# ChainSafe/halo2-verifier

Hardware: AMD Instinct MI355X
Metric: proofs verified/sec (BN254, k=14) (higher is better)
Workload: dtype u32 limbs (254-bit prime-field integers)

## Files before the change

### halo2_verifier_amd/csrc/batch.hip

```cpp
#include "../../include/h2v.h"
#include "batch.h"
#include <string.h>
#include <algorithm>
#include <utility>
#include <stdio.h>

using namespace h2v;

namespace h2v {

struct BatchSizes {
    uint32_t stream_words;
    size_t proofs, inst, pts, ycanon, words, chal, mult, slots, msm_scal, shared, left_scal, insteval, guard_scal, acc, results;
    uint32_t ws_terms, ws_problems, ws_per_problem;
};
BatchSizes batch_sizes(const Plan& pl, size_t N, size_t G, size_t largest) {
    BatchSizes z;
    z.stream_words = stream_words_for(pl.stream.size(), pl.opts.transcript);
    z.proofs = N * pl.proof_len;
    z.inst = N * (size_t)pl.n_instance_values * 32;
    z.pts = N * pl.n_points + pl.n_shared;
    z.ycanon = N * pl.n_points * 32;
    z.words = (size_t)z.stream_words * N;
    z.chal = (size_t)pl.squeeze_at.size() * N;
    z.mult = N;
    z.slots = (size_t)std::max(std::max(pl.n_slots, pl.n_slots_k[0]), std::max(pl.n_slots_k[1], pl.n_slots_k[2])) * N;
    z.msm_scal = (N * pl.n_points + G * pl.n_shared) * 8;
    z.shared = (size_t)pl.n_shared * N;
    z.left_scal = N * pl.n_points * 8;
    z.insteval = N * pl.inst_queries.size();
    z.guard_scal = N * pl.guard_term_order.size() * 8;
    z.acc = 2 * G;
    z.results = ResultsLayout{G, N}.total();
    z.ws_terms = (uint32_t)(2 * (N * pl.n_points + G * pl.n_shared));
    z.ws_problems = (uint32_t)(2 * G);
    z.ws_per_problem = (uint32_t)(largest * pl.n_points + pl.n_shared);
    return z;
}

int ensure_buffers(h2v_batch* b, const Plan& pl) {
    const size_t N = b->max_proofs, G = b->groups;
    size_t largest = (N + G - 1) / G;
    if (ragged(b)) { largest = 0; for (size_t g = 0; g < G; ++g) largest = std::max<size_t>(largest, b->group_off[g + 1] - b->group_off[g]); }
    const BatchSizes z = batch_sizes(pl, N, G, largest);
    int rc;
    if ((rc = b->proofs.reserve(z.proofs)) || (rc = b->inst.reserve(z.inst)) || (rc = b->pts.reserve(z.pts)) || (rc = b->phi.reserve(z.pts)) ||
        (rc = b->ycanon.reserve(z.ycanon)) || (rc = b->words.reserve(z.words)) || (rc = b->chal.reserve(z.chal)) || (rc = b->mult.reserve(z.mult)) ||
        (rc = b->slots.reserve(z.slots)) || (rc = b->msm_scal.reserve(z.msm_scal)) || (rc = b->shared.reserve(z.shared)) ||
        (rc = b->left_scal.reserve(z.left_scal)) || (rc = b->insteval.reserve(z.insteval)) || (rc = b->guard_scal.reserve(z.guard_scal)) ||
        (rc = b->acc.reserve(z.acc)) || (rc = b->results.reserve(z.results)) || (rc = b->results_host.reserve(z.results)))
        return rc;
    const ResultsLayout L{G, N};
    b->ok = reinterpret_cast<uint32_t*>(static_cast<uint8_t*>(b->results_host.dev) + L.ok());
    b->fold_failed = reinterpret_cast<uint32_t*>(b->results.p + L.fold_failed());
    b->out_ident = reinterpret_cast<uint32_t*>(b->results.p + L.out_ident());
    b->out_bytes = b->results.p + L.out_bytes();
    b->status = reinterpret_cast<int*>(b->results.p + L.status());
    if ((rc = b->ws.reserve(z.ws_terms, z.ws_problems, z.ws_per_problem))) return rc;
    b->stream_words = z.stream_words;
    return 0;
}

bool scalar_is_canonical(const uint8_t* s) {
    uint32_t raw[8];
    for (int j = 0; j < 8; ++j) raw[j] = (uint32_t)s[4 * j] | ((uint32_t)s[4 * j + 1] << 8) | ((uint32_t)s[4 * j + 2] << 16) | ((uint32_t)s[4 * j + 3] << 24);
    return !Fr::geq_p(raw);
}
bool scalar_is_zero(const uint8_t* s) { for (int k = 0; k < 32; ++k) if (s[k]) return false; return true; }

int os_random_scalars(std::vector<uint8_t>& out, size_t n) {
    out.resize(32 * n);
    FILE* f = fopen("/dev/urandom", "rb");
    if (!f) { set_last_error("cannot open /dev/urandom"); return H2V_ERR_DEVICE; }
    for (size_t i = 0; i < n; ++i) {
        uint8_t buf[64];
        if (fread(buf, 1, 64, f) != 64) { fclose(f); set_last_error("short read from /dev/urandom"); return H2V_ERR_DEVICE; }
        uint32_t w[16];
        for (int j = 0; j < 16; ++j) w[j] = (uint32_t)buf[4 * j] | ((uint32_t)buf[4 * j + 1] << 8) | ((uint32_t)buf[4 * j + 2] << 16) | ((uint32_t)buf[4 * j + 3] << 24);
        Fr::from_uniform_words(w).to_bytes(&out[32 * i]);
    }
    fclose(f);
    return 0;
}

int require_stage(const h2v_batch* b, BatchStage least, const char* who) {
    if (b && b->stage >= least) return 0;
    static const char* const missing[] = {"", "nothing uploaded since the last failed call or set_groups", "nothing launched", "no finished launch"};
    set_last_error(std::string(who) + ": " + (b ? missing[(int)least] : "null argument"));
    return H2V_ERR_BAD_ARGUMENT;
}

struct StageCommit {
    h2v_batch* b;
    ~StageCommit() { if (b) b->stage = BatchStage::Empty; }
    void commit(BatchStage st) { b->stage = st; b = nullptr; }
};

#define H2V_SPLIT_MAX_GROUPS 64u

ChannelTerms channel_terms(const Plan& pl, uint32_t count, uint32_t n_shared) {
    const bool strided = pl.left_term_order.size() == 1 && !pl.left_term_order[0].first;
    return ChannelTerms{strided, strided ? count : count * pl.n_points, count * pl.n_points + n_shared};
}
bool groups_cut_within_limit(const Plan& pl, const size_t* sizes, size_t n_groups) {
    std::vector<uint32_t> terms;
    for (size_t g = 0; g < n_groups; ++g) { const ChannelTerms t = channel_terms(pl, (uint32_t)sizes[g], pl.n_shared); terms.push_back(t.left); terms.push_back(t.right); }
    return msm_cuts_within_limit(terms.data(), terms.size());
}
void channel_problems(MsmProblems& pr, const h2v_batch* b, const Plan& pl, size_t p0, uint32_t count, G1J* acc2, const uint32_t* shared_scal, uint32_t n_shared) {
    const uint32_t np = pl.n_points;
    const size_t first = p0 * np;
    const ChannelTerms terms = channel_terms(pl, count, n_shared);
    if (terms.strided) {
        const size_t at = first + pl.left_term_order[0].second;
        pr.p.push_back(MsmProblem(b->left_scal.p + at * 8, b->pts.p + at, acc2, 8 * np, np, terms.left));
        pr.p.back().phi = b->phi.p + at;
    } else {
        pr.p.push_back(MsmProblem(b->left_scal.p + first * 8, b->pts.p + first, acc2, 8, 1, terms.left));
        pr.p.back().phi = b->phi.p + first;
        pr.p.back().nnz = count * (uint32_t)pl.left_term_order.size();
    }
    pr.p.push_back(MsmProblem(b->msm_scal.p + first * 8, b->pts.p + first, acc2 + 1, 8, 1, terms.right - n_shared, shared_scal, b->pts.p + (size_t)b->n * np, n_shared));
    pr.p.back().phi = b->phi.p + first; pr.p.back().phi2 = b->phi.p + (size_t)b->n * np;
}

int need_stream(h2v_batch* b) {
    if (b->stream || !b->owns_stream) return 0;
    H2V_HIP_CHECK(hipSetDevice(b->ctx->device));
    H2V_HIP_CHECK(hipStreamCreateWithFlags(&b->stream, hipStreamNonBlocking));
    return 0;
}
int need_aux(h2v_batch* b) {
    if (b->aux) return 0;
    H2V_HIP_CHECK(hipStreamCreateWithFlags(&b->aux, hipStreamNonBlocking));
    H2V_HIP_CHECK(hipEventCreateWithFlags(&b->ev_fork, hipEventDisableTiming));
    H2V_HIP_CHECK(hipEventCreateWithFlags(&b->ev_join, hipEventDisableTiming));
    return 0;
}

int close_enqueue(h2v_batch* b, bool with_pairing) {
    hipStream_t s = b->stream;
    const uint32_t G = b->groups;
    int rc;
    b->last.pairing = with_pairing; b->last.pieces = false; b->last.host_block = false;
    if (!with_pairing) {
        if (b->split.parts) { b->last.pieces = true; return 0; }
        return point_to_bytes_enqueue(s, b->acc.p, b->out_bytes, b->out_ident, 2 * G);
    }
    const ResultsLayout L{G, b->n};
    uint8_t* const host = static_cast<uint8_t*>(b->results_host.dev);
    const bool one_stream = b->ctx->tuning.pairing_one_stream != 0;
    if (b->split.parts && pairing_tail_fits(b->ctx->pairing, one_stream)) {
        PairTail t;
        t.pieces = b->split.pts; t.prs = b->ws.final_problems; t.count = b->split.count; t.parts = b->split.parts; t.shift = b->split.shift;
        t.out_bytes = b->out_bytes; t.out_ident = b->out_ident;
        t.host_bytes = host + L.out_bytes(); t.host_ident = reinterpret_cast<uint32_t*>(host + L.out_ident());
        t.src = reinterpret_cast<const uint32_t*>(b->results.p + L.fold_failed()); t.dst = reinterpret_cast<uint32_t*>(host + L.fold_failed());
        t.n_words = (uint32_t)((L.total() - L.fold_failed()) / 4);
        t.skip_lo = (uint32_t)((L.out_ident() - L.fold_failed()) / 4); t.skip_hi = (uint32_t)((L.status() - L.fold_failed()) / 4);
        if (t.count != 2 * G) { set_last_error("close_enqueue: the pieces are not this launch's"); return H2V_ERR_BAD_ARGUMENT; }
        b->last.host_block = true;
        return pairing_check_split_enqueue(s, b->ctx->pairing, b->split.ready, G, b->split.parts, b->split.shift, b->line_ws.p, b->ok, false, &t);
    }
    if ((rc = need_aux(b))) return rc;
    H2V_HIP_CHECK(hipEventRecord(b->ev_fork, s));
    H2V_HIP_CHECK(hipStreamWaitEvent(b->aux, b->ev_fork, 0));
    if (b->split.parts && (rc = msm_combine_enqueue(b->aux, b->ws, b->split, H2V_AUX_LDS_RESERVE))) return rc;
    if ((rc = point_to_bytes_enqueue(b->aux, b->acc.p, b->out_bytes, b->out_ident, 2 * G, H2V_AUX_LDS_RESERVE))) return rc;
    if ((rc = copy_words_enqueue(b->aux, b->results.p + L.fold_failed(), host + L.fold_failed(), (L.total() - L.fold_failed()) / 4, H2V_AUX_LDS_RESERVE))) return rc;
    H2V_HIP_CHECK(hipEventRecord(b->ev_join, b->aux));
    b->last.tail_on_aux = true; b->last.host_block = true;
    if (b->split.parts) { if ((rc = pairing_check_split_enqueue(s, b->ctx->pairing, b->split.ready, G, b->split.parts, b->split.shift, b->line_ws.p, b->ok, one_stream))) return rc; }
    else if ((rc = pairing_check_enqueue(s, b->ctx->pairing, b->acc.p, G, b->ok))) return rc;
    return 0;
}
int join_tail(h2v_batch* b) {
    if (!b->last.tail_on_aux) return 0;
    b->last.tail_on_aux = false;
    H2V_HIP_CHECK(hipStreamWaitEvent(b->stream, b->ev_join, 0));
    return 0;
}
int ensure_whole(h2v_batch* b) {
    if (!b->last.pieces) return 0;
    int rc;
    if ((rc = msm_combine_enqueue(b->stream, b->ws, b->split))) return rc;
    if ((rc = point_to_bytes_enqueue(b->stream, b->acc.p, b->out_bytes, b->out_ident, 2 * b->groups))) return rc;
    b->last.pieces = false;
    return 0;
}

int resolve_draws(const uint8_t*& rand32, size_t n, std::vector<uint8_t>& storage, const char* who, bool nonzero) {
    int rc;
    std::vector<uint8_t> one;
    if (!rand32) {
        if ((rc = os_random_scalars(storage, n))) return rc;
        for (size_t i = 0; nonzero && i < n; ++i)
            while (scalar_is_zero(&storage[32 * i])) { if ((rc = os_random_scalars(one, 1))) return rc; memcpy(&storage[32 * i], one.data(), 32); }
        rand32 = storage.data();
        return 0;
    }
    for (size_t i = 0; i < n; ++i) {
        if (nonzero && scalar_is_zero(rand32 + 32 * i)) { set_last_error(std::string(who) + ": a draw in rand32 is zero"); return H2V_ERR_BAD_ARGUMENT; }
        if (!scalar_is_canonical(rand32 + 32 * i)) { set_last_error(std::string(who) + ": rand32 scalar not canonical"); return H2V_ERR_BAD_ARGUMENT; }
    }
    return 0;
}

static StageArgs stage_args(const h2v_batch* b) {
    return StageArgs{b->n, &b->plan->host, b->plan, b->proofs.p, b->inst.p, b->pts.p, b->phi.p, b->ycanon.p, b->status, b->words.p, b->stream_words, b->chal.p};
}

static int draw_multipliers_enqueue(h2v_batch* b) {
    if (ragged(b)) return ragged_multipliers_enqueue(b->stream, b->tail.p, b->d_group_last.p, b->n, b->mult.p, b->mult_tiles.p, b->mult_seg.p);
    return multipliers_enqueue(b->stream, b->tail.p, b->n_tail, b->n, b->groups, b->mult.p, b->mult_tiles.p);
}

int upload_impl(h2v_batch* b, size_t n, const uint8_t* proofs_flat, size_t proof_len, const uint8_t* instances_flat, size_t ncols, const size_t* col_lens,
                const uint8_t* rand_tail, size_t n_tail, bool overlap, bool guard) {
    StageCommit commit{b};
    if (!b || (n && !proofs_flat)) { set_last_error("h2v_batch_upload: null argument"); return H2V_ERR_BAD_ARGUMENT; }
    if (n > b->max_proofs) { set_last_error("h2v_batch_upload: n exceeds the batch capacity"); return H2V_ERR_BAD_ARGUMENT; }
    h2v_ctx* ctx = b->ctx;
    H2V_HIP_CHECK(hipSetDevice(ctx->device));
    if (!ctx->vk) { set_last_error("the context was created without a VerifyingKey"); return H2V_ERR_BAD_ARGUMENT; }
    if (ncols != ctx_total_instance_columns(ctx)) { set_last_error("instances do not match the VK's instance column count"); return H2V_ERR_INVALID_INSTANCES; }
    PlanPin pin(ctx);
    int rc = pin.get(std::vector<size_t>(col_lens, col_lens + ncols), guard);
    if (rc) return rc;
    const Plan& pl = pin.pd->host;
    if (proof_len < pl.proof_len) { set_last_error("h2v_batch_upload: proof_len is shorter than this VK's proof"); return H2V_ERR_BAD_ARGUMENT; }
    if (pl.n_instance_values && n && !instances_flat) { set_last_error("h2v_batch_upload: instances missing"); return H2V_ERR_BAD_ARGUMENT; }
    if (rand_tail && n_tail < n) { set_last_error("h2v_batch_upload: n_tail < n"); return H2V_ERR_BAD_ARGUMENT; }
    if (ragged(b)) {
        if (n != b->group_off.back()) { set_last_error("h2v_batch_upload: n is not the sum of the group sizes (h2v_batch_set_group_sizes)"); return H2V_ERR_BAD_ARGUMENT; }
        if (rand_tail && n_tail != n) { set_last_error("h2v_batch_upload: groups of unequal size take one draw per proof (n_tail == n)"); return H2V_ERR_BAD_ARGUMENT; }
        std::vector<size_t> sizes(b->groups);
        for (size_t g = 0; g < b->groups; ++g) sizes[g] = b->group_off[g + 1] - b->group_off[g];
        if (!ctx->tuning.msm_no_term_split && !groups_cut_within_limit(pl, sizes.data(), sizes.size())) {
            set_last_error("h2v_batch_upload: the groups' MSM problems, cut into sub-problems of at most 16384 terms, exceed the launch's problem limit");
            return H2V_ERR_UNSUPPORTED;
        }
    } else if (b->groups > 1 && (n % b->groups || (rand_tail && n_tail % b->groups))) { set_last_error("h2v_batch_upload: n and n_tail must be multiples of the group count"); return H2V_ERR_BAD_ARGUMENT; }
    std::vector<uint8_t> os_rand;
    if (!rand_tail) n_tail = n;
    if ((rc = resolve_draws(rand_tail, n_tail, os_rand, "h2v_batch_upload"))) return rc;
    if ((rc = need_stream(b)) || (rc = join_tail(b)) || (rc = ensure_buffers(b, pl))) return rc;
    if (b->plan) ctx_put_plan(ctx, b->plan);
    b->plan = pin.take(); b->n = (uint32_t)n;
    const PlanDevice* pd = b->plan;
    b->zero_below.assign(b->groups, 0);
    if (ragged(b)) {
        for (size_t g = 0; g < b->groups; ++g)
            for (size_t f = b->group_off[g], j = b->group_off[g + 1] - f; j-- > 1;)
                if (scalar_is_zero(rand_tail + 32 * (f + j))) { b->zero_below[g] = (uint32_t)j; break; }
    } else if (n) {
        const size_t G = b->groups, gs = n / G, nt = n_tail / G;
        for (size_t g = 0; g < G; ++g)
            for (size_t j = nt; j-- > 1;)
                if (scalar_is_zero(rand_tail + 32 * (g * nt + j))) { b->zero_below[g] = (uint32_t)std::min(j, gs); break; }
    }
    if ((rc = b->tail.reserve(32 * n_tail))) return rc;
    if (ragged(b)) {
        const size_t tiles = ragged_multipliers_tiles((uint32_t)n);
        if ((rc = b->mult_tiles.reserve(tiles)) || (rc = b->mult_seg.reserve(2 * tiles)) || (rc = b->d_group_off.reserve(b->group_off.size())) || (rc = b->d_group_last.reserve(n))) return rc;
    } else if ((rc = b->mult_tiles.reserve(multipliers_scratch((uint32_t)n_tail, b->groups)))) return rc;
    b->n_tail = (uint32_t)n_tail; b->mult_of_draws = false;
    hipStream_t s = b->stream;
    auto copy_proofs = [&](hipStream_t cs, size_t p0, size_t p1) -> int {
        if (proof_len == pl.proof_len) H2V_HIP_CHECK(hipMemcpyAsync(b->proofs.p + p0 * pl.proof_len, proofs_flat + p0 * proof_len, (p1 - p0) * proof_len, hipMemcpyHostToDevice, cs));
        else H2V_HIP_CHECK(hipMemcpy2DAsync(b->proofs.p + p0 * pl.proof_len, pl.proof_len, proofs_flat + p0 * proof_len, proof_len, pl.proof_len, p1 - p0, hipMemcpyHostToDevice, cs));
        return 0;
    };
    auto copy_rest = [&](hipStream_t cs) -> int {
        if (pl.n_instance_values) H2V_HIP_CHECK(hipMemcpyAsync(b->inst.p, instances_flat, n * (size_t)pl.n_instance_values * 32, hipMemcpyHostToDevice, cs));
        H2V_HIP_CHECK(hipMemcpyAsync(b->tail.p, rand_tail, 32 * n_tail, hipMemcpyHostToDevice, cs));
        if (ragged(b)) {
            H2V_HIP_CHECK(hipMemcpyAsync(b->d_group_last.p, b->group_last.data(), n, hipMemcpyHostToDevice, cs));
            H2V_HIP_CHECK(hipMemcpyAsync(b->d_group_off.p, b->group_off.data(), 4 * b->group_off.size(), hipMemcpyHostToDevice, cs));
        }
        H2V_HIP_CHECK(hipMemcpyAsync(b->pts.p + n * (size_t)pl.n_points, pd->shared_bases.p, sizeof(G1A) * pl.n_shared, hipMemcpyDeviceToDevice, cs));
        H2V_HIP_CHECK(hipMemcpyAsync(b->phi.p + n * (size_t)pl.n_points, pd->shared_phi.p, sizeof(G1A) * pl.n_shared, hipMemcpyDeviceToDevice, cs));
        return 0;
    };
    std::vector<std::pair<uint32_t, uint32_t>> runs;
    {
        std::vector<uint32_t> offs(pl.point_offsets);
        std::sort(offs.begin(), offs.end());
        for (uint32_t o : offs) { if (!runs.empty() && runs.back().first + runs.back().second == o) runs.back().second += 32; else runs.push_back({o, 32u}); }
    }
    size_t point_bytes = 0;
    for (auto& r : runs) point_bytes += r.second;
    const bool points_first = overlap && n >= 2048 &&
                              runs.size() <= 4 && 2 * point_bytes <= pl.proof_len;
    if (!points_first) {
        if (n && ((rc = copy_proofs(s, 0, n)) || (rc = copy_rest(s)))) return rc;
        H2V_HIP_CHECK(hipStreamSynchronize(s));
    } else {
        if (!b->copy) H2V_HIP_CHECK(hipStreamCreateWithFlags(&b->copy, hipStreamNonBlocking));
        H2V_HIP_CHECK(hipStreamSynchronize(s));
        const StageArgs g = stage_args(b);
        for (auto& r : runs) H2V_HIP_CHECK(hipMemcpy2DAsync(b->proofs.p + r.first, pl.proof_len, proofs_flat + r.first, proof_len, r.second, n, hipMemcpyHostToDevice, b->copy));
        H2V_HIP_CHECK(hipStreamSynchronize(b->copy));
        if ((rc = decompress_begin_enqueue(s, g))) return rc;
        if ((rc = decompress_range_enqueue(s, g, 0, (uint32_t)n))) return rc;
        if ((rc = copy_proofs(b->copy, 0, n)) || (rc = copy_rest(b->copy))) return rc;
        H2V_HIP_CHECK(hipStreamSynchronize(b->copy));
        if ((rc = decompress_finish_enqueue(s, g))) return rc;
    }
    b->decompressed = points_first;
    if (n) { if ((rc = draw_multipliers_enqueue(b))) return rc; b->mult_of_draws = true; }
    commit.commit(BatchStage::Uploaded);
    return 0;
}

int launch_impl(h2v_batch* b, int with_pairing, const Fr* ext_mult, const uint32_t* ext_idx) {
    int rc;
    if ((rc = require_stage(b, BatchStage::Uploaded, "h2v_batch_launch"))) return rc;
    StageCommit commit{b};
    h2v_ctx* ctx = b->ctx;
    H2V_HIP_CHECK(hipSetDevice(ctx->device));
    PlanDevice* pd = b->plan;
    const Plan& pl = pd->host;
    hipStream_t s = b->stream;
    uint32_t n = b->n;
    const uint32_t G = b->groups;
    if ((rc = join_tail(b))) return rc;
    int ev = 0;
    auto mark = [&]() { if (b->profiling >= 2) hipEventRecord(b->ev[ev], s); ++ev; };
    mark();
    const StageArgs g = stage_args(b);
    const bool run_decompress = !(b->stage == BatchStage::Uploaded && b->decompressed);
    const ResultsLayout L{G, n};
    if (run_decompress && n) H2V_HIP_CHECK(hipMemsetAsync(b->fold_failed, 0, L.total() - L.fold_failed(), s));
    else H2V_HIP_CHECK(hipMemsetAsync(b->fold_failed, 0, 4 * (size_t)G, s));
    if (run_decompress && n && ((rc = decompress_finish_enqueue(s, g)) || (rc = decompress_range_enqueue(s, g, 0, n)))) return rc;
    mark();
    if ((rc = transcript_stage_enqueue(s, g))) return rc;
    MsmProblems pr;
    for (uint32_t g = 0; g < G; ++g)
        channel_problems(pr, b, pl, group_first(b, g), (uint32_t)group_count(b, g), b->acc.p + 2 * g, b->msm_scal.p + ((size_t)n * pl.n_points + (size_t)g * pl.n_shared) * 8, n ? pl.n_shared : 0);
    b->ws.tune = ctx->tuning;
    if (n) {
        if (ext_mult) { b->mult_of_draws = false; if ((rc = gather_multipliers_enqueue(s, ext_mult, ext_idx, n, b->mult.p))) return rc; }
        else if (!b->mult_of_draws) { if ((rc = draw_multipliers_enqueue(b))) return rc; b->mult_of_draws = true; }
        if (!(pl.left_term_order.size() == 1 && !pl.left_term_order[0].first)) H2V_HIP_CHECK(hipMemsetAsync(b->left_scal.p, 0, (size_t)n * pl.n_points * 32, s));
    }
    mark();
    FrvmArgs a{pd->code.p, (uint32_t)pl.code.size(), pd->consts.p, b->slots.p, n, b->proofs.p, pl.proof_len, pd->scalar_offsets.p, b->inst.p, pl.n_instance_values,
               b->chal.p, b->mult.p, b->status, b->msm_scal.p, pl.n_points, b->shared.p, b->left_scal.p, b->insteval.p, b->guard_scal.p, (uint32_t)pl.guard_term_order.size()};
    if (n && pl.wide_instances) {
        Fr step = pl.omega;
        for (int i = 0; i < 8; ++i) step = step.sqr();
        const Fr step_inv = step.inv();
        for (size_t q = 0; q < pl.inst_queries.size(); ++q) {
            InstEvalArgs ia{b->inst.p, pl.n_instance_values, b->chal.p, pl.x_chal, n, pl.domain_k, pl.inst_queries[q].base, pl.inst_queries[q].len,
                            pl.inst_queries[q].w_start, pl.omega, step, step_inv, pl.n_inv, b->insteval.p + q * (size_t)n, b->status};
            if ((rc = instance_eval_enqueue(s, ia))) return rc;
        }
    }
    a.force_streams = ctx->tuning.frvm_streams; a.force_lds_kb = ctx->tuning.frvm_lds_kb;
    for (int k = 0; k < 3; ++k) { for (int q = 0; q < k + 2; ++q) { a.code_k[k][q] = pd->code_k[k][q].p; a.n_code_k[k][q] = (uint32_t)pl.code_k[k][q].size(); } a.n_slots_k[k] = pl.n_slots_k[k]; }
    if ((rc = frvm_enqueue(s, a, pl.n_slots))) return rc;
    mark();
    if (n) {
        if (ragged(b)) rc = fold_shared_offsets_enqueue(s, b->shared.p, n, pl.n_points, pl.n_shared, G, b->d_group_off.p, b->msm_scal.p);
        else rc = fold_shared_enqueue(s, b->shared.p, n, pl.n_points, pl.n_shared, G, b->msm_scal.p);
        if (rc) return rc;
    }
    mark();
    {
        b->ws.profile = b->profiling >= 1; b->ws.profile_recorded = false;
        b->split = MsmSplit();
        const uint32_t parts_knob = ctx->tuning.msm_parts > 0 ? (uint32_t)ctx->tuning.msm_parts : MSM_MAX_PARTS;
        b->ws.tune = ctx->tuning;
        if (n && G <= H2V_SPLIT_MAX_GROUPS && parts_knob > 1) {
            const size_t line_bytes = (size_t)G * H2V_PAIRING_LINE_WS_BYTES;
            if (b->line_ws.p && line_bytes > b->line_ws.cap) H2V_HIP_CHECK(hipStreamSynchronize(s));
            if ((rc = b->line_ws.reserve(line_bytes))) return rc;
            b->split.want_parts = parts_knob;
        }
        if ((rc = msm_enqueue_multi(s, b->ws, pr, b->split.want_parts > 1 ? &b->split : nullptr))) return rc;
    }
    mark();
    if ((rc = close_enqueue(b, with_pairing != 0))) return rc;
    b->last.folded = false;
    mark();
    commit.commit(BatchStage::Launched);
    return 0;
}

int export_whole_records(h2v_batch* b, void* device_dst) {
    int rc;
    if ((rc = join_tail(b)) || (rc = ensure_whole(b))) return rc;
    return export_records_enqueue(b->stream, b->acc.p, nullptr, 1, 0, b->status, b->n, b->groups, device_dst);
}

int finish_impl(h2v_batch* b, const char* who, int* per_proof_status, int* group_ok, uint8_t* out_left, uint8_t* out_right) {
    if (int rc = require_stage(b, BatchStage::Launched, who)) return rc;
    StageCommit commit{b};
    H2V_HIP_CHECK(hipSetDevice(b->ctx->device));
    hipStream_t s = b->stream;
    const uint32_t n = b->n, G = b->groups;
    { int rcw = ensure_whole(b); if (rcw) return rcw; }
    const ResultsLayout L{G, n};
    hipError_t e;
    if (b->last.host_block) {
        e = hipStreamSynchronize(s);
        if (e == hipSuccess && b->last.tail_on_aux) e = hipStreamSynchronize(b->aux);
        b->last.tail_on_aux = false;
    } else {
        H2V_HIP_CHECK(hipMemcpyAsync(b->results_host.p + L.fold_failed(), b->results.p + L.fold_failed(), L.total() - L.fold_failed(), hipMemcpyDeviceToHost, s));
        e = hipStreamSynchronize(s);
    }
    if (e != hipSuccess) { set_last_error(std::string("h2v_batch_finish: ") + hipGetErrorString(e)); return H2V_ERR_DEVICE; }
    const uint8_t* host = b->results_host.p;
    const uint32_t* okv = reinterpret_cast<const uint32_t*>(host + L.ok());
    const uint32_t* foldf = reinterpret_cast<const uint32_t*>(host + L.fold_failed());
    const uint8_t* outb = host + L.out_bytes();
    const int* st = reinterpret_cast<const int*>(host + L.status());
    for (int i = 0; i < 7; ++i) b->last_ms[i] = 0;
    if (b->profiling >= 2) {
        float t01 = 0, t12 = 0, t23 = 0, t34 = 0, t45 = 0, t56 = 0;
        hipEventElapsedTime(&t01, b->ev[0], b->ev[1]); hipEventElapsedTime(&t12, b->ev[1], b->ev[2]); hipEventElapsedTime(&t23, b->ev[2], b->ev[3]);
        hipEventElapsedTime(&t34, b->ev[3], b->ev[4]); hipEventElapsedTime(&t45, b->ev[4], b->ev[5]); hipEventElapsedTime(&t56, b->ev[5], b->ev[6]);
        b->last_ms[0] = t01; b->last_ms[1] = t12; b->last_ms[2] = t23; b->last_ms[3] = t34; b->last_ms[4] = t45; b->last_ms[5] = t56;
    }
    if (b->profiling >= 1) {
        float tacc = 0;
        if (b->ws.profile_recorded) hipEventElapsedTime(&tacc, b->ws.ev_acc[0], b->ws.ev_acc[1]);
        b->last_ms[6] = tacc;
    }
    std::vector<char> all_ok(G, 1);
    uint32_t any = 0;
    for (uint32_t i = 0; i < n; ++i) any |= (uint32_t)st[i];
    if (!any) { if (per_proof_status && n) memset(per_proof_status, 0, sizeof(int) * (size_t)n); }
    else for (uint32_t g = 0, i = 0; g < G; ++g) for (uint32_t k = 0, gs = (uint32_t)group_count(b, g); k < gs; ++k, ++i) {
        const int v = status_decode(st[i]);
        if (per_proof_status) per_proof_status[i] = v;
        if (v != 0) all_ok[g] = 0;
    }
    for (uint32_t g = 0; g < G; ++g) {
        if (group_ok) group_ok[g] = (all_ok[g] && !foldf[g] && (!b->last.pairing || okv[g])) ? 1 : 0;
        if (out_left) memcpy(out_left + 64 * (size_t)g, &outb[128 * (size_t)g], 64);
        if (out_right) memcpy(out_right + 64 * (size_t)g, &outb[128 * (size_t)g + 64], 64);
    }
    commit.commit(BatchStage::Finished);
    return 0;
}
bool pairing_passed(const h2v_batch* b, uint32_t g) {
    return b->last.pairing && reinterpret_cast<const uint32_t*>(b->results_host.p + ResultsLayout{b->groups, b->n}.ok())[g] != 0;
}

bool same_srs(const ParamsHost& a, const ParamsHost& b) {
    auto same_g2 = [](const G2A& p, const G2A& q) { return p.inf == q.inf && !memcmp(&p.x, &q.x, sizeof(Fq2)) && !memcmp(&p.y, &q.y, sizeof(Fq2)); };
    return !memcmp(&a.g, &b.g, sizeof(G1A)) && same_g2(a.g2, b.g2) && same_g2(a.s_g2, b.s_g2);
}

int recheck_impl(const char* who, h2v_batch* const* batches, size_t n_batches, size_t n_ranges, const uint32_t* batch_of_range, const size_t* first,
                 const size_t* count, int* range_ok, uint8_t* out_left, uint8_t* out_right) {
    const std::string w(who);
    int rc;
    if (!batches || !n_batches) { set_last_error(w + ": null argument"); return H2V_ERR_BAD_ARGUMENT; }
    for (size_t k = 0; k < n_batches; ++k) {
        if ((rc = require_stage(batches[k], BatchStage::Finished, who))) return rc;
        if (batches[k]->ctx->device != batches[0]->ctx->device) { set_last_error(w + ": batches on different devices"); return H2V_ERR_BAD_ARGUMENT; }
        if (!same_srs(batches[k]->ctx->params, batches[0]->ctx->params)) { set_last_error(w + ": batches over different params (g[0], g2 or s_g2 differ)"); return H2V_ERR_BAD_ARGUMENT; }
    }
    if (n_ranges && (!first || !count || !range_ok)) { set_last_error(w + ": null argument"); return H2V_ERR_BAD_ARGUMENT; }
    auto batch_of = [&](size_t i) -> h2v_batch* { return batches[batch_of_range ? batch_of_range[i] : 0]; };
    for (size_t i = 0; i < n_ranges; ++i) {
        if (batch_of_range && batch_of_range[i] >= n_batches) { set_last_error(w + ": batch index out of range"); return H2V_ERR_BAD_ARGUMENT; }
        const h2v_batch* b = batch_of(i);
        const size_t n = b->n;
        const size_t f = first[i], c = count[i];
        if (!c || f >= n || c > n - f) { set_last_error(w + ": empty range, or a range past the launch's proofs"); return H2V_ERR_BAD_ARGUMENT; }
        const size_t g = group_of(b, f);
        if (group_of(b, f + c - 1) != g) { set_last_error(w + ": a range crosses a group boundary of the launch"); return H2V_ERR_BAD_ARGUMENT; }
        if (f - group_first(b, g) < b->zero_below[g]) { set_last_error(w + ": a range covers a proof whose multiplier is zero (a zero draw)"); return H2V_ERR_BAD_ARGUMENT; }
    }
    if (!n_ranges) return 0;
    h2v_batch* host = batches[0];
    h2v_ctx* ctx = host->ctx;
    H2V_HIP_CHECK(hipSetDevice(ctx->device));
    if ((rc = join_tail(host))) return rc;
    for (size_t k = 1; k < n_batches; ++k)
        if (batches[k] != host) { H2V_HIP_CHECK(hipStreamSynchronize(batches[k]->stream)); if (batches[k]->aux) H2V_HIP_CHECK(hipStreamSynchronize(batches[k]->aux)); }
    hipStream_t s = host->stream;
    Recheck& rk = host->recheck;
    const uint32_t max_ranges = MSM_MAX_PROBLEMS / 2;
    auto plan_of = [&](size_t i) -> const Plan& { return batch_of(i)->plan->host; };
    auto strided = [](const Plan& pl) { return pl.left_term_order.size() == 1 && !pl.left_term_order[0].first; };
    auto terms_of = [&](size_t i) { const Plan& pl = plan_of(i); const size_t c = count[i], np = pl.n_points; return (strided(pl) ? c : c * np) + c * np + pl.n_shared; };
    size_t budget = 0;
    for (size_t k = 0; k < n_batches; ++k) { const Plan& pl = batches[k]->plan->host; budget = std::max(budget, 2 * ((size_t)batches[k]->n * pl.n_points + (size_t)max_ranges * pl.n_shared)); }
    if ((rc = rk.ranges.reserve(max_ranges)) || (rc = rk.acc.reserve(2 * (size_t)max_ranges)) || (rc = rk.ok.reserve(max_ranges)) ||
        (rc = rk.out_bytes.reserve(128 * (size_t)max_ranges)) || (rc = rk.out_ident.reserve(2 * (size_t)max_ranges))) return rc;
    std::vector<FoldRange> desc;
    std::vector<uint32_t> okv;
    std::vector<uint8_t> outb;
    for (size_t i0 = 0; i0 < n_ranges;) {
        size_t i1 = i0, total = 0;
        uint32_t per = 0, rows = 0, max_shared = 0;
        while (i1 < n_ranges && i1 - i0 < max_ranges && (i1 == i0 || total + terms_of(i1) <= budget)) {
            const Plan& pl = plan_of(i1);
            total += terms_of(i1);
            per = std::max(per, (uint32_t)(count[i1] * pl.n_points + pl.n_shared));
            rows += pl.n_shared; max_shared = std::max(max_shared, pl.n_shared);
            ++i1;
        }
        const uint32_t R = (uint32_t)(i1 - i0);
        const bool grow = !rk.ws.covers((uint32_t)total, 2 * R, per) || rk.fold.cap < 8 * (size_t)rows;
        if (grow) H2V_HIP_CHECK(hipStreamSynchronize(s));
        if ((rc = rk.ws.reserve((uint32_t)total, 2 * R, per)) || (rc = rk.fold.reserve(8 * (size_t)std::max(rows, 1u)))) return rc;
        desc.resize(R);
        for (uint32_t r = 0, row = 0; r < R; ++r) {
            const h2v_batch* b = batch_of(i0 + r);
            const uint32_t ns = b->plan->host.n_shared;
            desc[r] = FoldRange{b->shared.p, b->n, ns, (uint32_t)first[i0 + r], (uint32_t)count[i0 + r], row, 0};
            row += ns;
        }
        H2V_HIP_CHECK(hipMemcpyAsync(rk.ranges.p, desc.data(), sizeof(FoldRange) * R, hipMemcpyHostToDevice, s));
        if ((rc = fold_shared_ranges_enqueue(s, rk.ranges.p, R, max_shared, rk.fold.p))) return rc;
        MsmProblems pr;
        for (uint32_t r = 0; r < R; ++r)
            channel_problems(pr, batch_of(i0 + r), plan_of(i0 + r), first[i0 + r], (uint32_t)count[i0 + r], rk.acc.p + 2 * r, rk.fold.p + (size_t)desc[r].out * 8, desc[r].n_shared);
        rk.ws.tune = ctx->tuning; rk.ws.profile = false;
        if ((rc = msm_enqueue_multi(s, rk.ws, pr))) return rc;
        if ((rc = pairing_check_enqueue(s, ctx->pairing, rk.acc.p, R, rk.ok.p))) return rc;
        okv.resize(R);
        H2V_HIP_CHECK(hipMemcpyAsync(okv.data(), rk.ok.p, 4 * (size_t)R, hipMemcpyDeviceToHost, s));
        if (out_left || out_right) {
            if ((rc = point_to_bytes_enqueue(s, rk.acc.p, rk.out_bytes.p, rk.out_ident.p, 2 * R))) return rc;
            outb.resize(128 * (size_t)R);
            H2V_HIP_CHECK(hipMemcpyAsync(outb.data(), rk.out_bytes.p, outb.size(), hipMemcpyDeviceToHost, s));
        }
        const hipError_t e = hipStreamSynchronize(s);
        if (e != hipSuccess) { set_last_error(w + ": " + hipGetErrorString(e)); return H2V_ERR_DEVICE; }
        for (uint32_t r = 0; r < R; ++r) {
            range_ok[i0 + r] = okv[r] ? 1 : 0;
            if (out_left) memcpy(out_left + 64 * (i0 + r), &outb[128 * (size_t)r], 64);
            if (out_right) memcpy(out_right + 64 * (i0 + r), &outb[128 * (size_t)r + 64], 64);
        }
        i0 = i1;
    }
    return 0;
}

}

extern "C" {

int h2v_batch_recheck(h2v_batch* b, size_t n_ranges, const size_t* first, const size_t* count, int* range_ok, uint8_t* out_left, uint8_t* out_right) {
    if (!b) return require_stage(b, BatchStage::Finished, "h2v_batch_recheck");
    return recheck_impl("h2v_batch_recheck", &b, 1, n_ranges, nullptr, first, count, range_ok, out_left, out_right);
}

int h2v_batches_recheck(h2v_batch* const* batches, size_t n_batches, size_t n_ranges, const uint32_t* batch_of_range, const size_t* first, const size_t* count,
                        int* range_ok, uint8_t* out_left_xy, uint8_t* out_right_xy) {
    if (!batches || (n_ranges && !batch_of_range)) { set_last_error("h2v_batches_recheck: null argument"); return H2V_ERR_BAD_ARGUMENT; }
    return recheck_impl("h2v_batches_recheck", batches, n_batches, n_ranges, batch_of_range, first, count, range_ok, out_left_xy, out_right_xy);
}

int h2v_random_scalars(uint8_t* out32, size_t n) {
    if (n && !out32) { set_last_error("h2v_random_scalars: null argument"); return H2V_ERR_BAD_ARGUMENT; }
    std::vector<uint8_t> v;
    int rc = os_random_scalars(v, n);
    if (rc) return rc;
    if (n) memcpy(out32, v.data(), 32 * n);
    return 0;
}

int h2v_ctx_proof_shape(const h2v_ctx* ctx, size_t* proof_len, size_t* n_points, size_t* n_scalars, size_t* n_right_terms, size_t* n_instance_columns) {
    if (!ctx || !ctx->vk) { set_last_error("the context was created without a VerifyingKey"); return H2V_ERR_BAD_ARGUMENT; }
    std::vector<size_t> lens(ctx_total_instance_columns(ctx), 0);
    PlanPin pin(const_cast<h2v_ctx*>(ctx));
    int rc = pin.get(lens);
    if (rc) return rc;
    PlanDevice* pd = pin.pd;
    if (proof_len) *proof_len = pd->host.proof_len;
    if (n_points) *n_points = pd->host.n_points;
    if (n_scalars) *n_scalars = pd->host.n_scalars;
    if (n_right_terms) *n_right_terms = pd->host.right_term_order.size();
    if (n_instance_columns) *n_instance_columns = ctx_total_instance_columns(ctx);
    return 0;
}

int h2v_batch_create(h2v_ctx* ctx, size_t max_proofs, size_t max_instance_values_per_proof, h2v_batch** out) {
    if (!ctx || !out || !max_proofs) { set_last_error("h2v_batch_create: bad argument"); return H2V_ERR_BAD_ARGUMENT; }
    if (max_proofs > (1u << 22)) { set_last_error("h2v_batch_create: max_proofs too large"); return H2V_ERR_BAD_ARGUMENT; }
    H2V_HIP_CHECK(hipSetDevice(ctx->device));
    h2v_batch* b = new h2v_batch();
    b->ctx = ctx; b->max_proofs = max_proofs; b->max_inst = max_instance_values_per_proof;
    for (int i = 0; i < 8; ++i) hipEventCreate(&b->ev[i]);
    *out = b;
    return 0;
}

void h2v_batch_destroy(h2v_batch* b) {
    if (!b) return;
    hipSetDevice(b->ctx->device);
    if (b->stream || !b->owns_stream) hipStreamSynchronize(b->stream);
    if (b->aux) hipStreamSynchronize(b->aux);
    if (b->plan) { ctx_put_plan(b->ctx, b->plan); b->plan = nullptr; }
    for (int i = 0; i < 8; ++i) if (b->ev[i]) hipEventDestroy(b->ev[i]);
    if (b->aux) { hipStreamSynchronize(b->aux); hipStreamDestroy(b->aux); }
    if (b->copy) { hipStreamSynchronize(b->copy); hipStreamDestroy(b->copy); }

    if (b->ev_fork) hipEventDestroy(b->ev_fork);
    if (b->ev_join) hipEventDestroy(b->ev_join);
    if (b->stream && b->owns_stream) hipStreamDestroy(b->stream);
    delete b;
}

int h2v_batch_upload(h2v_batch* b, size_t n, const uint8_t* proofs_flat, size_t proof_len, const uint8_t* instances_flat, size_t n_instance_columns,
                     const size_t* col_lens, const uint8_t* rand32_tail, size_t n_tail) {
    return upload_impl(b, n, proofs_flat, proof_len, instances_flat, n_instance_columns, col_lens, rand32_tail, n_tail);
}
int h2v_batch_launch(h2v_batch* b, int with_pairing) { return launch_impl(b, with_pairing); }
int h2v_batch_upload_launch(h2v_batch* b, size_t n, const uint8_t* proofs_flat, size_t proof_len, const uint8_t* instances_flat, size_t n_instance_columns,
                            const size_t* col_lens, const uint8_t* rand32_tail, size_t n_tail, int with_pairing) {
    if (int rc = upload_impl(b, n, proofs_flat, proof_len, instances_flat, n_instance_columns, col_lens, rand32_tail, n_tail, true)) return rc;
    return launch_impl(b, with_pairing);
}
int h2v_batch_finish(h2v_batch* b, int* per_proof_status, int* batch_ok, uint8_t out_left_xy[64], uint8_t out_right_xy[64]) {
    if (b && b->groups > 1) { set_last_error("h2v_batch_finish: the batch is grouped, use h2v_batch_finish_groups"); return H2V_ERR_BAD_ARGUMENT; }
    return finish_impl(b, "h2v_batch_finish", per_proof_status, batch_ok, out_left_xy, out_right_xy);
}
int h2v_batch_set_groups(h2v_batch* b, size_t groups) {
    if (!b || !groups || groups > MSM_MAX_PROBLEMS / 2 || groups > b->max_proofs) { set_last_error("h2v_batch_set_groups: bad group count"); return H2V_ERR_BAD_ARGUMENT; }
    if (b->stream) hipStreamSynchronize(b->stream);
    if (b->aux) hipStreamSynchronize(b->aux);
    if (b->copy) hipStreamSynchronize(b->copy);
    if (b->plan) { ctx_put_plan(b->ctx, b->plan); b->plan = nullptr; }
    b->groups = (uint32_t)groups; b->stage = BatchStage::Empty;
    b->group_off.clear(); b->group_last.clear();
    return 0;
}
int h2v_batch_set_group_sizes(h2v_batch* b, const size_t* sizes, size_t n_groups) {
    static const char who[] = "h2v_batch_set_group_sizes";
    if (!b || !sizes || !n_groups || n_groups > MSM_MAX_PROBLEMS / 2) { set_last_error(std::string(who) + ": null argument or bad group count"); return H2V_ERR_BAD_ARGUMENT; }
    size_t total = 0;
    for (size_t g = 0; g < n_groups; ++g) {
        if (!sizes[g]) { set_last_error(std::string(who) + ": a group of no proofs"); return H2V_ERR_BAD_ARGUMENT; }
        if (sizes[g] > b->max_proofs - total) { set_last_error(std::string(who) + ": the sizes exceed the batch capacity"); return H2V_ERR_BAD_ARGUMENT; }
        total += sizes[g];
    }
    if (b->stream) hipStreamSynchronize(b->stream);
    if (b->aux) hipStreamSynchronize(b->aux);
    if (b->copy) hipStreamSynchronize(b->copy);
    if (b->plan) { ctx_put_plan(b->ctx, b->plan); b->plan = nullptr; }
    b->groups = (uint32_t)n_groups; b->stage = BatchStage::Empty;
    b->group_off.assign(n_groups + 1, 0); b->group_last.assign(total, 0);
    for (size_t g = 0; g < n_groups; ++g) { b->group_off[g + 1] = b->group_off[g] + (uint32_t)sizes[g]; b->group_last[b->group_off[g + 1] - 1] = 1; }
    return 0;
}
int h2v_batch_finish_groups(h2v_batch* b, int* per_proof_status, int* group_ok, uint8_t* out_left_xy, uint8_t* out_right_xy, size_t n_groups) {
    if (!b || n_groups != b->groups) { set_last_error("h2v_batch_finish_groups: n_groups does not match h2v_batch_set_groups"); return H2V_ERR_BAD_ARGUMENT; }
    return finish_impl(b, "h2v_batch_finish_groups", per_proof_status, group_ok, out_left_xy, out_right_xy);
}
int h2v_batch_accumulators(h2v_batch* b, void** device_ptr, size_t* nbytes) {
    if (!b || !b->acc.p || !device_ptr) { set_last_error("h2v_batch_accumulators: nothing uploaded"); return H2V_ERR_BAD_ARGUMENT; }
    if (b->stage >= BatchStage::Launched) { H2V_HIP_CHECK(hipSetDevice(b->ctx->device)); int rcw = join_tail(b); if (!rcw) rcw = ensure_whole(b); if (rcw) return rcw; }
    *device_ptr = b->acc.p;
    if (nbytes) *nbytes = 2 * sizeof(G1J) * b->groups;
    return 0;
}
void* h2v_batch_stream(h2v_batch* b) { return b && !need_stream(b) ? (void*)b->stream : nullptr; }
int h2v_batch_set_stream(h2v_batch* b, void* hip_stream) {
    if (!b) return H2V_ERR_BAD_ARGUMENT;
    hipSetDevice(b->ctx->device);
    if (b->stream || !b->owns_stream) hipStreamSynchronize(b->stream);
    if (b->owns_stream && b->stream) hipStreamDestroy(b->stream);
    b->stream = (hipStream_t)hip_stream; b->owns_stream = false;
    return join_tail(b);
}
int h2v_batch_export_accumulators(h2v_batch* b, void* device_dst) {
    if (int rc = require_stage(b, BatchStage::Launched, "h2v_batch_export_accumulators")) return rc;
    if (!device_dst) { set_last_error("h2v_batch_export_accumulators: null argument"); return H2V_ERR_BAD_ARGUMENT; }
    if (ragged(b)) { set_last_error("h2v_batch_export_accumulators: the batch has groups of unequal size (a record counts the failures of n / groups proofs)"); return H2V_ERR_BAD_ARGUMENT; }
    H2V_HIP_CHECK(hipSetDevice(b->ctx->device));
    if (int rc = join_tail(b)) return rc;
    if (b->split.parts) return export_records_enqueue(b->stream, nullptr, b->split.pts, b->split.parts, b->split.shift, b->status, b->n, b->groups, device_dst);
    return export_records_enqueue(b->stream, b->acc.p, nullptr, 1, 0, b->status, b->n, b->groups, device_dst);
}
int h2v_batch_fold_check_enqueue(h2v_batch* b, const void* device_accumulators, size_t n_parts) {
    int rc;
    if ((rc = require_stage(b, BatchStage::Launched, "h2v_batch_fold_check_enqueue"))) return rc;
    if (ragged(b)) { set_last_error("h2v_batch_fold_check_enqueue: the batch has groups of unequal size"); return H2V_ERR_BAD_ARGUMENT; }
    StageCommit commit{b};
    if (!device_accumulators || !n_parts) { set_last_error("h2v_batch_fold_check_enqueue: bad argument"); return H2V_ERR_BAD_ARGUMENT; }
    H2V_HIP_CHECK(hipSetDevice(b->ctx->device));
    if ((rc = join_tail(b))) return rc;
    const uint32_t G = b->groups;
    if (b->split.parts) {
        G1JSlot* pieces = b->ws.pieces.p; G1JSlot* ready = b->ws.pieces.p + (size_t)MSM_MAX_PARTS * b->ws.cap_problems;
        if ((rc = fold_records_enqueue(b->stream, device_accumulators, (uint32_t)n_parts, G, b->split.parts, b->split.shift, b->acc.p, pieces, ready, b->fold_failed))) return rc;
    } else if ((rc = fold_records_enqueue(b->stream, device_accumulators, (uint32_t)n_parts, G, 1, 0, b->acc.p, nullptr, nullptr, b->fold_failed))) return rc;
    if ((rc = close_enqueue(b, true))) return rc;
    b->last.folded = true;
    commit.commit(b->stage);
    return 0;
}
int h2v_batch_identify(h2v_batch* b, const void* own_records, int* per_proof_status, int* group_own_ok, size_t* n_range_checks) {
    static const char who[] = "h2v_batch_identify";
    int rc;
    if ((rc = require_stage(b, BatchStage::Finished, who))) return rc;
    const uint32_t n = b->n, G = b->groups;
    if (!own_records && b->last.folded) { set_last_error(std::string(who) + ": a fold has replaced the batch's own accumulators: pass the records it exported"); return H2V_ERR_BAD_ARGUMENT; }
    for (uint32_t g = 0; g < G; ++g)
        if (b->zero_below[g]) { set_last_error(std::string(who) + ": a proof of the batch has a zero multiplier (a zero draw)"); return H2V_ERR_BAD_ARGUMENT; }
    h2v_ctx* ctx = b->ctx;
    H2V_HIP_CHECK(hipSetDevice(ctx->device));
    hipStream_t s = b->stream;
    H2V_HIP_CHECK(hipStreamSynchronize(s));
    if (b->aux) H2V_HIP_CHECK(hipStreamSynchronize(b->aux));
    const ResultsLayout L{G, n};
    const int* raw = reinterpret_cast<const int*>(b->results_host.p + L.status());
    std::vector<std::vector<int>> st(1, std::vector<int>(n));
    std::vector<uint32_t> failed(G, 0);
    for (uint32_t i = 0; i < n; ++i) { st[0][i] = status_decode(raw[i]); if (raw[i]) ++failed[group_of(b, i)]; }
    if (own_records && ragged(b)) { set_last_error(std::string(who) + ": a batch with groups of unequal size exports no records"); return H2V_ERR_BAD_ARGUMENT; }
    if (own_records) {
        std::vector<uint32_t> hdr(4 * (size_t)G);
        H2V_HIP_CHECK(hipMemcpy2DAsync(hdr.data(), 16, own_records, H2V_ACC_RECORD_BYTES, 16, G, hipMemcpyDeviceToHost, s));
        H2V_HIP_CHECK(hipStreamSynchronize(s));
        for (uint32_t g = 0; g < G; ++g)
            if (hdr[4 * g + 1] < 1 || hdr[4 * g + 1] > H2V_ACC_RECORD_PIECES || hdr[4 * g] != failed[g]) {
                set_last_error(std::string(who) + ": own_records does not hold the records this launch exported (piece count, or failure count against the statuses)");
                return H2V_ERR_BAD_ARGUMENT;
            }
    }
    std::vector<uint32_t> own(G, 0);
    if (b->last.pairing && !b->last.folded) {
        for (uint32_t g = 0; g < G; ++g) own[g] = pairing_passed(b, g) ? 1u : 0u;
    } else {
        Recheck& rk = b->recheck;
        const uint32_t max_ranges = MSM_MAX_PROBLEMS / 2;
        if ((rc = rk.acc.reserve(2 * (size_t)max_ranges)) || (rc = rk.ok.reserve(max_ranges)) || (rc = rk.failed.reserve(max_ranges))) return rc;
        if ((rc = join_tail(b))) return rc;
        const G1J* pts = b->acc.p;
        if (own_records) {
            if ((rc = fold_records_enqueue(s, own_records, 1, G, 1, 0, rk.acc.p, nullptr, nullptr, rk.failed.p))) return rc;
            pts = rk.acc.p;
        }
        if ((rc = pairing_check_enqueue(s, ctx->pairing, pts, G, rk.ok.p))) return rc;
        H2V_HIP_CHECK(hipMemcpyAsync(own.data(), rk.ok.p, 4 * (size_t)G, hipMemcpyDeviceToHost, s));
        const hipError_t e = hipStreamSynchronize(s);
        if (e != hipSuccess) { set_last_error(std::string(who) + ": " + hipGetErrorString(e)); return H2V_ERR_DEVICE; }
    }
    std::vector<IdentifyStart> start;
    for (uint32_t g = 0; g < G; ++g) if (!own[g] && group_count(b, g)) start.push_back({0, group_first(b, g), group_count(b, g)});
    size_t checks = 0;
    if (!start.empty() && (rc = identify_search({b}, start, true, st, &checks))) return rc;
    if (per_proof_status) for (uint32_t i = 0; i < n; ++i) per_proof_status[i] = st[0][i];
    if (group_own_ok) for (uint32_t g = 0; g < G; ++g) group_own_ok[g] = own[g] ? 1 : 0;
    if (n_range_checks) *n_range_checks = checks;
    return 0;
}
int h2v_batch_set_profiling(h2v_batch* b, int level) { if (!b) return H2V_ERR_BAD_ARGUMENT; b->profiling = level == 0 ? 0 : (level == H2V_PROFILE_KERNEL ? 1 : 2); return 0; }
int h2v_batch_timings(h2v_batch* b, float* ms, int cap) {
    if (!b || !ms) return H2V_ERR_BAD_ARGUMENT;
    int k = cap < 7 ? cap : 7;
    for (int i = 0; i < k; ++i) ms[i] = b->last_ms[i];
    return k;
}

}
```

### halo2_verifier_amd/csrc/internal.h

```cpp
#pragma once
#include <hip/hip_runtime.h>
#include <stdint.h>
#include <string>
#include <vector>
#include "../../include/h2v.h"
#include "curve.hip.h"

namespace h2v {

void set_last_error(const std::string& s);
#define H2V_HIP_CHECK(expr)                                                                     \
    do {                                                                                        \
        hipError_t e_ = (expr);                                                                 \
        if (e_ != hipSuccess) {                                                                 \
            ::h2v::set_last_error(std::string(#expr) + ": " + hipGetErrorString(e_));           \
            return H2V_ERR_DEVICE;                                                              \
        }                                                                                       \
    } while (0)

template <class T> struct DevBuf {
    T* p = nullptr;
    size_t cap = 0;
    DevBuf() {}
    DevBuf(const DevBuf&) = delete;
    DevBuf& operator=(const DevBuf&) = delete;
    DevBuf(DevBuf&& o) noexcept : p(o.p), cap(o.cap) { o.p = nullptr; o.cap = 0; }
    DevBuf& operator=(DevBuf&& o) noexcept { if (this != &o) { reset(); p = o.p; cap = o.cap; o.p = nullptr; o.cap = 0; } return *this; }
    ~DevBuf() { reset(); }
    int alloc(size_t count) {
        reset();
        H2V_HIP_CHECK(hipMalloc(&p, (count ? count : 1) * sizeof(T)));
        cap = count ? count : 1;
        return 0;
    }
    int reserve(size_t count) { return p && count <= cap ? 0 : alloc(count); }
    void reset() { if (p) hipFree(p); p = nullptr; cap = 0; }
};

struct MappedHostBuf {
    uint8_t* p = nullptr;
    void* dev = nullptr;
    size_t cap = 0;
    MappedHostBuf() {}
    MappedHostBuf(const MappedHostBuf&) = delete;
    MappedHostBuf& operator=(const MappedHostBuf&) = delete;
    ~MappedHostBuf() { reset(); }
    int reserve(size_t bytes) {
        if (p && bytes <= cap) return 0;
        reset();
        H2V_HIP_CHECK(hipHostMalloc((void**)&p, bytes ? bytes : 1, hipHostMallocMapped));
        H2V_HIP_CHECK(hipHostGetDevicePointer(&dev, p, 0));
        cap = bytes ? bytes : 1;
        return 0;
    }
    void reset() { if (p) hipHostFree(p); p = nullptr; dev = nullptr; cap = 0; }
};


struct MsmPlan {
    uint32_t n;
    uint32_t c;
    uint32_t windows;
    uint32_t buckets;
};
MsmPlan msm_plan(uint32_t n, bool latency = false);

struct MsmProblem {
    const uint32_t* scalars; const G1A* bases; G1J* out;
    uint32_t sstride, bstride, n;
    uint32_t n1;
    const uint32_t* scalars2; const G1A* bases2;
    const G1A* phi = nullptr; const G1A* phi2 = nullptr;
    uint32_t glv_off = 0;
    uint32_t sub_first = 0, sub_count = 0;
    uint32_t nnz = 0;
    MsmProblem() : scalars(nullptr), bases(nullptr), out(nullptr), sstride(8), bstride(1), n(0), n1(0), scalars2(nullptr), bases2(nullptr) {}
    MsmProblem(const uint32_t* s, const G1A* b, G1J* o, uint32_t ss, uint32_t bs, uint32_t n_) : scalars(s), bases(b), out(o), sstride(ss), bstride(bs), n(n_), n1(n_), scalars2(nullptr), bases2(nullptr) {}
    MsmProblem(const uint32_t* s, const G1A* b, G1J* o, uint32_t ss, uint32_t bs, uint32_t n1_, const uint32_t* s2, const G1A* b2, uint32_t n2)
        : scalars(s), bases(b), out(o), sstride(ss), bstride(bs), n(n1_ + n2), n1(n1_), scalars2(s2), bases2(b2) {}
};
#define MSM_MAX_PROBLEMS 1024
#define MSM_PROBLEM_CHUNK 44
struct MsmProblemChunk { MsmProblem p[MSM_PROBLEM_CHUNK]; };
static_assert(sizeof(MsmProblemChunk) <= 4000, "a chunk of problem descriptors travels as one kernel argument (4 KB limit)");
struct MsmProblems { std::vector<MsmProblem> p; };

struct alignas(128) G1JSlot {
    G1J p;
    uint32_t pad[5];
    __host__ __device__ G1JSlot& operator=(const G1J& v) { p = v; for (int i = 0; i < 5; ++i) pad[i] = 0; return *this; }
    __host__ __device__ operator const G1J&() const { return p; }
};

#define MSM_MAX_PARTS 6
struct MsmSplit {
    uint32_t want_parts = 0;
    uint32_t parts = 0, shift = 0, count = 0;
    const G1JSlot* pts = nullptr;
    const G1JSlot* ready = nullptr;
};

struct AccRecord { uint32_t failed, parts, shift, reserved; G1J left[H2V_ACC_RECORD_PIECES], right[H2V_ACC_RECORD_PIECES]; };
static_assert(sizeof(AccRecord) == H2V_ACC_RECORD_BYTES && H2V_ACC_RECORD_BYTES == 16 + 2 * H2V_ACC_RECORD_PIECES * 108, "accumulator record layout");
static_assert(H2V_ACC_RECORD_PIECES >= MSM_MAX_PARTS, "a record holds every piece a launch can leave");

struct MsmWorkspace {
    uint32_t cap_terms = 0, cap_parents = 0, cap_per_problem = 0;
    uint32_t cap_problems = 0;
    size_t cap_buckets = 0, cap_list = 0;
    DevBuf<uint32_t> counts;
    DevBuf<uint32_t> offsets;
    DevBuf<uint32_t> cursor;
    DevBuf<uint32_t> list;
    DevBuf<G1JSlot> bucket_pts;
    DevBuf<G1JSlot> window_sums;
    DevBuf<G1JSlot> pieces;
    std::vector<MsmProblem> resident;
    int resident_no_split = 0;
    DevBuf<MsmProblem> problems;
    DevBuf<MsmProblem> parents;
    DevBuf<G1JSlot> merged_sums;
    const MsmProblem* final_problems = nullptr;
    DevBuf<uint32_t> block_sums;
    DevBuf<G1JSlot> partial;
    DevBuf<uint32_t> redo;
    DevBuf<uint32_t> glv;
    DevBuf<G1A> phi_pts;
    DevBuf<uint32_t> seg_total;
    DevBuf<uint32_t> seg_start;
    h2v_tuning tune = {};
    bool profile = false, profile_recorded = false;
    hipEvent_t ev_acc[2] = {nullptr, nullptr};
    int reserve(uint32_t max_total_terms, uint32_t max_problems, uint32_t max_terms_per_problem = 0);
    bool covers(uint32_t max_total_terms, uint32_t max_problems, uint32_t max_terms_per_problem = 0) const;
    MsmWorkspace() {}
    MsmWorkspace(const MsmWorkspace&) = delete;
    MsmWorkspace& operator=(const MsmWorkspace&) = delete;
    ~MsmWorkspace() { for (hipEvent_t e : ev_acc) if (e) hipEventDestroy(e); }
};
int msm_enqueue_multi(hipStream_t s, MsmWorkspace& ws, const MsmProblems& pr, MsmSplit* split = nullptr);
int msm_combine_enqueue(hipStream_t s, MsmWorkspace& ws, const MsmSplit& sp, size_t lds_reserve = 0);
bool msm_cuts_within_limit(const uint32_t* terms, size_t n_problems);
#define H2V_AUX_LDS_RESERVE ((size_t)110 * 1024)
int msm_enqueue(hipStream_t s, MsmWorkspace& ws, const uint32_t* d_scalars, const G1A* d_bases, uint32_t n, G1J* d_out);
int accumulator_scale_enqueue(hipStream_t s, const G1J* d_points, const uint32_t* d_scalar_words, void* d_record);
int accumulator_scale_many_enqueue(hipStream_t s, const G1J* d_pairs, const uint32_t* d_slots, const uint32_t* d_scalar_words, uint32_t n, void* d_records);

int bases_from_bytes_enqueue(hipStream_t s, const uint8_t* d_bytes, G1A* d_out, uint32_t* d_flags, uint32_t n);
int scalars_from_bytes_enqueue(hipStream_t s, const uint8_t* d_bytes, uint32_t* d_out, uint32_t* d_flags, uint32_t n);
int copy_words_enqueue(hipStream_t s, const void* d_src, void* d_dst, size_t n_words, size_t lds_reserve = 0);
int point_to_bytes_enqueue(hipStream_t s, const G1J* d_in, uint8_t* d_out_xy64, uint32_t* d_is_identity, uint32_t n, size_t lds_reserve = 0);
int export_records_enqueue(hipStream_t s, const G1J* d_acc, const G1JSlot* d_pieces, uint32_t parts, uint32_t shift, const int* d_status, uint32_t n, uint32_t groups, void* d_out);
int fold_records_enqueue(hipStream_t s, const void* d_recs, uint32_t n_recs, uint32_t groups, uint32_t parts, uint32_t shift, G1J* d_acc, G1JSlot* d_pieces, G1JSlot* d_ready,
                         uint32_t* d_fold_failed);
uint32_t accumulator_merge_team(uint32_t n);
int accumulator_merge_fold_enqueue(hipStream_t s, const void* d_recs, uint32_t n, uint32_t team, const uint32_t* d_slots, G1J* d_sums, G1J* d_acc);

}
```

### halo2_verifier_amd/csrc/msm.hip

```cpp
#include "../../include/h2v.h"
#include <hip/hip_ext.h>
#include "batch.h"

namespace h2v {

#define MSM_LDS_SORT_MAX_TERMS 16384u
#define MSM_SORT_THREADS 512u
#define MSM_CHUNK_MIN 16u
#define MSM_CHUNK_MAX 64u
#define MSM_ACC_LANES_PER_ROUND 196608u
#define MSM_CHUNK_SMALL 4u
#define MSM_SHORT_LIST 98304u
__host__ __device__ __forceinline__ uint32_t msm_chunk_len(uint32_t E, uint32_t R) {
    if (E <= MSM_SHORT_LIST) return MSM_CHUNK_SMALL;
    if (E <= R * MSM_CHUNK_MIN) return MSM_CHUNK_MIN;
    const uint32_t k = (uint32_t)(((uint64_t)E + (uint64_t)R * MSM_CHUNK_MAX - 1) / ((uint64_t)R * MSM_CHUNK_MAX));
    const uint32_t c = (uint32_t)(((uint64_t)E + (uint64_t)k * R - 1) / ((uint64_t)k * R));
    return c < MSM_CHUNK_MIN ? MSM_CHUNK_MIN : c;
}
static inline uint32_t msm_accumulate_blocks(size_t max_entries, size_t R) {
    size_t lanes;
    if (max_entries <= R * MSM_CHUNK_MIN)
        lanes = std::max<size_t>((max_entries + MSM_CHUNK_MIN - 1) / MSM_CHUNK_MIN, (std::min<size_t>(max_entries, MSM_SHORT_LIST) + MSM_CHUNK_SMALL - 1) / MSM_CHUNK_SMALL);
    else lanes = (max_entries + R * MSM_CHUNK_MAX - 1) / (R * MSM_CHUNK_MAX) * R;
    return (uint32_t)(((lanes + 63) / 64 + 1 + 7) / 8 * 8);
}
#define MSM_CONTROL_WORDS 8u
#define MSM_FIXUP_SERIAL 64u
#define MSM_FIXUP_TEAM 3u
#define MSM_FIXUP_TEAM_BLOCKS 256u
#define MSM_FIXUP_HEAVY_BLOCKS 256u
#define MSM_WIN_THREADS 256

static inline uint32_t msm_window_threads(uint32_t buckets, uint32_t n_workgroups = 0xffffffffu, int forced = 0) {
    if (buckets <= 64) return std::max(1u, buckets);
    if (n_workgroups != 0xffffffffu && (forced == 64 || forced == 128 || forced == 256)) return (uint32_t)forced;
    if (buckets > 2048 || (buckets >= 256 && n_workgroups <= 256)) return 256u;
    return 64u;
}

MsmPlan msm_plan(uint32_t n, bool latency) {
    MsmPlan best{n, 2, 65, 2};
    double best_cost = 1e300;
    for (uint32_t c = 2; c <= 15; ++c) {
        uint32_t w = (130 + c - 1) / c;
        uint32_t b = 1u << (c - 1);
        uint32_t T = msm_window_threads(b), slice = (b + T - 1) / T;
        double lg = 0; for (uint32_t t = T; t > 1; t >>= 1) lg += 1;
        double cost = latency ? 9.0 * w + 9.0 * (2.0 * slice + 1.5 * c + 1.0 + lg) + 5.0 * std::min<double>(32.0, 2.0 * n)
                              : (double)w * (11.0 * 2.0 * n + 16.0 * T * (2.0 * slice + 1.5 * c + 1.0 + lg));
        if (cost < best_cost) { best_cost = cost; best = MsmPlan{n, c, w, b}; }
    }
    return best;
}
static inline bool msm_latency_bound(size_t total_terms) { return total_terms <= 4096; }

static inline uint32_t msm_subproblems(uint32_t n) { return n > MSM_LDS_SORT_MAX_TERMS ? (n + MSM_LDS_SORT_MAX_TERMS - 1) / MSM_LDS_SORT_MAX_TERMS : 1u; }
bool msm_cuts_within_limit(const uint32_t* terms, size_t n_problems) {
    size_t subs = 0;
    for (size_t q = 0; q < n_problems; ++q) subs += msm_subproblems(terms[q]);
    return subs <= MSM_MAX_PROBLEMS;
}
bool MsmWorkspace::covers(uint32_t max_terms, uint32_t max_problems, uint32_t max_per_problem) const {
    if (!max_per_problem || max_per_problem > max_terms) max_per_problem = max_terms;
    return counts.p && max_terms <= cap_terms && max_problems <= cap_parents && max_per_problem <= cap_per_problem;
}
int MsmWorkspace::reserve(uint32_t max_terms, uint32_t max_problems, uint32_t max_per_problem) {
    if (!max_per_problem || max_per_problem > max_terms) max_per_problem = max_terms;
    if (covers(max_terms, max_problems, max_per_problem)) return 0;
    max_terms = std::max(max_terms, cap_terms); max_problems = std::max(max_problems, cap_parents); max_per_problem = std::max(max_per_problem, cap_per_problem);
    cap_terms = cap_parents = cap_per_problem = 0;
    resident.clear(); final_problems = nullptr; profile_recorded = false;
    const uint32_t subs = msm_subproblems(max_per_problem);
    cap_problems = (uint32_t)std::min<size_t>((size_t)max_problems * subs, MSM_MAX_PROBLEMS);
    if (cap_problems < max_problems) cap_problems = max_problems;
    const uint32_t per_sub = subs > 1 ? MSM_LDS_SORT_MAX_TERMS : max_per_problem;
    const uint32_t form_n[2] = {per_sub, max_per_problem}, form_q[2] = {cap_problems, max_problems};
    size_t mb = 0;
    cap_list = 0;
    for (int f = 0; f < 2; ++f) {
        size_t fb = 0;
        for (int lat = 0; lat < 2; ++lat) {
            for (uint32_t n = 1; n <= form_n[f]; n = n < 16 ? n + 1 : n + n / 8) { MsmPlan p = msm_plan(n, lat != 0); fb = std::max(fb, (size_t)p.windows * p.buckets); }
            MsmPlan p = msm_plan(form_n[f], lat != 0); fb = std::max(fb, (size_t)p.windows * p.buckets);
        }
        mb = std::max(mb, fb * form_q[f]);
        for (uint32_t n = 1;; n = n < 16 ? n + 1 : n + n / 8) {
            if (n > form_n[f]) n = form_n[f];
            size_t terms = n <= MSM_LDS_SORT_MAX_TERMS ? (size_t)n * form_q[f] : std::min<size_t>((size_t)max_terms, (size_t)n * form_q[f]);
            cap_list = std::max(cap_list, terms * 2 * std::max(msm_plan(n, false).windows, msm_plan(n, true).windows));
            if (n == form_n[f]) break;
        }
    }
    cap_buckets = mb;
    const size_t max_chunks = std::max<size_t>(cap_list / MSM_CHUNK_MIN + 1, std::min<size_t>(cap_list, MSM_SHORT_LIST) / MSM_CHUNK_SMALL + 1);
    int rc;
    if ((rc = counts.alloc(mb + MSM_CONTROL_WORDS)) || (rc = offsets.alloc(mb)) ||
        (rc = cursor.alloc(2 * mb)) ||
        (rc = list.alloc(cap_list)) || (rc = bucket_pts.alloc(mb)) || (rc = window_sums.alloc((size_t)128 * cap_problems)) ||
        (rc = merged_sums.alloc((size_t)128 * max_problems)) || (rc = pieces.alloc((size_t)2 * MSM_MAX_PARTS * cap_problems)) ||
        (rc = problems.alloc(cap_problems)) || (rc = parents.alloc(max_problems)) || (rc = block_sums.alloc(mb / 1024 + 2)) ||
        (rc = partial.alloc(max_chunks * 2)) || (rc = redo.alloc(max_chunks)) ||
        (rc = glv.alloc(cap_list / 2 + 1)) ||
        (rc = phi_pts.alloc((size_t)max_terms + 1)) || (rc = seg_total.alloc((size_t)128 * cap_problems + 2)) || (rc = seg_start.alloc((size_t)128 * cap_problems + 2))) {
        cap_problems = 0; cap_buckets = cap_list = 0;
        return rc;
    }
    for (int i = 0; i < 2; ++i) if (!ev_acc[i]) H2V_HIP_CHECK(hipEventCreate(&ev_acc[i]));
    cap_terms = max_terms; cap_parents = max_problems; cap_per_problem = max_per_problem;
    return 0;
}

__device__ __forceinline__ void mul_lo5(uint32_t out[5], const uint32_t* a, int na, const uint32_t* b, int nb) {
    uint64_t acc[5] = {0, 0, 0, 0, 0};
    for (int i = 0; i < na && i < 5; ++i) {
        uint64_t carry = 0;
        for (int j = 0; j < nb && i + j < 5; ++j) {
            uint64_t t = (uint64_t)a[i] * b[j] + (uint32_t)acc[i + j] + carry;
            acc[i + j] = (uint32_t)t; carry = t >> 32;
        }
    }
    for (int i = 0; i < 5; ++i) out[i] = (uint32_t)acc[i];
}
__device__ __forceinline__ void mul_hi256(uint32_t out[5], const uint32_t k[8], const uint32_t g[5]) {
    uint32_t t[13];
    for (int i = 0; i < 13; ++i) t[i] = 0;
    for (int i = 0; i < 8; ++i) {
        uint64_t carry = 0;
        for (int j = 0; j < 5; ++j) {
            uint64_t v = (uint64_t)k[i] * g[j] + t[i + j] + carry;
            t[i + j] = (uint32_t)v; carry = v >> 32;
        }
        t[i + 5] = (uint32_t)carry;
    }
    for (int i = 0; i < 5; ++i) out[i] = t[8 + i];
}
__device__ __forceinline__ void mul_lo8(uint32_t out[8], const uint32_t a[8], const uint32_t* b, int nb) {
    for (int i = 0; i < 8; ++i) out[i] = 0;
    for (int j = 0; j < nb; ++j) {
        uint64_t carry = 0;
        for (int i = 0; i + j < 8; ++i) {
            uint64_t t = (uint64_t)a[i] * b[j] + out[i + j] + carry;
            out[i + j] = (uint32_t)t; carry = t >> 32;
        }
    }
}
__device__ __forceinline__ bool glv_geq_r(const uint32_t v[8]) {
    const uint32_t RW[8] = {0xf0000001u, 0x43e1f593u, 0x79b97091u, 0x2833e848u, 0x8181585du, 0xb85045b6u, 0xe131a029u, 0x30644e72u};
    for (int i = 7; i >= 0; --i) { if (v[i] > RW[i]) return true; if (v[i] < RW[i]) return false; }
    return true;
}
struct GlvHalf { uint32_t mag[5]; bool neg; };
__device__ __forceinline__ void glv_finish(GlvHalf& h, uint32_t t[5]) {
    h.neg = (t[4] >> 31) != 0;
    if (h.neg) { uint64_t c = 1; for (int i = 0; i < 5; ++i) { uint64_t v = (uint64_t)(~t[i]) + c; t[i] = (uint32_t)v; c = v >> 32; } }
    for (int i = 0; i < 5; ++i) h.mag[i] = t[i];
}
__device__ __forceinline__ void glv_decompose(const uint32_t* __restrict__ k, GlvHalf& h1, GlvHalf& h2) {
    const uint32_t A1[5] = {0x7d4f1128u, 0x8211bbebu, 0xeeb859fcu, 0x6f4d8248u, 0u};
    const uint32_t B1N[5] = {0x94d213e3u, 0x89d32568u, 0u, 0u, 0u};
    const uint32_t B2[5] = {0x1221250bu, 0x0be4e154u, 0xeeb859fdu, 0x6f4d8248u, 0u};
    const uint32_t G1[5] = {0x00ff6565u, 0x5398fd03u, 0xa773d2d2u, 0x4ccef014u, 0x2u};
    const uint32_t G2[5] = {0xc7e0b3d7u, 0xd91d232eu, 0x2u, 0u, 0u};
    uint32_t kk[8];
    for (int i = 0; i < 8; ++i) kk[i] = k[i];
    uint32_t c1[5], c2[5], p1[5], p2[5], t1[8], t2[8];
    mul_hi256(c1, kk, G1);
    mul_hi256(c2, kk, G2);
    mul_lo5(p1, c1, 5, A1, 5); mul_lo5(p2, c2, 5, B1N, 5);
    {
        int64_t borrow = 0;
        for (int i = 0; i < 5; ++i) { int64_t v = (int64_t)kk[i] - p1[i] - p2[i] + borrow; t1[i] = (uint32_t)v; borrow = v >> 32; }
    }
    mul_lo5(p1, c1, 5, B1N, 5); mul_lo5(p2, c2, 5, B2, 5);
    {
        int64_t borrow = 0;
        for (int i = 0; i < 5; ++i) { int64_t v = (int64_t)p1[i] - p2[i] + borrow; t2[i] = (uint32_t)v; borrow = v >> 32; }
    }
    {
        const uint32_t s1 = (t1[4] >> 31) ? 0xffffffffu : 0u, s2 = (t2[4] >> 31) ? 0xffffffffu : 0u;
        for (int i = 5; i < 8; ++i) { t1[i] = s1; t2[i] = s2; }
        uint32_t u[8], v[8], w[8];
        mul_lo8(u, t1, B2, 4); mul_lo8(w, t2, B1N, 2);
        { int64_t borrow = 0; for (int i = 0; i < 8; ++i) { int64_t d = (int64_t)u[i] - w[i] + borrow; u[i] = (uint32_t)d; borrow = d >> 32; } }
        mul_lo8(v, t2, A1, 4); mul_lo8(w, t1, B1N, 2);
        { uint64_t carry = 0; for (int i = 0; i < 8; ++i) { uint64_t d = (uint64_t)v[i] + w[i] + carry; v[i] = (uint32_t)d; carry = d >> 32; } }
        const bool e1 = glv_geq_r(u), e2 = glv_geq_r(v);
        int64_t b1 = 0, b2 = 0;
        for (int i = 0; i < 5; ++i) {
            int64_t d = (int64_t)t1[i] - (e1 ? A1[i] : 0u) - (e2 ? B1N[i] : 0u) + b1; t1[i] = (uint32_t)d; b1 = d >> 32;
            d = (int64_t)t2[i] + (e1 ? B1N[i] : 0u) - (e2 ? B2[i] : 0u) + b2; t2[i] = (uint32_t)d; b2 = d >> 32;
        }
    }
    glv_finish(h1, t1);
    glv_finish(h2, t2);
}
__device__ __forceinline__ uint32_t raw_window(const uint32_t m[5], uint32_t w, uint32_t c) {
    uint32_t off = w * c, word = off >> 5, sh = off & 31;
    if (word >= 5) return 0;
    uint32_t v = m[word] >> sh;
    if (sh + c > 32 && word + 1 < 5) v |= m[word + 1] << (32 - sh);
    return v & ((1u << c) - 1);
}
#define ACC_SCALE_TABLE 8u
#define ACC_SCALE_DIGITS 33u
__global__ void __launch_bounds__(64) k_accumulator_scale(const G1J* __restrict__ in, const uint32_t* __restrict__ slots, const uint32_t* __restrict__ scalars,
                                                          AccRecord* __restrict__ out) {
    __shared__ G1J table[4][ACC_SCALE_TABLE];
    __shared__ G1J half_sum[4];
    const uint32_t item = blockIdx.x;
    in += 2 * (size_t)(slots ? slots[item] : item);
    const uint32_t* m_words = scalars + 8 * (size_t)item;
    out += item;
    const uint32_t lane = threadIdx.x, chain = (lane >> 2) & 3u, r = lane & 3u;
    const uint32_t side = chain >> 1, half = chain & 1u;
    const bool writer = lane < 16 && r == 0;
    uint32_t k[8];
    for (int i = 0; i < 8; ++i) k[i] = m_words[i];
    GlvHalf h1, h2;
    glv_decompose(k, h1, h2);
    const bool neg = half ? h2.neg : h1.neg;
    uint32_t mag[5];
    {
        uint64_t c = 0;
        for (int i = 0; i < 5; ++i) { const uint64_t v = (uint64_t)(half ? h2.mag[i] : h1.mag[i]) + (i < 4 ? 0x88888888u : 0x8u) + c; mag[i] = (uint32_t)v; c = v >> 32; }
    }
    G1J p = in[side];
    if (half) p.X = g1_beta_times(p.X);
    if (neg) p.Y = p.Y.neg();
    {
        G1J t = p;
        if (writer) table[chain][0] = t;
        t = g1_dbl(t);
        if (writer) table[chain][1] = t;
#pragma unroll 1
        for (uint32_t j = 2; j < ACC_SCALE_TABLE; ++j) { t = g1_add(t, p); if (writer) table[chain][j] = t; }
    }
    __syncthreads();
    G1J acc = G1J::identity();
#pragma unroll 1
    for (int w = (int)ACC_SCALE_DIGITS - 1; w >= 0; --w) {
        if (w != (int)ACC_SCALE_DIGITS - 1) {
#pragma unroll 1
            for (int i = 0; i < 4; ++i) g1_dbl_quad(acc, r);
        }
        const int d = (int)raw_window(mag, (uint32_t)w, 4) - 8;
        if (d != 0) {
            G1J t = table[chain][(d < 0 ? -d : d) - 1];
            if (d < 0) t.Y = t.Y.neg();
            acc = g1_add_inl(acc, t);
        }
    }
    if (writer) half_sum[chain] = acc;
    __syncthreads();
    if (lane < 2) {
        const G1J a = half_sum[2 * lane], b = half_sum[2 * lane + 1];
        G1J* dst = lane ? out->right : out->left;
        dst[0] = g1_add_inl(a, b);
        for (uint32_t j = 1; j < H2V_ACC_RECORD_PIECES; ++j) dst[j] = G1J::identity();
    }
    if (lane == 0) { out->failed = 0; out->parts = 1; out->shift = 0; out->reserved = 0; }
}
int accumulator_scale_enqueue(hipStream_t s, const G1J* d_points, const uint32_t* d_scalar_words, void* d_record) {
    return accumulator_scale_many_enqueue(s, d_points, nullptr, d_scalar_words, 1, d_record);
}
int accumulator_scale_many_enqueue(hipStream_t s, const G1J* d_pairs, const uint32_t* d_slots, const uint32_t* d_scalar_words, uint32_t n, void* d_records) {
    if (!n) return 0;
    hipLaunchKernelGGL(k_accumulator_scale, dim3(n), dim3(64), 0, s, d_pairs, d_slots, d_scalar_words, (AccRecord*)d_records);
    H2V_HIP_CHECK(hipGetLastError());
    return 0;
}

#define MSM_ENTRY_HALF 0x40000000u
#define MSM_ENTRY_NEG 0x80000000u
#define MSM_ENTRY_TERM 0x3fffffffu

#define MSM_TILE 1024u
#define MSM_TILE_THREADS 256u
#define MSM_LDS_WORDS 16384u

template <bool SCATTER>
__global__ void __launch_bounds__(MSM_TILE_THREADS) msm_count_or_scatter(const MsmProblem* __restrict__ prs, uint32_t n_problems, uint32_t tiles_per_problem, MsmPlan p, uint32_t windows_per_pass, uint32_t* __restrict__ counts,
                                                                         const uint32_t* __restrict__ offsets, uint32_t* __restrict__ cursor, uint32_t* __restrict__ list) {
    extern __shared__ uint32_t hist[];
    const uint32_t tiles = tiles_per_problem, per_xcd = (n_problems + 7) / 8;
    const uint32_t q = (blockIdx.x % 8) * per_xcd + (blockIdx.x / 8) / tiles, tile0 = ((blockIdx.x / 8) % tiles) * MSM_TILE, tid = threadIdx.x;
    if (q >= n_problems) return;
    const MsmProblem pq = prs[q];
    const uint32_t n = pq.n;
    if (tile0 >= n) return;
    const uint32_t nbq = p.windows * p.buckets;
    const uint32_t half_range = 1u << (p.c - 1);
    constexpr uint32_t PER = MSM_TILE / MSM_TILE_THREADS;
    for (uint32_t w0 = 0; w0 < p.windows; w0 += windows_per_pass) {
        const uint32_t w1 = min(p.windows, w0 + windows_per_pass), nwords = (w1 - w0) * p.buckets;
        for (uint32_t i = tid; i < nwords; i += MSM_TILE_THREADS) hist[i] = 0;
        __syncthreads();
        for (int phase = 0; phase < (SCATTER ? 2 : 1); ++phase) {
            for (uint32_t k = 0; k < PER; ++k) {
                const uint32_t t = tile0 + tid + k * MSM_TILE_THREADS;
                if (t >= n) break;
                const uint32_t* s = t < pq.n1 ? pq.scalars + (size_t)pq.sstride * t : pq.scalars2 + (size_t)pq.sstride * (t - pq.n1);
                uint32_t nz = 0;
                for (int i = 0; i < 8; ++i) nz |= s[i];
                if (!nz) continue;
                const uint32_t* bw = reinterpret_cast<const uint32_t*>(t < pq.n1 ? pq.bases + (size_t)pq.bstride * t : pq.bases2 + (size_t)pq.bstride * (t - pq.n1));
                uint32_t any = 0;
                for (int i = 0; i < (int)(sizeof(G1A) / 4); ++i) any |= bw[i];
                if (!any) continue;
                GlvHalf h[2];
                glv_decompose(s, h[0], h[1]);
                for (uint32_t hf = 0; hf < 2; ++hf) {
                    uint32_t carry = 0;
                    for (uint32_t w = 0; w < w1; ++w) {
                        uint32_t raw = raw_window(h[hf].mag, w, p.c) + carry;
                        bool neg_digit = raw > half_range;
                        uint32_t mag = neg_digit ? (1u << p.c) - raw : raw;
                        carry = neg_digit ? 1u : 0u;
                        if (!mag || w < w0) continue;
                        uint32_t local = (w - w0) * p.buckets + mag - 1;
                        if (!SCATTER || phase == 0) atomicAdd(&hist[local], 1u);
                        else {
                            uint32_t b = q * nbq + w * p.buckets + mag - 1;
                            uint32_t pos = atomicAdd(&hist[local], 1u);
                            list[offsets[b] + pos] = t | (hf ? MSM_ENTRY_HALF : 0u) | ((neg_digit != h[hf].neg) ? MSM_ENTRY_NEG : 0u);
                        }
                    }
                }
            }
            __syncthreads();
            if (phase == 0) {
                for (uint32_t i = tid; i < nwords; i += MSM_TILE_THREADS) {
                    uint32_t v = hist[i];
                    if (!v) continue;
                    uint32_t b = q * nbq + w0 * p.buckets + i;
                    if (SCATTER) hist[i] = atomicAdd(&cursor[b], v);
                    else atomicAdd(&counts[b], v);
                }
                __syncthreads();
            }
        }
    }
}

__global__ void __launch_bounds__(256) msm_glv_prep(const MsmProblem* __restrict__ prs, uint32_t n_problems, MsmPlan p, uint32_t* __restrict__ dig, G1A* __restrict__ phi_pts) {
    const uint32_t q = blockIdx.y, t = blockIdx.x * blockDim.x + threadIdx.x;
    if (q >= n_problems) return;
    const MsmProblem pq = prs[q];
    if (t >= pq.n) return;
    uint32_t* out = dig + (size_t)pq.glv_off * p.windows + t;
    const uint32_t* sc = t < pq.n1 ? pq.scalars + (size_t)pq.sstride * t : pq.scalars2 + (size_t)pq.sstride * (t - pq.n1);
    uint32_t nz = 0;
    for (int i = 0; i < 8; ++i) nz |= sc[i];
    if (nz) {
        const uint32_t* bw = reinterpret_cast<const uint32_t*>(t < pq.n1 ? pq.bases + (size_t)pq.bstride * t : pq.bases2 + (size_t)pq.bstride * (t - pq.n1));
        uint32_t any = 0;
        for (int i = 0; i < (int)(sizeof(G1A) / 4); ++i) any |= bw[i];
        nz = any;
        if (any && !(t < pq.n1 ? pq.phi : pq.phi2)) phi_pts[(size_t)pq.glv_off + t] = g1_phi(*reinterpret_cast<const G1A*>(bw));
    }
    if (!nz) { for (uint32_t w = 0; w < p.windows; ++w) out[(size_t)w * pq.n] = 0; return; }
    GlvHalf h[2];
    glv_decompose(sc, h[0], h[1]);
    const uint32_t half_range = 1u << (p.c - 1);
    uint32_t carry[2] = {0, 0};
    for (uint32_t w = 0; w < p.windows; ++w) {
        uint32_t word = 0;
#pragma unroll
        for (uint32_t hf = 0; hf < 2; ++hf) {
            const uint32_t raw = raw_window(h[hf].mag, w, p.c) + carry[hf];
            const bool neg_digit = raw > half_range;
            const uint32_t mag = neg_digit ? (1u << p.c) - raw : raw;
            carry[hf] = neg_digit ? 1u : 0u;
            const uint32_t d16 = mag ? (mag | ((neg_digit != h[hf].neg) ? 0x8000u : 0u)) : 0u;
            word |= d16 << (16 * hf);
        }
        out[(size_t)w * pq.n] = word;
    }
}
__global__ void __launch_bounds__(MSM_SORT_THREADS) msm_sort_lds(const MsmProblem* __restrict__ prs, const uint32_t* __restrict__ dig, MsmPlan p, uint32_t stride,
                                                                 uint32_t* __restrict__ counts, uint32_t* __restrict__ offsets, uint32_t* __restrict__ list,
                                                                 uint32_t* __restrict__ seg_total) {
    extern __shared__ uint32_t sort_lds[];
    uint32_t* hist = sort_lds;
    uint32_t* part = sort_lds + p.buckets;
    unsigned short* rec = reinterpret_cast<unsigned short*>(part + MSM_SORT_THREADS);
    const uint32_t w = blockIdx.x, q = blockIdx.y, tid = threadIdx.x;
    const MsmProblem pq = prs[q];
    const uint32_t n = pq.n, seg = q * p.windows + w;
    const uint32_t* dw = dig + (size_t)pq.glv_off * p.windows + (size_t)w * n;
    for (uint32_t i = tid; i < p.buckets; i += MSM_SORT_THREADS) hist[i] = 0;
    __syncthreads();
    for (int pass = 0; pass < 2; ++pass) {
        for (uint32_t t = tid; t < n; t += MSM_SORT_THREADS) {
            const uint32_t word = dw[t];
#pragma unroll
            for (uint32_t hf = 0; hf < 2; ++hf) {
                const uint32_t d16 = (word >> (16 * hf)) & 0xffffu, mag = d16 & 0x7fffu;
                if (!mag) continue;
                const uint32_t pos = atomicAdd(&hist[mag - 1], 1u);
                if (pass == 1) rec[pos] = (unsigned short)(t | (hf ? 0x4000u : 0u) | (d16 & 0x8000u));
            }
        }
        __syncthreads();
        if (pass == 0) {
            const uint32_t per = (p.buckets + MSM_SORT_THREADS - 1) / MSM_SORT_THREADS, b0 = tid * per;
            uint32_t local = 0;
            for (uint32_t i = 0; i < per; ++i) if (b0 + i < p.buckets) local += hist[b0 + i];
            part[tid] = local;
            __syncthreads();
            for (uint32_t d = 1; d < MSM_SORT_THREADS; d <<= 1) {
                const uint32_t v = tid >= d ? part[tid - d] : 0;
                __syncthreads();
                part[tid] += v;
                __syncthreads();
            }
            uint32_t run = part[tid] - local;
            const size_t bin0 = (size_t)seg * p.buckets;
            for (uint32_t i = 0; i < per; ++i) if (b0 + i < p.buckets) {
                const uint32_t cnt = hist[b0 + i];
                counts[bin0 + b0 + i] = cnt; offsets[bin0 + b0 + i] = run;
                hist[b0 + i] = run;
                run += cnt;
            }
            if (tid == MSM_SORT_THREADS - 1) seg_total[seg] = part[tid];
            __syncthreads();
        }
    }
    const uint32_t total = part[MSM_SORT_THREADS - 1];
    uint32_t* dst = list + (size_t)seg * stride;
    for (uint32_t i = tid; i < total; i += MSM_SORT_THREADS) {
        const uint32_t r = rec[i];
        dst[i] = (r & 0x3fffu) | ((r & 0x4000u) ? MSM_ENTRY_HALF : 0u) | ((r & 0x8000u) ? MSM_ENTRY_NEG : 0u);
    }
}
__global__ void __launch_bounds__(1024) msm_seg_scan(const uint32_t* __restrict__ seg_total, uint32_t nseg, uint32_t* __restrict__ seg_start, uint32_t* __restrict__ control) {
    __shared__ uint32_t part[1024];
    __shared__ uint32_t carry;
    const uint32_t t = threadIdx.x;
    if (t == 0) carry = 0;
    __syncthreads();
    for (uint32_t base = 0; base < nseg; base += 1024) {
        const uint32_t i = base + t, c = i < nseg ? seg_total[i] : 0;
        part[t] = c;
        __syncthreads();
        for (uint32_t d = 1; d < 1024; d <<= 1) {
            const uint32_t v = t >= d ? part[t - d] : 0;
            __syncthreads();
            part[t] += v;
            __syncthreads();
        }
        if (i < nseg) seg_start[i] = carry + part[t] - c;
        __syncthreads();
        if (t == 1023) carry += part[1023];
        __syncthreads();
    }
    if (t == 0) { seg_start[nseg] = carry; control[0] = 0; control[1] = carry; control[2] = 0; control[3] = 0; control[4] = 0; }
}

__device__ __forceinline__ G1A msm_entry_load(const MsmProblem& q, uint32_t e, const G1A* __restrict__ phi_pts) {
    const uint32_t t = e & MSM_ENTRY_TERM;
    const bool first = t < q.n1;
    const size_t off = (size_t)(first ? t : t - q.n1) * q.bstride;
    const G1A* b = (first ? q.bases : q.bases2) + off;
    if (phi_pts && (e & MSM_ENTRY_HALF)) {
        const G1A* ph = first ? q.phi : q.phi2;
        b = ph ? ph + off : phi_pts + ((size_t)q.glv_off + t);
    }
    return *b;
}
__device__ __forceinline__ G1A msm_entry_apply(G1A b, uint32_t e, bool have_phi) {
    if (!have_phi && (e & MSM_ENTRY_HALF)) b.x = g1_beta_times(b.x);
    if ((e & MSM_ENTRY_NEG) && !b.y.is_zero()) b.y = Fq::lazy_neg(b.y);
    return b;
}
__device__ __forceinline__ G1A msm_entry_base(const MsmProblem& q, uint32_t e) { return msm_entry_apply(msm_entry_load(q, e, nullptr), e, false); }

__global__ void __launch_bounds__(1024) msm_block_sums(const uint32_t* __restrict__ counts, uint32_t* __restrict__ block_sums, uint32_t nb) {
    __shared__ uint32_t part[1024];
    const uint32_t t = threadIdx.x, i = blockIdx.x * 1024 + t;
    part[t] = i < nb ? counts[i] : 0;
    __syncthreads();
    for (uint32_t d = 512; d > 0; d >>= 1) { if (t < d) part[t] += part[t + d]; __syncthreads(); }
    if (t == 0) block_sums[blockIdx.x] = part[0];
}
__global__ void __launch_bounds__(1024) msm_scan_sums(uint32_t* __restrict__ block_sums, uint32_t nblk, uint32_t* __restrict__ total) {
    __shared__ uint32_t part[1024];
    __shared__ uint32_t carry;
    const uint32_t t = threadIdx.x;
    if (t == 0) carry = 0;
    __syncthreads();
    for (uint32_t base = 0; base < nblk; base += 1024) {
        const uint32_t i = base + t;
        const uint32_t c = i < nblk ? block_sums[i] : 0;
        part[t] = c;
        __syncthreads();
        for (uint32_t d = 1; d < 1024; d <<= 1) {
            uint32_t v = t >= d ? part[t - d] : 0;
            __syncthreads();
            part[t] += v;
            __syncthreads();
        }
        if (i < nblk) block_sums[i] = carry + part[t] - c;
        __syncthreads();
        if (t == 1023) carry += part[1023];
        __syncthreads();
    }
    if (t == 0) *total = carry;
}
__global__ void __launch_bounds__(1024) msm_offsets(const uint32_t* __restrict__ counts, const uint32_t* __restrict__ block_sums, uint32_t* __restrict__ offsets,
                                                    uint32_t* __restrict__ cursor, uint32_t nb) {
    __shared__ uint32_t part[1024];
    const uint32_t t = threadIdx.x, i = blockIdx.x * 1024 + t;
    const uint32_t c = i < nb ? counts[i] : 0;
    part[t] = c;
    __syncthreads();
    for (uint32_t d = 1; d < 1024; d <<= 1) {
        uint32_t v = t >= d ? part[t - d] : 0;
        __syncthreads();
        part[t] += v;
        __syncthreads();
    }
    if (i < nb) { offsets[i] = block_sums[blockIdx.x] + part[t] - c; cursor[i] = 0; }
}

struct MsmSeg { const uint32_t* seg_start; uint32_t nseg, bps, stride, lanes_round; };
__device__ __forceinline__ uint32_t msm_bin_start(const MsmSeg& g, const uint32_t* __restrict__ offsets, uint32_t b) { return g.seg_start[b / g.bps] + offsets[b]; }
__device__ __forceinline__ uint32_t msm_bin_of(const MsmSeg& g, const uint32_t* __restrict__ offsets, uint32_t pos) {
    uint32_t lo = 0, hi = g.nseg;
    while (hi - lo > 1) { uint32_t mid = (lo + hi) >> 1; if (g.seg_start[mid] <= pos) lo = mid; else hi = mid; }
    const uint32_t base = lo * g.bps, local = pos - g.seg_start[lo];
    lo = 0; hi = g.bps;
    while (hi - lo > 1) { uint32_t mid = (lo + hi) >> 1; if (offsets[base + mid] <= local) lo = mid; else hi = mid; }
    return base + lo;
}
__device__ __forceinline__ G1JSlot* msm_piece_dst(G1JSlot* __restrict__ bucket_pts, G1JSlot* __restrict__ partial, uint32_t lane, uint32_t b, uint32_t bin_lo, uint32_t bin_hi,
                                              uint32_t chunk_lo, uint32_t chunk_hi, bool first) {
    if (bin_lo >= chunk_lo && bin_hi <= chunk_hi) return bucket_pts + b;
    return partial + 2 * (size_t)lane + (first ? 0 : 1);
}
__device__ __noinline__ void msm_chunk_slow(const MsmProblem* __restrict__ prs, uint32_t nbq, const uint32_t* __restrict__ counts, const uint32_t* __restrict__ offsets,
                                            const uint32_t* __restrict__ list, G1JSlot* __restrict__ bucket_pts, G1JSlot* __restrict__ partial, uint32_t nb, uint32_t lane, uint32_t E, MsmSeg g) {
    const uint32_t CH = msm_chunk_len(E, g.lanes_round);
    const uint32_t chunk_lo = lane * CH, chunk_hi = min(chunk_lo + CH, E);
    uint32_t b = msm_bin_of(g, offsets, chunk_lo);
    uint32_t bin_lo = msm_bin_start(g, offsets, b), bin_hi = bin_lo + counts[b];
    MsmProblem q = prs[b / nbq];
    G1J acc = G1J::identity();
    bool first = true;
    for (uint32_t pos = chunk_lo; pos < chunk_hi;) {
        const uint32_t sg = b / g.bps;
        acc = g1_add_affine(acc, msm_entry_base(q, list[(size_t)sg * g.stride + (pos - g.seg_start[sg])]));
        ++pos;
        if (pos == bin_hi || pos == chunk_hi) {
            *msm_piece_dst(bucket_pts, partial, lane, b, bin_lo, bin_hi, chunk_lo, chunk_hi, first) = acc;
            acc = G1J::identity(); first = false;
            if (pos == bin_hi && pos < chunk_hi) {
                { uint32_t tries = 0; do { ++b; } while (counts[b] == 0 && ++tries < 2); if (counts[b] == 0) b = msm_bin_of(g, offsets, pos); }
                bin_lo = bin_hi; bin_hi = bin_lo + counts[b];
                q = prs[b / nbq];
            }
        }
    }
}
__device__ __forceinline__ void msm_chunk_tail(uint32_t b, uint32_t bin_lo, uint32_t bin_hi, uint32_t chunk_lo, uint32_t chunk_hi, uint32_t CH, uint32_t lane, uint32_t nb,
                                               uint32_t* __restrict__ control, uint32_t* __restrict__ lists) {
    if (bin_hi > chunk_hi && bin_lo >= chunk_lo) {
        const uint32_t span = (bin_hi - 1) / CH - lane;
        if (span >= MSM_FIXUP_SERIAL) lists[nb - 1 - atomicAdd(&control[0], 1u)] = b;
        else if (span >= MSM_FIXUP_TEAM) lists[nb + atomicAdd(&control[3], 1u)] = b;
        else lists[atomicAdd(&control[2], 1u)] = b;
    }
}
__device__ __forceinline__ void msm_accumulate_chunk(const MsmProblem* __restrict__ prs, uint32_t nbq, const uint32_t* __restrict__ counts, const uint32_t* __restrict__ offsets,
                                                     const uint32_t* __restrict__ list, G1JSlot* __restrict__ bucket_pts, G1JSlot* __restrict__ partial, uint32_t nb, const MsmSeg& g,
                                                     uint32_t* __restrict__ control, uint32_t* __restrict__ lists, const G1A* __restrict__ phi_pts, uint32_t* __restrict__ redo, uint32_t E, uint32_t CH,
                                                     uint32_t lane) {
    const uint32_t chunk_lo = lane * CH;
    if (chunk_lo >= E) return;
    const uint32_t chunk_hi = min(chunk_lo + CH, E);
    uint32_t b = msm_bin_of(g, offsets, chunk_lo);
    uint32_t sg = b / g.bps, seg_lo = g.seg_start[sg];
    uint32_t bin_lo = seg_lo + offsets[b], bin_hi = bin_lo + counts[b];
    uint32_t qi = b / nbq;
    MsmProblem q = prs[qi];
    G1J acc = G1J::identity();
    bool first = true, ok = true;
    uint32_t e_next = list[(size_t)sg * g.stride + (chunk_lo - seg_lo)];
    G1A raw_next = msm_entry_load(q, e_next, phi_pts);
    for (uint32_t pos = chunk_lo; pos < chunk_hi && ok;) {
        const uint32_t e = e_next;
        const G1A raw = raw_next;
        ++pos;
        const bool flush = pos == bin_hi || pos == chunk_hi;
        uint32_t b_next = b, lo_next = bin_lo, hi_next = bin_hi, qn = qi;
        MsmProblem q_next = q;
        if (pos == bin_hi && pos < chunk_hi) {
            uint32_t tries = 0;
            do { ++b_next; } while (counts[b_next] == 0 && ++tries < 2);
            if (counts[b_next] == 0) b_next = msm_bin_of(g, offsets, pos);
            lo_next = bin_hi; hi_next = lo_next + counts[b_next];
            const uint32_t sn = b_next / g.bps;
            if (sn != sg) { sg = sn; seg_lo = g.seg_start[sn]; }
            qn = b_next / nbq;
            if (qn != qi) q_next = prs[qn];
        }
        const uint32_t pos_n = min(pos, chunk_hi - 1);
        e_next = list[(size_t)sg * g.stride + (pos_n - seg_lo)]; raw_next = msm_entry_load(q_next, e_next, phi_pts);
        ok = g1_madd_fast(acc, msm_entry_apply(raw, e, phi_pts != nullptr));
        if (flush) {
            if (ok) *msm_piece_dst(bucket_pts, partial, lane, b, bin_lo, bin_hi, chunk_lo, chunk_hi, first) = acc;
            acc = G1J::identity(); first = false;
        }
        b = b_next; bin_lo = lo_next; bin_hi = hi_next; qi = qn; q = q_next;
    }
    if (!ok) { redo[atomicAdd(&control[4], 1u)] = lane; return; }
    msm_chunk_tail(b, bin_lo, bin_hi, chunk_lo, chunk_hi, CH, lane, nb, control, lists);
}
__global__ void __launch_bounds__(64) __attribute__((amdgpu_waves_per_eu(3, 3))) msm_accumulate(const MsmProblem* __restrict__ prs, uint32_t nbq, const uint32_t* __restrict__ counts, const uint32_t* __restrict__ offsets,
                                                     const uint32_t* __restrict__ list, G1JSlot* __restrict__ bucket_pts, G1JSlot* __restrict__ partial, uint32_t nb, MsmSeg g,
                                                     uint32_t* __restrict__ control, uint32_t* __restrict__ lists, const G1A* __restrict__ phi_pts, uint32_t* __restrict__ redo) {
    const uint32_t E = counts[nb + 1];
    const uint32_t CH = msm_chunk_len(E, g.lanes_round);
    const uint32_t blocks = ((E + CH - 1) / CH + 63) / 64, per_xcd = (blocks + 7) / 8;
    for (uint32_t j = blockIdx.x / 8; j < per_xcd; j += gridDim.x / 8)
        msm_accumulate_chunk(prs, nbq, counts, offsets, list, bucket_pts, partial, nb, g, control, lists, phi_pts, redo, E, CH, ((blockIdx.x % 8) * per_xcd + j) * 64 + threadIdx.x);
}
__global__ void __launch_bounds__(64) msm_accumulate_redo(const MsmProblem* __restrict__ prs, uint32_t nbq, const uint32_t* __restrict__ counts, const uint32_t* __restrict__ offsets,
                                                          const uint32_t* __restrict__ list, G1JSlot* __restrict__ bucket_pts, G1JSlot* __restrict__ partial, uint32_t nb, MsmSeg g,
                                                          uint32_t* __restrict__ control, uint32_t* __restrict__ lists, const uint32_t* __restrict__ redo) {
    const uint32_t n_redo = control[4], E = counts[nb + 1], CH = msm_chunk_len(E, g.lanes_round);
    for (uint32_t i = blockIdx.x * blockDim.x + threadIdx.x; i < n_redo; i += gridDim.x * blockDim.x) {
        const uint32_t lane = redo[i], chunk_lo = lane * CH, chunk_hi = min(chunk_lo + CH, E);
        msm_chunk_slow(prs, nbq, counts, offsets, list, bucket_pts, partial, nb, lane, E, g);
        const uint32_t b = msm_bin_of(g, offsets, chunk_hi - 1), bin_lo = msm_bin_start(g, offsets, b), bin_hi = bin_lo + counts[b];
        msm_chunk_tail(b, bin_lo, bin_hi, chunk_lo, chunk_hi, CH, lane, nb, control, lists);
    }
}

__device__ __forceinline__ const G1JSlot* msm_piece_src(const G1JSlot* __restrict__ partial, uint32_t i, uint32_t i0, uint32_t off, uint32_t CH) {
    return partial + 2 * (size_t)i + ((i == i0 && off > i0 * CH) ? 1 : 0);
}
__device__ __noinline__ void msm_fixup_slow(const G1JSlot* __restrict__ partial, uint32_t i0, uint32_t i1, uint32_t off, uint32_t CH, G1JSlot* __restrict__ out) {
    G1J acc = msm_piece_src(partial, i0, i0, off, CH)->p;
    for (uint32_t i = i0 + 1; i <= i1; ++i) acc = g1_add(acc, msm_piece_src(partial, i, i0, off, CH)->p);
    *out = acc;
}
__device__ __noinline__ void g1_add_to(G1J* dst, const G1J* a, const G1J* b);
__device__ __noinline__ void msm_fixup_team(const uint32_t* __restrict__ counts, const uint32_t* __restrict__ offsets, const G1JSlot* __restrict__ partial,
                                            const uint32_t* __restrict__ lists, G1JSlot* __restrict__ bucket_pts, uint32_t nb, const MsmSeg& g, G1J* team_acc) {
    const uint32_t n_team = counts[nb + 3], r = threadIdx.x & 7u;
    const uint32_t CH = msm_chunk_len(counts[nb + 1], g.lanes_round);
    for (uint32_t m0 = blockIdx.x * 8; m0 < n_team; m0 += MSM_FIXUP_TEAM_BLOCKS * 8) {
        const uint32_t m = m0 + (threadIdx.x >> 3);
        const bool live = m < n_team;
        const uint32_t b = live ? lists[nb + m] : 0;
        const uint32_t cnt = live ? counts[b] : 0, off = live ? msm_bin_start(g, offsets, b) : 0;
        const uint32_t i0 = off / CH, i1 = cnt ? (off + cnt - 1) / CH : i0;
        G1J* mine = team_acc + threadIdx.x;
        *mine = G1J::identity();
        if (live) for (uint32_t i = i0 + r; i <= i1; i += 8) g1_add_to(mine, mine, &msm_piece_src(partial, i, i0, off, CH)->p);
        for (uint32_t d = 4; d > 0; d >>= 1)
            g1_add_to(mine, mine, team_acc + min(threadIdx.x + d, 63u));
        if (live && r == 0) bucket_pts[b] = *mine;
    }
}
__device__ __noinline__ void msm_fixup_heavy(const uint32_t* __restrict__ counts, const uint32_t* __restrict__ offsets, const G1JSlot* __restrict__ partial,
                                             const uint32_t* __restrict__ lists, G1JSlot* __restrict__ bucket_pts, uint32_t nb, const MsmSeg& g, uint32_t first_block) {
    const uint32_t n_heavy = counts[nb], t = threadIdx.x;
    const uint32_t CH = msm_chunk_len(counts[nb + 1], g.lanes_round);
    for (uint32_t h = blockIdx.x - first_block; h < n_heavy; h += MSM_FIXUP_HEAVY_BLOCKS) {
        const uint32_t b = lists[nb - 1 - h];
        const uint32_t cnt = counts[b], off = msm_bin_start(g, offsets, b);
        const uint32_t i0 = off / CH, i1 = (off + cnt - 1) / CH;
        G1J acc = G1J::identity();
        for (uint32_t i = i0 + t; i <= i1; i += 64) acc = g1_add(acc, msm_piece_src(partial, i, i0, off, CH)->p);
        for (uint32_t d = 32; d > 0; d >>= 1) {
            G1J other;
            uint32_t* dst = reinterpret_cast<uint32_t*>(&other);
            const uint32_t* src = reinterpret_cast<const uint32_t*>(&acc);
#pragma unroll
            for (uint32_t k = 0; k < sizeof(G1J) / 4; ++k) dst[k] = (uint32_t)__shfl_down((int)src[k], d, 64);
            acc = g1_add(acc, other);
        }
        if (t == 0) bucket_pts[b] = acc;
    }
}
__global__ void __launch_bounds__(64) msm_fixup(const uint32_t* __restrict__ counts, const uint32_t* __restrict__ offsets, const G1JSlot* __restrict__ partial,
                                                const uint32_t* __restrict__ lists, G1JSlot* __restrict__ bucket_pts, uint32_t nb, MsmSeg g) {
    __shared__ G1J team_acc[64];
    if (blockIdx.x < MSM_FIXUP_TEAM_BLOCKS) { msm_fixup_team(counts, offsets, partial, lists, bucket_pts, nb, g, team_acc); return; }
    if (blockIdx.x < MSM_FIXUP_TEAM_BLOCKS + MSM_FIXUP_HEAVY_BLOCKS) { msm_fixup_heavy(counts, offsets, partial, lists, bucket_pts, nb, g, MSM_FIXUP_TEAM_BLOCKS); return; }
    const uint32_t k = (blockIdx.x - MSM_FIXUP_TEAM_BLOCKS - MSM_FIXUP_HEAVY_BLOCKS) * blockDim.x + threadIdx.x;
    if (k >= counts[nb + 2]) return;
    const uint32_t b = lists[k];
    const uint32_t cnt = counts[b], off = msm_bin_start(g, offsets, b);
    const uint32_t CH = msm_chunk_len(counts[nb + 1], g.lanes_round);
    const uint32_t i0 = off / CH, i1 = (off + cnt - 1) / CH;
    G1J acc = msm_piece_src(partial, i0, i0, off, CH)->p;
    bool ok = true;
    for (uint32_t i = i0 + 1; i <= i1 && ok; ++i) ok = g1_add_fast<false>(acc, msm_piece_src(partial, i, i0, off, CH)->p);
    if (!ok) { msm_fixup_slow(partial, i0, i1, off, CH, bucket_pts + b); return; }
    bucket_pts[b] = acc;
}
#define MSM_WIN_SLOTS 5
__device__ __noinline__ void g1_add_to(G1J* dst, const G1J* a, const G1J* b) { const G1J x = *a, y = *b; *dst = g1_add_inl(x, y); }
__device__ __noinline__ void g1_dbl_to(G1J* dst, const G1J* a) { const G1J x = *a; *dst = g1_dbl_inl(x); }

__global__ void __launch_bounds__(MSM_WIN_THREADS) msm_window(const G1JSlot* __restrict__ bucket_pts, const uint32_t* __restrict__ counts, G1JSlot* __restrict__ window_sums, MsmPlan p,
                                                              uint32_t n_windows, uint32_t wpw, uint32_t slots) {
    __builtin_amdgcn_s_setprio(3);
    extern __shared__ G1J win_lds[];
    const uint32_t T = blockDim.x / wpw, sub = threadIdx.x / T, t = threadIdx.x % T;
    const uint32_t widx = blockIdx.x * wpw + sub;
    const bool live = widx < n_windows;
    G1J* mine = win_lds + (size_t)sub * slots * T;
    G1J* run = mine + t;
    G1J* sum = mine + T + t;
    G1J* scaled = mine + 2 * T + t;
    G1J* red = mine + 2 * T;
    const uint32_t slice = (p.buckets + T - 1) / T;
    const uint32_t lo = live ? min(p.buckets, t * slice) : 0, hi = live ? min(p.buckets, lo + slice) : 0;
    *run = G1J::identity(); *sum = G1J::identity();
    const G1JSlot* bp = bucket_pts + (size_t)widx * p.buckets;
    const uint32_t* cn = counts + (size_t)widx * p.buckets;
    for (uint32_t b = hi; b > lo; --b) {
        if (cn[b - 1]) g1_add_to(run, run, &bp[b - 1].p);
        g1_add_to(sum, sum, run);
    }
    if ((slice & (slice - 1)) == 0 && T > 1 && slots >= MSM_WIN_SLOTS) {
        G1J* run2 = mine + 3 * T + t;
        G1J* run3 = mine + 4 * T + t;
        if (lo < hi && t > 0) {
            g1_dbl_to(run2, run);
            g1_add_to(run3, run2, run);
            *scaled = G1J::identity();
            const int nd = (32 - (int)__clz((int)(T - 1)) + 1) / 2;
            for (int d = nd - 1; d >= 0; --d) {
                if (d < nd - 1) { g1_dbl_to(scaled, scaled); g1_dbl_to(scaled, scaled); }
                const uint32_t dig = (t >> (2 * d)) & 3u;
                if (dig) g1_add_to(scaled, scaled, dig == 1 ? run : (dig == 2 ? run2 : run3));
            }
            for (uint32_t w = slice; w > 1; w >>= 1) g1_dbl_to(scaled, scaled);
            g1_add_to(sum, sum, scaled);
        }
    } else if (lo < hi && lo > 0) {
        const int top = 31 - (int)__clz((int)lo);
        *scaled = G1J::identity();
        for (int i = top; i >= 0; --i) {
            if (i < top) g1_dbl_to(scaled, scaled);
            if ((lo >> i) & 1) g1_add_to(scaled, scaled, run);
        }
        g1_add_to(sum, sum, scaled);
    }
    if (blockDim.x <= 64) {
        for (uint32_t d = 32; d > 0; d >>= 1) {
            const G1J mine_sum = *sum;
            G1J other;
            uint32_t* dst = reinterpret_cast<uint32_t*>(&other);
            const uint32_t* src = reinterpret_cast<const uint32_t*>(&mine_sum);
#pragma unroll
            for (uint32_t k = 0; k < sizeof(G1J) / 4; ++k) dst[k] = (uint32_t)__shfl_down((int)src[k], d, 64);
            if (t + d >= T) other = G1J::identity();
            *scaled = other;
            g1_add_to(sum, sum, scaled);
        }
        if (t == 0 && live) window_sums[widx] = *sum;
        return;
    }
    const uint32_t W = T < 64u ? T : 64u;
    for (uint32_t d = W / 2; d > 0; d >>= 1) {
        const G1J mine_sum = *sum;
        G1J other;
        uint32_t* dst = reinterpret_cast<uint32_t*>(&other);
        const uint32_t* src = reinterpret_cast<const uint32_t*>(&mine_sum);
#pragma unroll
        for (uint32_t k = 0; k < sizeof(G1J) / 4; ++k) dst[k] = (uint32_t)__shfl_down((int)src[k], d, 64);
        if ((t & (W - 1)) + d >= W) other = G1J::identity();
        *scaled = other;
        g1_add_to(sum, sum, scaled);
    }
    __syncthreads();
    if ((t & (W - 1)) == 0) red[t >> 6] = *sum;
    __syncthreads();
    if (t == 0) {
        for (uint32_t wv = 1; wv < (T >> 6); ++wv) g1_add_to(&red[0], &red[0], &red[wv]);
        if (live) window_sums[widx] = red[0];
    }
}

__global__ void __launch_bounds__(64) msm_final(const G1JSlot* __restrict__ window_sums, const MsmProblem* __restrict__ prs, uint32_t count, MsmPlan p) {
    __builtin_amdgcn_s_setprio(3);
    const uint32_t t = blockIdx.x * blockDim.x + threadIdx.x, q = t >> 2, r = t & 3u;
    if (q >= count) return;
    G1J acc = G1J::identity();
    if (prs[q].n) acc = msm_horner_quad(window_sums + (size_t)q * p.windows, p.windows, p.c, r);
    if (r == 0) *prs[q].out = acc;
}
__global__ void __launch_bounds__(64) msm_final_parts(const G1JSlot* __restrict__ window_sums, const MsmProblem* __restrict__ prs, uint32_t count, MsmPlan p,
                                                      uint32_t parts, uint32_t wpp, G1JSlot* __restrict__ out, G1JSlot* __restrict__ ready) {
    __builtin_amdgcn_s_setprio(3);
    const uint32_t t = blockIdx.x * blockDim.x + threadIdx.x, quad = t >> 2, r = t & 3u;
    if (quad >= count * parts) return;
    const uint32_t q = quad / parts, j = quad % parts, lo = j * wpp, hi = min(p.windows, lo + wpp);
    G1J acc = G1J::identity();
    if (prs[q].n && lo < hi) acc = msm_horner_quad(window_sums + (size_t)q * p.windows + lo, hi - lo, p.c, r);
    if (r == 0) out[quad] = acc;
    if (r == 0) { ready[quad].p.X = Fq::mul_chain(acc.X, acc.Z); ready[quad].p.Y = acc.Y; }
    if (r == 1) ready[quad].p.Z = Fq::mul_chain(acc.Z.sqr_chain(), acc.Z);
}
__global__ void __launch_bounds__(64) msm_combine_parts(const G1JSlot* __restrict__ pieces, const MsmProblem* __restrict__ prs, uint32_t count, uint32_t parts, uint32_t shift) {
    const uint32_t t = blockIdx.x * blockDim.x + threadIdx.x, q = t >> 2, r = t & 3u;
    if (q >= count) return;
    const G1J acc = msm_horner_quad(pieces + (size_t)q * parts, parts, shift, r);
    if (r == 0) *prs[q].out = acc;
}

__global__ void __launch_bounds__(64) msm_merge_windows(const G1JSlot* __restrict__ sub_sums, const MsmProblem* __restrict__ parents, uint32_t n_parents, uint32_t windows,
                                                        G1JSlot* __restrict__ merged) {
    const uint32_t team = (blockIdx.x * blockDim.x + threadIdx.x) >> 3, r = threadIdx.x & 7u;
    const bool live = team < n_parents * windows;
    const uint32_t q = live ? team / windows : 0, w = live ? team % windows : 0;
    const uint32_t first = parents[q].sub_first, cnt = live ? parents[q].sub_count : 0;
    G1J acc = G1J::identity();
    for (uint32_t k = r; k < cnt; k += 8) acc = g1_add(acc, sub_sums[(size_t)(first + k) * windows + w].p);
    for (uint32_t d = 4; d > 0; d >>= 1) {
        G1J other;
        uint32_t* dst = reinterpret_cast<uint32_t*>(&other);
        const uint32_t* src = reinterpret_cast<const uint32_t*>(&acc);
#pragma unroll
        for (uint32_t k = 0; k < sizeof(G1J) / 4; ++k) dst[k] = (uint32_t)__shfl_down((int)src[k], d, 8);
        acc = g1_add(acc, other);
    }
    if (live && r == 0) merged[(size_t)q * windows + w] = acc;
}

__global__ void msm_set_problems(MsmProblemChunk ch, uint32_t count, MsmProblem* __restrict__ dst) {
    uint32_t i = threadIdx.x;
    if (i < count) dst[i] = ch.p[i];
}

static MsmProblem msm_problem_slice(const MsmProblem& q, uint32_t first, uint32_t len) {
    MsmProblem r = q;
    r.out = nullptr; r.n = len; r.nnz = 0; r.sub_first = 0; r.sub_count = 0;
    if (first < q.n1) {
        r.scalars = q.scalars + (size_t)q.sstride * first; r.bases = q.bases + (size_t)q.bstride * first;
        if (q.phi) r.phi = q.phi + (size_t)q.bstride * first;
        r.n1 = std::min(q.n1 - first, len);
    } else {
        r.scalars = q.scalars2 + (size_t)q.sstride * (first - q.n1); r.bases = q.bases2 + (size_t)q.bstride * (first - q.n1);
        r.phi = q.phi2 ? q.phi2 + (size_t)q.bstride * (first - q.n1) : nullptr;
        r.n1 = len; r.scalars2 = nullptr; r.bases2 = nullptr; r.phi2 = nullptr;
    }
    return r;
}
static void msm_upload_problems(hipStream_t s, const std::vector<MsmProblem>& v, bool assign_glv, MsmProblem* dst) {
    uint32_t glv_next = 0;
    const uint32_t count = (uint32_t)v.size();
    for (uint32_t q0 = 0; q0 < count; q0 += MSM_PROBLEM_CHUNK) {
        MsmProblemChunk ch;
        uint32_t k = std::min<uint32_t>(MSM_PROBLEM_CHUNK, count - q0);
        for (uint32_t i = 0; i < k; ++i) { ch.p[i] = v[q0 + i]; if (assign_glv) { ch.p[i].glv_off = glv_next; glv_next += v[q0 + i].n; } }
        hipLaunchKernelGGL(msm_set_problems, dim3(1), dim3(64), 0, s, ch, k, dst + q0);
    }
}

struct MsmLaunchShape { std::vector<MsmProblem> launch_p, parents_p; bool cut = false; uint32_t nmax = 0; size_t total = 0, total_nz = 0; };
static int msm_shape(const MsmWorkspace& ws, const MsmProblems& pr, MsmLaunchShape& L) {
    const uint32_t n_callers = (uint32_t)pr.p.size();
    if (n_callers > MSM_MAX_PROBLEMS || n_callers > std::max(ws.cap_problems, ws.cap_parents)) { set_last_error("msm_enqueue_multi: too many problems"); return H2V_ERR_BAD_ARGUMENT; }
    for (uint32_t q = 0; q < n_callers; ++q) { L.nmax = std::max(L.nmax, pr.p[q].n); L.total += pr.p[q].n; L.total_nz += pr.p[q].nnz ? std::min(pr.p[q].nnz, pr.p[q].n) : pr.p[q].n; }
    if (L.nmax > MSM_LDS_SORT_MAX_TERMS && !ws.tune.msm_no_term_split) {
        size_t subs = 0;
        for (uint32_t q = 0; q < n_callers; ++q) subs += msm_subproblems(pr.p[q].n);
        L.cut = subs <= ws.cap_problems && subs <= MSM_MAX_PROBLEMS && n_callers <= ws.cap_parents;
    }
    if (L.cut) {
        for (uint32_t q = 0; q < n_callers; ++q) {
            const MsmProblem& c = pr.p[q];
            const uint32_t k = msm_subproblems(c.n), per = (c.n + k - 1) / k;
            MsmProblem parent = c;
            parent.sub_first = (uint32_t)L.launch_p.size(); parent.sub_count = k;
            for (uint32_t i = 0; i < k; ++i) { const uint32_t first = std::min(c.n, i * per); L.launch_p.push_back(msm_problem_slice(c, first, std::min(per, c.n - first))); }
            L.parents_p.push_back(parent);
        }
        L.nmax = 0;
        for (const MsmProblem& q : L.launch_p) L.nmax = std::max(L.nmax, q.n);
    } else {
        if (n_callers > ws.cap_problems) { set_last_error("msm_enqueue_multi: too many problems"); return H2V_ERR_BAD_ARGUMENT; }
        L.launch_p = pr.p;
    }
    return 0;
}
static bool msm_same_problems(const std::vector<MsmProblem>& a, const std::vector<MsmProblem>& b) {
    if (a.size() != b.size()) return false;
    for (size_t i = 0; i < a.size(); ++i) {
        const MsmProblem &x = a[i], &y = b[i];
        if (x.scalars != y.scalars || x.bases != y.bases || x.out != y.out || x.sstride != y.sstride || x.bstride != y.bstride || x.n != y.n || x.n1 != y.n1 ||
            x.scalars2 != y.scalars2 || x.bases2 != y.bases2 || x.phi != y.phi || x.phi2 != y.phi2 || x.nnz != y.nnz) return false;
    }
    return true;
}
int msm_enqueue_multi(hipStream_t s, MsmWorkspace& ws, const MsmProblems& pr, MsmSplit* split) {
    if (split) { split->parts = 0; split->shift = 0; split->count = 0; split->pts = nullptr; split->ready = nullptr; }
    const uint32_t n_callers = (uint32_t)pr.p.size();
    if (n_callers == 0) return 0;
    MsmLaunchShape L;
    { int rc = msm_shape(ws, pr, L); if (rc) return rc; }
    const bool cut = L.cut;
    uint32_t nmax = L.nmax; const size_t total = L.total, total_nz = L.total_nz;
    const std::vector<MsmProblem>& launch_p = L.launch_p;
    const bool uploaded = !ws.resident.empty() && ws.resident_no_split == ws.tune.msm_no_term_split && msm_same_problems(ws.resident, pr.p);
    if (!uploaded) {
        if (cut) msm_upload_problems(s, L.parents_p, false, ws.parents.p);
        msm_upload_problems(s, launch_p, true, ws.problems.p);
        ws.resident = pr.p; ws.resident_no_split = ws.tune.msm_no_term_split;
    }
    const uint32_t count = (uint32_t)launch_p.size();
    ws.final_problems = cut ? ws.parents.p : ws.problems.p;
    if (nmax == 0) {
        hipLaunchKernelGGL(msm_final, dim3((4 * count + 63) / 64), dim3(64), 0, s, ws.window_sums.p, ws.problems.p, count, MsmPlan{0, 2, 0, 3});
        H2V_HIP_CHECK(hipGetLastError());
        return 0;
    }
    if (nmax > MSM_ENTRY_TERM) { set_last_error("msm_enqueue_multi: more than 2^30 terms in one problem"); return H2V_ERR_BAD_ARGUMENT; }
    if (total > ws.cap_terms) { set_last_error("msm_enqueue_multi: terms exceed workspace capacity"); return H2V_ERR_BAD_ARGUMENT; }
    MsmPlan p = msm_plan(nmax, msm_latency_bound(total));
    uint32_t nbq = p.windows * p.buckets, nb = nbq * count;
    if (nb > ws.cap_buckets || total * 2 * p.windows > ws.cap_list) { set_last_error("msm_enqueue_multi: workspace too small"); return H2V_ERR_BAD_ARGUMENT; }
    const uint32_t stride = 2 * nmax;
    const size_t sort_lds = ((size_t)p.buckets + MSM_SORT_THREADS) * 4 + (size_t)stride * 2;
    const bool lds_sort = nmax <= MSM_LDS_SORT_MAX_TERMS && sort_lds <= 150 * 1024 && (size_t)count * p.windows * stride <= ws.cap_list &&
                          (size_t)count * p.windows <= (size_t)128 * ws.cap_problems && !ws.tune.msm_global_sort;
    MsmSeg g;
    if (lds_sort) {
        hipLaunchKernelGGL(msm_glv_prep, dim3((nmax + 255) / 256, count), dim3(256), 0, s, ws.problems.p, count, p, ws.glv.p, ws.phi_pts.p);
        if (sort_lds > 64 * 1024) H2V_HIP_CHECK(hipFuncSetAttribute((const void*)msm_sort_lds, hipFuncAttributeMaxDynamicSharedMemorySize, (int)sort_lds));
        hipLaunchKernelGGL(msm_sort_lds, dim3(p.windows, count), dim3(MSM_SORT_THREADS), sort_lds, s, ws.problems.p, ws.glv.p, p, stride, ws.counts.p, ws.offsets.p, ws.list.p, ws.seg_total.p);
        hipLaunchKernelGGL(msm_seg_scan, dim3(1), dim3(1024), 0, s, ws.seg_total.p, p.windows * count, ws.seg_start.p, ws.counts.p + nb);
        g = MsmSeg{ws.seg_start.p, p.windows * count, p.buckets, stride, MSM_ACC_LANES_PER_ROUND};
    } else {
    H2V_HIP_CHECK(hipMemsetAsync(ws.counts.p, 0, ((size_t)nb + MSM_CONTROL_WORDS) * 4, s));
    H2V_HIP_CHECK(hipMemsetAsync(ws.seg_start.p, 0, 4, s));
    const uint32_t tiles = (nmax + MSM_TILE - 1) / MSM_TILE;
    dim3 gt(8 * ((count + 7) / 8) * tiles);
    const uint32_t wpp = std::max<uint32_t>(1u, std::min<uint32_t>(p.windows, MSM_LDS_WORDS / p.buckets));
    const size_t lds = (size_t)wpp * p.buckets * 4;
    hipLaunchKernelGGL(msm_count_or_scatter<false>, gt, dim3(MSM_TILE_THREADS), lds, s, ws.problems.p, count, tiles, p, wpp, ws.counts.p, ws.offsets.p, ws.cursor.p, ws.list.p);
    const uint32_t nblk = (nb + 1023) / 1024;
    hipLaunchKernelGGL(msm_block_sums, dim3(nblk), dim3(1024), 0, s, ws.counts.p, ws.block_sums.p, nb);
    hipLaunchKernelGGL(msm_scan_sums, dim3(1), dim3(1024), 0, s, ws.block_sums.p, nblk, ws.counts.p + nb + 1);
    hipLaunchKernelGGL(msm_offsets, dim3(nblk), dim3(1024), 0, s, ws.counts.p, ws.block_sums.p, ws.offsets.p, ws.cursor.p, nb);
    hipLaunchKernelGGL(msm_count_or_scatter<true>, gt, dim3(MSM_TILE_THREADS), lds, s, ws.problems.p, count, tiles, p, wpp, ws.counts.p, ws.offsets.p, ws.cursor.p, ws.list.p);
    g = MsmSeg{ws.seg_start.p, 1, nb, 0, MSM_ACC_LANES_PER_ROUND};
    }
    const uint32_t acc_blocks = msm_accumulate_blocks(total_nz * 2 * p.windows, MSM_ACC_LANES_PER_ROUND);
    {
        const G1A* phi_tab = lds_sort ? (const G1A*)ws.phi_pts.p : (const G1A*)nullptr;
        if (ws.profile) {
            hipExtLaunchKernelGGL(msm_accumulate, dim3(acc_blocks), dim3(64), 0, s, ws.ev_acc[0], ws.ev_acc[1], 0, ws.problems.p, nbq, ws.counts.p, ws.offsets.p, ws.list.p, ws.bucket_pts.p, ws.partial.p, nb, g, ws.counts.p + nb, ws.cursor.p, phi_tab, ws.redo.p);
            ws.profile_recorded = true;
        } else hipLaunchKernelGGL(msm_accumulate, dim3(acc_blocks), dim3(64), 0, s, ws.problems.p, nbq, ws.counts.p, ws.offsets.p, ws.list.p, ws.bucket_pts.p, ws.partial.p, nb, g, ws.counts.p + nb, ws.cursor.p, phi_tab, ws.redo.p);
    }
    hipLaunchKernelGGL(msm_accumulate_redo, dim3(256), dim3(64), 0, s, ws.problems.p, nbq, ws.counts.p, ws.offsets.p, ws.list.p, ws.bucket_pts.p, ws.partial.p, nb, g, ws.counts.p + nb, ws.cursor.p, ws.redo.p);
    hipLaunchKernelGGL(msm_fixup, dim3((nb + 63) / 64 + MSM_FIXUP_TEAM_BLOCKS + MSM_FIXUP_HEAVY_BLOCKS), dim3(64), 0, s, ws.counts.p, ws.offsets.p, ws.partial.p, ws.cursor.p, ws.bucket_pts.p, nb, g);
    {
        const uint32_t nw = p.windows * count;
        uint32_t T = msm_window_threads(p.buckets, nw, ws.tune.msm_window_threads), wpw = 1;
        if (T == 64 && p.buckets >= 256 && nw > 256 && nw <= 512 && !ws.tune.msm_window_threads) { T = 128; wpw = 2; }
        const uint32_t wpw_forced = (uint32_t)ws.tune.msm_window_wpw;
        if ((wpw_forced == 1 || wpw_forced == 2 || wpw_forced == 4) && T * wpw_forced <= MSM_WIN_THREADS) wpw = wpw_forced;
        const uint32_t slots = ((T * wpw <= 64 && nw > 1024) || ws.tune.msm_window_slots == 3) ? 3u : (uint32_t)MSM_WIN_SLOTS;
        const size_t win_lds = (size_t)slots * T * wpw * sizeof(G1J);
        if (win_lds > 64 * 1024) H2V_HIP_CHECK(hipFuncSetAttribute((const void*)msm_window, hipFuncAttributeMaxDynamicSharedMemorySize, (int)win_lds));
        hipLaunchKernelGGL(msm_window, dim3((nw + wpw - 1) / wpw), dim3(T * wpw), win_lds, s, ws.bucket_pts.p, ws.counts.p, ws.window_sums.p, p, nw, wpw, slots);
    }
    const G1JSlot* sums = ws.window_sums.p;
    if (cut) {
        hipLaunchKernelGGL(msm_merge_windows, dim3((8 * n_callers * p.windows + 63) / 64), dim3(64), 0, s, ws.window_sums.p, ws.parents.p, n_callers, p.windows, ws.merged_sums.p);
        sums = ws.merged_sums.p;
    }
    if (split && split->want_parts > 1 && p.windows > 1) {
        const uint32_t want = std::min<uint32_t>(split->want_parts, MSM_MAX_PARTS);
        const uint32_t wpp = (p.windows + want - 1) / want, parts = (p.windows + wpp - 1) / wpp;
        hipLaunchKernelGGL(msm_final_parts, dim3((4 * n_callers * parts + 63) / 64), dim3(64), 0, s, sums, ws.final_problems, n_callers, p, parts, wpp, ws.pieces.p, ws.pieces.p + (size_t)MSM_MAX_PARTS * ws.cap_problems);
        split->parts = parts; split->shift = p.c * wpp; split->count = n_callers; split->pts = ws.pieces.p; split->ready = ws.pieces.p + (size_t)MSM_MAX_PARTS * ws.cap_problems;
    } else {
        hipLaunchKernelGGL(msm_final, dim3((4 * n_callers + 63) / 64), dim3(64), 0, s, sums, ws.final_problems, n_callers, p);
    }
    H2V_HIP_CHECK(hipGetLastError());
    return 0;
}
int msm_combine_enqueue(hipStream_t s, MsmWorkspace& ws, const MsmSplit& sp, size_t lds_reserve) {
    if (!sp.parts) return 0;
    if (lds_reserve > 64 * 1024) H2V_HIP_CHECK(hipFuncSetAttribute((const void*)msm_combine_parts, hipFuncAttributeMaxDynamicSharedMemorySize, (int)lds_reserve));
    hipLaunchKernelGGL(msm_combine_parts, dim3((4 * sp.count + 63) / 64), dim3(64), lds_reserve, s, sp.pts, ws.final_problems, sp.count, sp.parts, sp.shift);
    H2V_HIP_CHECK(hipGetLastError());
    return 0;
}

int msm_enqueue(hipStream_t s, MsmWorkspace& ws, const uint32_t* d_scalars, const G1A* d_bases, uint32_t n, G1J* d_out) {
    MsmProblems pr;
    pr.p.push_back(MsmProblem(d_scalars, d_bases, d_out, 8, 1, n));
    return msm_enqueue_multi(s, ws, pr);
}

}
```

Baseline: 11.85 million.

## Let left-channel MSM problems use a narrow per-problem window plan with variable segments

```diff
diff --git a/halo2_verifier_amd/csrc/batch.hip b/halo2_verifier_amd/csrc/batch.hip
--- a/halo2_verifier_amd/csrc/batch.hip
+++ b/halo2_verifier_amd/csrc/batch.hip
@@ -120,6 +120,7 @@
         pr.p.back().phi = b->phi.p + first;
         pr.p.back().nnz = count * (uint32_t)pl.left_term_order.size();
     }
+    pr.p.back().may_narrow = 1;
     pr.p.push_back(MsmProblem(b->msm_scal.p + first * 8, b->pts.p + first, acc2 + 1, 8, 1, terms.right - n_shared, shared_scal, b->pts.p + (size_t)b->n * np, n_shared));
     pr.p.back().phi = b->phi.p + first; pr.p.back().phi2 = b->phi.p + (size_t)b->n * np;
 }
diff --git a/halo2_verifier_amd/csrc/internal.h b/halo2_verifier_amd/csrc/internal.h
--- a/halo2_verifier_amd/csrc/internal.h
+++ b/halo2_verifier_amd/csrc/internal.h
@@ -5,6 +5,7 @@
 #include <vector>
 #include "../../include/h2v.h"
 #include "curve.hip.h"
+#include "msm_plan.h"
 
 namespace h2v {
 
@@ -57,12 +58,6 @@
 };
 
 
-struct MsmPlan {
-    uint32_t n;
-    uint32_t c;
-    uint32_t windows;
-    uint32_t buckets;
-};
 MsmPlan msm_plan(uint32_t n, bool latency = false);
 
 struct MsmProblem {
@@ -74,13 +69,15 @@
     uint32_t glv_off = 0;
     uint32_t sub_first = 0, sub_count = 0;
     uint32_t nnz = 0;
+    uint32_t may_narrow = 0;
+    uint32_t c = 0, windows = 0, seg_first = 0, dig_off = 0;
     MsmProblem() : scalars(nullptr), bases(nullptr), out(nullptr), sstride(8), bstride(1), n(0), n1(0), scalars2(nullptr), bases2(nullptr) {}
     MsmProblem(const uint32_t* s, const G1A* b, G1J* o, uint32_t ss, uint32_t bs, uint32_t n_) : scalars(s), bases(b), out(o), sstride(ss), bstride(bs), n(n_), n1(n_), scalars2(nullptr), bases2(nullptr) {}
     MsmProblem(const uint32_t* s, const G1A* b, G1J* o, uint32_t ss, uint32_t bs, uint32_t n1_, const uint32_t* s2, const G1A* b2, uint32_t n2)
         : scalars(s), bases(b), out(o), sstride(ss), bstride(bs), n(n1_ + n2), n1(n1_), scalars2(s2), bases2(b2) {}
 };
 #define MSM_MAX_PROBLEMS 1024
-#define MSM_PROBLEM_CHUNK 44
+#define MSM_PROBLEM_CHUNK 35
 struct MsmProblemChunk { MsmProblem p[MSM_PROBLEM_CHUNK]; };
 static_assert(sizeof(MsmProblemChunk) <= 4000, "a chunk of problem descriptors travels as one kernel argument (4 KB limit)");
 struct MsmProblems { std::vector<MsmProblem> p; };
@@ -92,7 +89,6 @@
     __host__ __device__ operator const G1J&() const { return p; }
 };
 
-#define MSM_MAX_PARTS 6
 struct MsmSplit {
     uint32_t want_parts = 0;
     uint32_t parts = 0, shift = 0, count = 0;
@@ -117,6 +113,7 @@
     DevBuf<G1JSlot> pieces;
     std::vector<MsmProblem> resident;
     int resident_no_split = 0;
+    int resident_lds = 0;
     DevBuf<MsmProblem> problems;
     DevBuf<MsmProblem> parents;
     DevBuf<G1JSlot> merged_sums;
@@ -128,6 +125,10 @@
     DevBuf<G1A> phi_pts;
     DevBuf<uint32_t> seg_total;
     DevBuf<uint32_t> seg_start;
+    DevBuf<MsmSegInfo> seg_info;
+    DevBuf<uint32_t> seg_order;
+    DevBuf<uint32_t> fix_start;
+    std::vector<MsmProblemShape> resident_shape;
     h2v_tuning tune = {};
     bool profile = false, profile_recorded = false;
     hipEvent_t ev_acc[2] = {nullptr, nullptr};
diff --git a/halo2_verifier_amd/csrc/msm.hip b/halo2_verifier_amd/csrc/msm.hip
--- a/halo2_verifier_amd/csrc/msm.hip
+++ b/halo2_verifier_amd/csrc/msm.hip
@@ -32,27 +32,8 @@
 #define MSM_FIXUP_HEAVY_BLOCKS 256u
 #define MSM_WIN_THREADS 256
 
-static inline uint32_t msm_window_threads(uint32_t buckets, uint32_t n_workgroups = 0xffffffffu, int forced = 0) {
-    if (buckets <= 64) return std::max(1u, buckets);
-    if (n_workgroups != 0xffffffffu && (forced == 64 || forced == 128 || forced == 256)) return (uint32_t)forced;
-    if (buckets > 2048 || (buckets >= 256 && n_workgroups <= 256)) return 256u;
-    return 64u;
-}
-
-MsmPlan msm_plan(uint32_t n, bool latency) {
-    MsmPlan best{n, 2, 65, 2};
-    double best_cost = 1e300;
-    for (uint32_t c = 2; c <= 15; ++c) {
-        uint32_t w = (130 + c - 1) / c;
-        uint32_t b = 1u << (c - 1);
-        uint32_t T = msm_window_threads(b), slice = (b + T - 1) / T;
-        double lg = 0; for (uint32_t t = T; t > 1; t >>= 1) lg += 1;
-        double cost = latency ? 9.0 * w + 9.0 * (2.0 * slice + 1.5 * c + 1.0 + lg) + 5.0 * std::min<double>(32.0, 2.0 * n)
-                              : (double)w * (11.0 * 2.0 * n + 16.0 * T * (2.0 * slice + 1.5 * c + 1.0 + lg));
-        if (cost < best_cost) { best_cost = cost; best = MsmPlan{n, c, w, b}; }
-    }
-    return best;
-}
+
+MsmPlan msm_plan(uint32_t n, bool latency) { return msm_plan_choose(n, latency); }
 static inline bool msm_latency_bound(size_t total_terms) { return total_terms <= 4096; }
 
 static inline uint32_t msm_subproblems(uint32_t n) { return n > MSM_LDS_SORT_MAX_TERMS ? (n + MSM_LDS_SORT_MAX_TERMS - 1) / MSM_LDS_SORT_MAX_TERMS : 1u; }
@@ -70,7 +51,7 @@
     if (covers(max_terms, max_problems, max_per_problem)) return 0;
     max_terms = std::max(max_terms, cap_terms); max_problems = std::max(max_problems, cap_parents); max_per_problem = std::max(max_per_problem, cap_per_problem);
     cap_terms = cap_parents = cap_per_problem = 0;
-    resident.clear(); final_problems = nullptr; profile_recorded = false;
+    resident.clear(); resident_shape.clear(); final_problems = nullptr; profile_recorded = false;
     const uint32_t subs = msm_subproblems(max_per_problem);
     cap_problems = (uint32_t)std::min<size_t>((size_t)max_problems * subs, MSM_MAX_PROBLEMS);
     if (cap_problems < max_problems) cap_problems = max_problems;
@@ -84,11 +65,16 @@
             for (uint32_t n = 1; n <= form_n[f]; n = n < 16 ? n + 1 : n + n / 8) { MsmPlan p = msm_plan(n, lat != 0); fb = std::max(fb, (size_t)p.windows * p.buckets); }
             MsmPlan p = msm_plan(form_n[f], lat != 0); fb = std::max(fb, (size_t)p.windows * p.buckets);
         }
+        if (f == 1) for (uint32_t n = 1;; n = n < 16 ? n + 1 : n + n / 8) {
+            if (n > form_n[f]) n = form_n[f];
+            const MsmNarrow nw = msm_plan_narrow(n); fb = std::max(fb, (size_t)nw.windows * nw.buckets);
+            if (n == form_n[f]) break;
+        }
         mb = std::max(mb, fb * form_q[f]);
         for (uint32_t n = 1;; n = n < 16 ? n + 1 : n + n / 8) {
             if (n > form_n[f]) n = form_n[f];
             size_t terms = n <= MSM_LDS_SORT_MAX_TERMS ? (size_t)n * form_q[f] : std::min<size_t>((size_t)max_terms, (size_t)n * form_q[f]);
-            cap_list = std::max(cap_list, terms * 2 * std::max(msm_plan(n, false).windows, msm_plan(n, true).windows));
+            cap_list = std::max(cap_list, terms * 2 * std::max(std::max(msm_plan(n, false).windows, msm_plan(n, true).windows), f == 1 ? msm_plan_narrow(n).windows : 0u));
             if (n == form_n[f]) break;
         }
     }
@@ -102,7 +88,8 @@
         (rc = problems.alloc(cap_problems)) || (rc = parents.alloc(max_problems)) || (rc = block_sums.alloc(mb / 1024 + 2)) ||
         (rc = partial.alloc(max_chunks * 2)) || (rc = redo.alloc(max_chunks)) ||
         (rc = glv.alloc(cap_list / 2 + 1)) ||
-        (rc = phi_pts.alloc((size_t)max_terms + 1)) || (rc = seg_total.alloc((size_t)128 * cap_problems + 2)) || (rc = seg_start.alloc((size_t)128 * cap_problems + 2))) {
+        (rc = phi_pts.alloc((size_t)max_terms + 1)) || (rc = seg_total.alloc((size_t)128 * cap_problems + 2)) || (rc = seg_start.alloc((size_t)128 * cap_problems + 2)) ||
+        (rc = seg_info.alloc((size_t)128 * cap_problems + 2)) || (rc = seg_order.alloc((size_t)128 * cap_problems + 2)) || (rc = fix_start.alloc(2 * mb))) {
         cap_problems = 0; cap_buckets = cap_list = 0;
         return rc;
     }
@@ -348,7 +335,8 @@
     if (q >= n_problems) return;
     const MsmProblem pq = prs[q];
     if (t >= pq.n) return;
-    uint32_t* out = dig + (size_t)pq.glv_off * p.windows + t;
+    const uint32_t c = pq.c ? pq.c : p.c, windows = pq.c ? pq.windows : p.windows;
+    uint32_t* out = dig + (pq.c ? (size_t)pq.dig_off : (size_t)pq.glv_off * p.windows) + t;
     const uint32_t* sc = t < pq.n1 ? pq.scalars + (size_t)pq.sstride * t : pq.scalars2 + (size_t)pq.sstride * (t - pq.n1);
     uint32_t nz = 0;
     for (int i = 0; i < 8; ++i) nz |= sc[i];
@@ -359,18 +347,18 @@
         nz = any;
         if (any && !(t < pq.n1 ? pq.phi : pq.phi2)) phi_pts[(size_t)pq.glv_off + t] = g1_phi(*reinterpret_cast<const G1A*>(bw));
     }
-    if (!nz) { for (uint32_t w = 0; w < p.windows; ++w) out[(size_t)w * pq.n] = 0; return; }
+    if (!nz) { for (uint32_t w = 0; w < windows; ++w) out[(size_t)w * pq.n] = 0; return; }
     GlvHalf h[2];
     glv_decompose(sc, h[0], h[1]);
-    const uint32_t half_range = 1u << (p.c - 1);
+    const uint32_t half_range = 1u << (c - 1);
     uint32_t carry[2] = {0, 0};
-    for (uint32_t w = 0; w < p.windows; ++w) {
+    for (uint32_t w = 0; w < windows; ++w) {
         uint32_t word = 0;
 #pragma unroll
         for (uint32_t hf = 0; hf < 2; ++hf) {
-            const uint32_t raw = raw_window(h[hf].mag, w, p.c) + carry[hf];
+            const uint32_t raw = raw_window(h[hf].mag, w, c) + carry[hf];
             const bool neg_digit = raw > half_range;
-            const uint32_t mag = neg_digit ? (1u << p.c) - raw : raw;
+            const uint32_t mag = neg_digit ? (1u << c) - raw : raw;
             carry[hf] = neg_digit ? 1u : 0u;
             const uint32_t d16 = mag ? (mag | ((neg_digit != h[hf].neg) ? 0x8000u : 0u)) : 0u;
             word |= d16 << (16 * hf);
@@ -378,18 +366,19 @@
         out[(size_t)w * pq.n] = word;
     }
 }
-__global__ void __launch_bounds__(MSM_SORT_THREADS) msm_sort_lds(const MsmProblem* __restrict__ prs, const uint32_t* __restrict__ dig, MsmPlan p, uint32_t stride,
+__global__ void __launch_bounds__(MSM_SORT_THREADS) msm_sort_lds(const MsmProblem* __restrict__ prs, const uint32_t* __restrict__ dig, const MsmSegInfo* __restrict__ info, uint32_t max_buckets,
                                                                  uint32_t* __restrict__ counts, uint32_t* __restrict__ offsets, uint32_t* __restrict__ list,
                                                                  uint32_t* __restrict__ seg_total) {
     extern __shared__ uint32_t sort_lds[];
     uint32_t* hist = sort_lds;
-    uint32_t* part = sort_lds + p.buckets;
+    uint32_t* part = sort_lds + max_buckets;
     unsigned short* rec = reinterpret_cast<unsigned short*>(part + MSM_SORT_THREADS);
-    const uint32_t w = blockIdx.x, q = blockIdx.y, tid = threadIdx.x;
-    const MsmProblem pq = prs[q];
-    const uint32_t n = pq.n, seg = q * p.windows + w;
-    const uint32_t* dw = dig + (size_t)pq.glv_off * p.windows + (size_t)w * n;
-    for (uint32_t i = tid; i < p.buckets; i += MSM_SORT_THREADS) hist[i] = 0;
+    const uint32_t seg = blockIdx.x, tid = threadIdx.x;
+    const MsmSegInfo si = info[seg];
+    const MsmProblem pq = prs[si.prob];
+    const uint32_t n = pq.n, w = seg - pq.seg_first, buckets = si.bins;
+    const uint32_t* dw = dig + (size_t)pq.dig_off + (size_t)w * n;
+    for (uint32_t i = tid; i < buckets; i += MSM_SORT_THREADS) hist[i] = 0;
     __syncthreads();
     for (int pass = 0; pass < 2; ++pass) {
         for (uint32_t t = tid; t < n; t += MSM_SORT_THREADS) {
@@ -404,9 +393,9 @@
         }
         __syncthreads();
         if (pass == 0) {
-            const uint32_t per = (p.buckets + MSM_SORT_THREADS - 1) / MSM_SORT_THREADS, b0 = tid * per;
+            const uint32_t per = (buckets + MSM_SORT_THREADS - 1) / MSM_SORT_THREADS, b0 = tid * per;
             uint32_t local = 0;
-            for (uint32_t i = 0; i < per; ++i) if (b0 + i < p.buckets) local += hist[b0 + i];
+            for (uint32_t i = 0; i < per; ++i) if (b0 + i < buckets) local += hist[b0 + i];
             part[tid] = local;
             __syncthreads();
             for (uint32_t d = 1; d < MSM_SORT_THREADS; d <<= 1) {
@@ -416,8 +405,8 @@
                 __syncthreads();
             }
             uint32_t run = part[tid] - local;
-            const size_t bin0 = (size_t)seg * p.buckets;
-            for (uint32_t i = 0; i < per; ++i) if (b0 + i < p.buckets) {
+            const size_t bin0 = si.bin0;
+            for (uint32_t i = 0; i < per; ++i) if (b0 + i < buckets) {
                 const uint32_t cnt = hist[b0 + i];
                 counts[bin0 + b0 + i] = cnt; offsets[bin0 + b0 + i] = run;
                 hist[b0 + i] = run;
@@ -428,7 +417,7 @@
         }
     }
     const uint32_t total = part[MSM_SORT_THREADS - 1];
-    uint32_t* dst = list + (size_t)seg * stride;
+    uint32_t* dst = list + si.list0;
     for (uint32_t i = tid; i < total; i += MSM_SORT_THREADS) {
         const uint32_t r = rec[i];
         dst[i] = (r & 0x3fffu) | ((r & 0x4000u) ? MSM_ENTRY_HALF : 0u) | ((r & 0x8000u) ? MSM_ENTRY_NEG : 0u);
@@ -524,69 +513,74 @@
     if (i < nb) { offsets[i] = block_sums[blockIdx.x] + part[t] - c; cursor[i] = 0; }
 }
 
-struct MsmSeg { const uint32_t* seg_start; uint32_t nseg, bps, stride, lanes_round; };
-__device__ __forceinline__ uint32_t msm_bin_start(const MsmSeg& g, const uint32_t* __restrict__ offsets, uint32_t b) { return g.seg_start[b / g.bps] + offsets[b]; }
-__device__ __forceinline__ uint32_t msm_bin_of(const MsmSeg& g, const uint32_t* __restrict__ offsets, uint32_t pos) {
+struct MsmSeg { const uint32_t* seg_start; const MsmSegInfo* info; uint32_t nseg, nbq, lanes_round; };
+__device__ __forceinline__ uint32_t msm_bin_of(const MsmSeg& g, const uint32_t* __restrict__ offsets, uint32_t pos, uint32_t& sg) {
     uint32_t lo = 0, hi = g.nseg;
     while (hi - lo > 1) { uint32_t mid = (lo + hi) >> 1; if (g.seg_start[mid] <= pos) lo = mid; else hi = mid; }
-    const uint32_t base = lo * g.bps, local = pos - g.seg_start[lo];
-    lo = 0; hi = g.bps;
+    sg = lo;
+    const uint32_t base = g.info[lo].bin0, local = pos - g.seg_start[lo];
+    hi = g.info[lo].bins; lo = 0;
     while (hi - lo > 1) { uint32_t mid = (lo + hi) >> 1; if (offsets[base + mid] <= local) lo = mid; else hi = mid; }
     return base + lo;
 }
+__device__ __forceinline__ uint32_t msm_bin_problem(const MsmSeg& g, uint32_t b, uint32_t sg) { return g.nbq ? b / g.nbq : g.info[sg].prob; }
 __device__ __forceinline__ G1JSlot* msm_piece_dst(G1JSlot* __restrict__ bucket_pts, G1JSlot* __restrict__ partial, uint32_t lane, uint32_t b, uint32_t bin_lo, uint32_t bin_hi,
                                               uint32_t chunk_lo, uint32_t chunk_hi, bool first) {
     if (bin_lo >= chunk_lo && bin_hi <= chunk_hi) return bucket_pts + b;
     return partial + 2 * (size_t)lane + (first ? 0 : 1);
 }
-__device__ __noinline__ void msm_chunk_slow(const MsmProblem* __restrict__ prs, uint32_t nbq, const uint32_t* __restrict__ counts, const uint32_t* __restrict__ offsets,
+__device__ __noinline__ void msm_chunk_slow(const MsmProblem* __restrict__ prs, const uint32_t* __restrict__ counts, const uint32_t* __restrict__ offsets,
                                             const uint32_t* __restrict__ list, G1JSlot* __restrict__ bucket_pts, G1JSlot* __restrict__ partial, uint32_t nb, uint32_t lane, uint32_t E, MsmSeg g) {
     const uint32_t CH = msm_chunk_len(E, g.lanes_round);
     const uint32_t chunk_lo = lane * CH, chunk_hi = min(chunk_lo + CH, E);
-    uint32_t b = msm_bin_of(g, offsets, chunk_lo);
-    uint32_t bin_lo = msm_bin_start(g, offsets, b), bin_hi = bin_lo + counts[b];
-    MsmProblem q = prs[b / nbq];
+    uint32_t sg;
+    uint32_t b = msm_bin_of(g, offsets, chunk_lo, sg);
+    uint32_t bin_lo = g.seg_start[sg] + offsets[b], bin_hi = bin_lo + counts[b];
+    MsmProblem q = prs[msm_bin_problem(g, b, sg)];
     G1J acc = G1J::identity();
     bool first = true;
     for (uint32_t pos = chunk_lo; pos < chunk_hi;) {
-        const uint32_t sg = b / g.bps;
-        acc = g1_add_affine(acc, msm_entry_base(q, list[(size_t)sg * g.stride + (pos - g.seg_start[sg])]));
+        acc = g1_add_affine(acc, msm_entry_base(q, list[(size_t)g.info[sg].list0 + (pos - g.seg_start[sg])]));
         ++pos;
         if (pos == bin_hi || pos == chunk_hi) {
             *msm_piece_dst(bucket_pts, partial, lane, b, bin_lo, bin_hi, chunk_lo, chunk_hi, first) = acc;
             acc = G1J::identity(); first = false;
             if (pos == bin_hi && pos < chunk_hi) {
-                { uint32_t tries = 0; do { ++b; } while (counts[b] == 0 && ++tries < 2); if (counts[b] == 0) b = msm_bin_of(g, offsets, pos); }
+                b = msm_bin_of(g, offsets, pos, sg);
                 bin_lo = bin_hi; bin_hi = bin_lo + counts[b];
-                q = prs[b / nbq];
+                q = prs[msm_bin_problem(g, b, sg)];
             }
         }
     }
 }
 __device__ __forceinline__ void msm_chunk_tail(uint32_t b, uint32_t bin_lo, uint32_t bin_hi, uint32_t chunk_lo, uint32_t chunk_hi, uint32_t CH, uint32_t lane, uint32_t nb,
-                                               uint32_t* __restrict__ control, uint32_t* __restrict__ lists) {
+                                               uint32_t* __restrict__ control, uint32_t* __restrict__ lists, uint32_t* __restrict__ starts) {
     if (bin_hi > chunk_hi && bin_lo >= chunk_lo) {
         const uint32_t span = (bin_hi - 1) / CH - lane;
-        if (span >= MSM_FIXUP_SERIAL) lists[nb - 1 - atomicAdd(&control[0], 1u)] = b;
-        else if (span >= MSM_FIXUP_TEAM) lists[nb + atomicAdd(&control[3], 1u)] = b;
-        else lists[atomicAdd(&control[2], 1u)] = b;
-    }
-}
-__device__ __forceinline__ void msm_accumulate_chunk(const MsmProblem* __restrict__ prs, uint32_t nbq, const uint32_t* __restrict__ counts, const uint32_t* __restrict__ offsets,
+        uint32_t at;
+        if (span >= MSM_FIXUP_SERIAL) at = nb - 1 - atomicAdd(&control[0], 1u);
+        else if (span >= MSM_FIXUP_TEAM) at = nb + atomicAdd(&control[3], 1u);
+        else at = atomicAdd(&control[2], 1u);
+        lists[at] = b; starts[at] = bin_lo;
+    }
+}
+__device__ __forceinline__ void msm_accumulate_chunk(const MsmProblem* __restrict__ prs, const uint32_t* __restrict__ counts, const uint32_t* __restrict__ offsets,
                                                      const uint32_t* __restrict__ list, G1JSlot* __restrict__ bucket_pts, G1JSlot* __restrict__ partial, uint32_t nb, const MsmSeg& g,
-                                                     uint32_t* __restrict__ control, uint32_t* __restrict__ lists, const G1A* __restrict__ phi_pts, uint32_t* __restrict__ redo, uint32_t E, uint32_t CH,
+                                                     uint32_t* __restrict__ control, uint32_t* __restrict__ lists, uint32_t* __restrict__ starts, const G1A* __restrict__ phi_pts, uint32_t* __restrict__ redo, uint32_t E, uint32_t CH,
                                                      uint32_t lane) {
     const uint32_t chunk_lo = lane * CH;
     if (chunk_lo >= E) return;
     const uint32_t chunk_hi = min(chunk_lo + CH, E);
-    uint32_t b = msm_bin_of(g, offsets, chunk_lo);
-    uint32_t sg = b / g.bps, seg_lo = g.seg_start[sg];
-    uint32_t bin_lo = seg_lo + offsets[b], bin_hi = bin_lo + counts[b];
-    uint32_t qi = b / nbq;
+    uint32_t sg;
+    uint32_t b = msm_bin_of(g, offsets, chunk_lo, sg);
+    uint32_t seg_end, list_rel, bin_lo;
+    { const MsmSegInfo si = g.info[sg]; const uint32_t seg_lo = g.seg_start[sg]; seg_end = si.bin0 + si.bins; list_rel = si.list0 - seg_lo; bin_lo = seg_lo + offsets[b]; }
+    uint32_t bin_hi = bin_lo + counts[b];
+    uint32_t qi = msm_bin_problem(g, b, sg);
     MsmProblem q = prs[qi];
     G1J acc = G1J::identity();
     bool first = true, ok = true;
-    uint32_t e_next = list[(size_t)sg * g.stride + (chunk_lo - seg_lo)];
+    uint32_t e_next = list[(uint32_t)(list_rel + chunk_lo)];
     G1A raw_next = msm_entry_load(q, e_next, phi_pts);
     for (uint32_t pos = chunk_lo; pos < chunk_hi && ok;) {
         const uint32_t e = e_next;
@@ -598,15 +592,16 @@
         if (pos == bin_hi && pos < chunk_hi) {
             uint32_t tries = 0;
             do { ++b_next; } while (counts[b_next] == 0 && ++tries < 2);
-            if (counts[b_next] == 0) b_next = msm_bin_of(g, offsets, pos);
+            uint32_t sn = sg;
+            if (counts[b_next] == 0) b_next = msm_bin_of(g, offsets, pos, sn);
+            else if (b_next >= seg_end) ++sn;
             lo_next = bin_hi; hi_next = lo_next + counts[b_next];
-            const uint32_t sn = b_next / g.bps;
-            if (sn != sg) { sg = sn; seg_lo = g.seg_start[sn]; }
-            qn = b_next / nbq;
+            if (sn != sg) { sg = sn; const MsmSegInfo si = g.info[sn]; seg_end = si.bin0 + si.bins; list_rel = si.list0 - g.seg_start[sn]; qn = si.prob; }
+            if (g.nbq) qn = b_next / g.nbq;
             if (qn != qi) q_next = prs[qn];
         }
         const uint32_t pos_n = min(pos, chunk_hi - 1);
-        e_next = list[(size_t)sg * g.stride + (pos_n - seg_lo)]; raw_next = msm_entry_load(q_next, e_next, phi_pts);
+        e_next = list[(uint32_t)(list_rel + pos_n)]; raw_next = msm_entry_load(q_next, e_next, phi_pts);
         ok = g1_madd_fast(acc, msm_entry_apply(raw, e, phi_pts != nullptr));
         if (flush) {
             if (ok) *msm_piece_dst(bucket_pts, partial, lane, b, bin_lo, bin_hi, chunk_lo, chunk_hi, first) = acc;
@@ -615,26 +610,27 @@
         b = b_next; bin_lo = lo_next; bin_hi = hi_next; qi = qn; q = q_next;
     }
     if (!ok) { redo[atomicAdd(&control[4], 1u)] = lane; return; }
-    msm_chunk_tail(b, bin_lo, bin_hi, chunk_lo, chunk_hi, CH, lane, nb, control, lists);
-}
-__global__ void __launch_bounds__(64) __attribute__((amdgpu_waves_per_eu(3, 3))) msm_accumulate(const MsmProblem* __restrict__ prs, uint32_t nbq, const uint32_t* __restrict__ counts, const uint32_t* __restrict__ offsets,
+    msm_chunk_tail(b, bin_lo, bin_hi, chunk_lo, chunk_hi, CH, lane, nb, control, lists, starts);
+}
+__global__ void __launch_bounds__(64) __attribute__((amdgpu_waves_per_eu(3, 3))) msm_accumulate(const MsmProblem* __restrict__ prs, const uint32_t* __restrict__ counts, const uint32_t* __restrict__ offsets,
                                                      const uint32_t* __restrict__ list, G1JSlot* __restrict__ bucket_pts, G1JSlot* __restrict__ partial, uint32_t nb, MsmSeg g,
-                                                     uint32_t* __restrict__ control, uint32_t* __restrict__ lists, const G1A* __restrict__ phi_pts, uint32_t* __restrict__ redo) {
+                                                     uint32_t* __restrict__ control, uint32_t* __restrict__ lists, uint32_t* __restrict__ starts, const G1A* __restrict__ phi_pts, uint32_t* __restrict__ redo) {
     const uint32_t E = counts[nb + 1];
     const uint32_t CH = msm_chunk_len(E, g.lanes_round);
     const uint32_t blocks = ((E + CH - 1) / CH + 63) / 64, per_xcd = (blocks + 7) / 8;
     for (uint32_t j = blockIdx.x / 8; j < per_xcd; j += gridDim.x / 8)
-        msm_accumulate_chunk(prs, nbq, counts, offsets, list, bucket_pts, partial, nb, g, control, lists, phi_pts, redo, E, CH, ((blockIdx.x % 8) * per_xcd + j) * 64 + threadIdx.x);
-}
-__global__ void __launch_bounds__(64) msm_accumulate_redo(const MsmProblem* __restrict__ prs, uint32_t nbq, const uint32_t* __restrict__ counts, const uint32_t* __restrict__ offsets,
+        msm_accumulate_chunk(prs, counts, offsets, list, bucket_pts, partial, nb, g, control, lists, starts, phi_pts, redo, E, CH, ((blockIdx.x % 8) * per_xcd + j) * 64 + threadIdx.x);
+}
+__global__ void __launch_bounds__(64) msm_accumulate_redo(const MsmProblem* __restrict__ prs, const uint32_t* __restrict__ counts, const uint32_t* __restrict__ offsets,
                                                           const uint32_t* __restrict__ list, G1JSlot* __restrict__ bucket_pts, G1JSlot* __restrict__ partial, uint32_t nb, MsmSeg g,
-                                                          uint32_t* __restrict__ control, uint32_t* __restrict__ lists, const uint32_t* __restrict__ redo) {
+                                                          uint32_t* __restrict__ control, uint32_t* __restrict__ lists, uint32_t* __restrict__ starts, const uint32_t* __restrict__ redo) {
     const uint32_t n_redo = control[4], E = counts[nb + 1], CH = msm_chunk_len(E, g.lanes_round);
     for (uint32_t i = blockIdx.x * blockDim.x + threadIdx.x; i < n_redo; i += gridDim.x * blockDim.x) {
         const uint32_t lane = redo[i], chunk_lo = lane * CH, chunk_hi = min(chunk_lo + CH, E);
-        msm_chunk_slow(prs, nbq, counts, offsets, list, bucket_pts, partial, nb, lane, E, g);
-        const uint32_t b = msm_bin_of(g, offsets, chunk_hi - 1), bin_lo = msm_bin_start(g, offsets, b), bin_hi = bin_lo + counts[b];
-        msm_chunk_tail(b, bin_lo, bin_hi, chunk_lo, chunk_hi, CH, lane, nb, control, lists);
+        msm_chunk_slow(prs, counts, offsets, list, bucket_pts, partial, nb, lane, E, g);
+        uint32_t sg;
+        const uint32_t b = msm_bin_of(g, offsets, chunk_hi - 1, sg), bin_lo = g.seg_start[sg] + offsets[b], bin_hi = bin_lo + counts[b];
+        msm_chunk_tail(b, bin_lo, bin_hi, chunk_lo, chunk_hi, CH, lane, nb, control, lists, starts);
     }
 }
 
@@ -647,7 +643,7 @@
     *out = acc;
 }
 __device__ __noinline__ void g1_add_to(G1J* dst, const G1J* a, const G1J* b);
-__device__ __noinline__ void msm_fixup_team(const uint32_t* __restrict__ counts, const uint32_t* __restrict__ offsets, const G1JSlot* __restrict__ partial,
+__device__ __noinline__ void msm_fixup_team(const uint32_t* __restrict__ counts, const uint32_t* __restrict__ starts, const G1JSlot* __restrict__ partial,
                                             const uint32_t* __restrict__ lists, G1JSlot* __restrict__ bucket_pts, uint32_t nb, const MsmSeg& g, G1J* team_acc) {
     const uint32_t n_team = counts[nb + 3], r = threadIdx.x & 7u;
     const uint32_t CH = msm_chunk_len(counts[nb + 1], g.lanes_round);
@@ -655,7 +651,7 @@
         const uint32_t m = m0 + (threadIdx.x >> 3);
         const bool live = m < n_team;
         const uint32_t b = live ? lists[nb + m] : 0;
-        const uint32_t cnt = live ? counts[b] : 0, off = live ? msm_bin_start(g, offsets, b) : 0;
+        const uint32_t cnt = live ? counts[b] : 0, off = live ? starts[nb + m] : 0;
         const uint32_t i0 = off / CH, i1 = cnt ? (off + cnt - 1) / CH : i0;
         G1J* mine = team_acc + threadIdx.x;
         *mine = G1J::identity();
@@ -665,13 +661,13 @@
         if (live && r == 0) bucket_pts[b] = *mine;
     }
 }
-__device__ __noinline__ void msm_fixup_heavy(const uint32_t* __restrict__ counts, const uint32_t* __restrict__ offsets, const G1JSlot* __restrict__ partial,
+__device__ __noinline__ void msm_fixup_heavy(const uint32_t* __restrict__ counts, const uint32_t* __restrict__ starts, const G1JSlot* __restrict__ partial,
                                              const uint32_t* __restrict__ lists, G1JSlot* __restrict__ bucket_pts, uint32_t nb, const MsmSeg& g, uint32_t first_block) {
     const uint32_t n_heavy = counts[nb], t = threadIdx.x;
     const uint32_t CH = msm_chunk_len(counts[nb + 1], g.lanes_round);
     for (uint32_t h = blockIdx.x - first_block; h < n_heavy; h += MSM_FIXUP_HEAVY_BLOCKS) {
         const uint32_t b = lists[nb - 1 - h];
-        const uint32_t cnt = counts[b], off = msm_bin_start(g, offsets, b);
+        const uint32_t cnt = counts[b], off = starts[nb - 1 - h];
         const uint32_t i0 = off / CH, i1 = (off + cnt - 1) / CH;
         G1J acc = G1J::identity();
         for (uint32_t i = i0 + t; i <= i1; i += 64) acc = g1_add(acc, msm_piece_src(partial, i, i0, off, CH)->p);
@@ -686,15 +682,15 @@
         if (t == 0) bucket_pts[b] = acc;
     }
 }
-__global__ void __launch_bounds__(64) msm_fixup(const uint32_t* __restrict__ counts, const uint32_t* __restrict__ offsets, const G1JSlot* __restrict__ partial,
+__global__ void __launch_bounds__(64) msm_fixup(const uint32_t* __restrict__ counts, const uint32_t* __restrict__ starts, const G1JSlot* __restrict__ partial,
                                                 const uint32_t* __restrict__ lists, G1JSlot* __restrict__ bucket_pts, uint32_t nb, MsmSeg g) {
     __shared__ G1J team_acc[64];
-    if (blockIdx.x < MSM_FIXUP_TEAM_BLOCKS) { msm_fixup_team(counts, offsets, partial, lists, bucket_pts, nb, g, team_acc); return; }
-    if (blockIdx.x < MSM_FIXUP_TEAM_BLOCKS + MSM_FIXUP_HEAVY_BLOCKS) { msm_fixup_heavy(counts, offsets, partial, lists, bucket_pts, nb, g, MSM_FIXUP_TEAM_BLOCKS); return; }
+    if (blockIdx.x < MSM_FIXUP_TEAM_BLOCKS) { msm_fixup_team(counts, starts, partial, lists, bucket_pts, nb, g, team_acc); return; }
+    if (blockIdx.x < MSM_FIXUP_TEAM_BLOCKS + MSM_FIXUP_HEAVY_BLOCKS) { msm_fixup_heavy(counts, starts, partial, lists, bucket_pts, nb, g, MSM_FIXUP_TEAM_BLOCKS); return; }
     const uint32_t k = (blockIdx.x - MSM_FIXUP_TEAM_BLOCKS - MSM_FIXUP_HEAVY_BLOCKS) * blockDim.x + threadIdx.x;
     if (k >= counts[nb + 2]) return;
     const uint32_t b = lists[k];
-    const uint32_t cnt = counts[b], off = msm_bin_start(g, offsets, b);
+    const uint32_t cnt = counts[b], off = starts[k];
     const uint32_t CH = msm_chunk_len(counts[nb + 1], g.lanes_round);
     const uint32_t i0 = off / CH, i1 = (off + cnt - 1) / CH;
     G1J acc = msm_piece_src(partial, i0, i0, off, CH)->p;
@@ -708,12 +704,13 @@
 __device__ __noinline__ void g1_dbl_to(G1J* dst, const G1J* a) { const G1J x = *a; *dst = g1_dbl_inl(x); }
 
 __global__ void __launch_bounds__(MSM_WIN_THREADS) msm_window(const G1JSlot* __restrict__ bucket_pts, const uint32_t* __restrict__ counts, G1JSlot* __restrict__ window_sums, MsmPlan p,
-                                                              uint32_t n_windows, uint32_t wpw, uint32_t slots) {
+                                                              uint32_t n_windows, uint32_t wpw, uint32_t slots, const MsmSegInfo* __restrict__ info, const uint32_t* __restrict__ order) {
     __builtin_amdgcn_s_setprio(3);
     extern __shared__ G1J win_lds[];
     const uint32_t T = blockDim.x / wpw, sub = threadIdx.x / T, t = threadIdx.x % T;
-    const uint32_t widx = blockIdx.x * wpw + sub;
-    const bool live = widx < n_windows;
+    const uint32_t wcls = blockIdx.x * wpw + sub;
+    const bool live = wcls < n_windows;
+    const uint32_t widx = order ? order[live ? wcls : 0] : wcls;
     G1J* mine = win_lds + (size_t)sub * slots * T;
     G1J* run = mine + t;
     G1J* sum = mine + T + t;
@@ -722,8 +719,9 @@
     const uint32_t slice = (p.buckets + T - 1) / T;
     const uint32_t lo = live ? min(p.buckets, t * slice) : 0, hi = live ? min(p.buckets, lo + slice) : 0;
     *run = G1J::identity(); *sum = G1J::identity();
-    const G1JSlot* bp = bucket_pts + (size_t)widx * p.buckets;
-    const uint32_t* cn = counts + (size_t)widx * p.buckets;
+    const size_t bin0 = order ? (size_t)info[widx].bin0 : (size_t)widx * p.buckets;
+    const G1JSlot* bp = bucket_pts + bin0;
+    const uint32_t* cn = counts + bin0;
     for (uint32_t b = hi; b > lo; --b) {
         if (cn[b - 1]) g1_add_to(run, run, &bp[b - 1].p);
         g1_add_to(sum, sum, run);
@@ -754,7 +752,7 @@
         g1_add_to(sum, sum, scaled);
     }
     if (blockDim.x <= 64) {
-        for (uint32_t d = 32; d > 0; d >>= 1) {
+        for (uint32_t d = (T < 64u ? T : 64u) / 2; d > 0; d >>= 1) {
             const G1J mine_sum = *sum;
             G1J other;
             uint32_t* dst = reinterpret_cast<uint32_t*>(&other);
@@ -789,22 +787,36 @@
     }
 }
 
-__global__ void __launch_bounds__(64) msm_final(const G1JSlot* __restrict__ window_sums, const MsmProblem* __restrict__ prs, uint32_t count, MsmPlan p) {
+__global__ void __launch_bounds__(64) msm_final(const G1JSlot* __restrict__ window_sums, const MsmProblem* __restrict__ prs, uint32_t count, MsmPlan p, uint32_t own) {
     __builtin_amdgcn_s_setprio(3);
     const uint32_t t = blockIdx.x * blockDim.x + threadIdx.x, q = t >> 2, r = t & 3u;
     if (q >= count) return;
     G1J acc = G1J::identity();
-    if (prs[q].n) acc = msm_horner_quad(window_sums + (size_t)q * p.windows, p.windows, p.c, r);
+    if (prs[q].n) {
+        if (own) acc = msm_horner_quad(window_sums + prs[q].seg_first, prs[q].windows, prs[q].c, r);
+        else acc = msm_horner_quad(window_sums + (size_t)q * p.windows, p.windows, p.c, r);
+    }
     if (r == 0) *prs[q].out = acc;
 }
 __global__ void __launch_bounds__(64) msm_final_parts(const G1JSlot* __restrict__ window_sums, const MsmProblem* __restrict__ prs, uint32_t count, MsmPlan p,
-                                                      uint32_t parts, uint32_t wpp, G1JSlot* __restrict__ out, G1JSlot* __restrict__ ready) {
+                                                      uint32_t parts, uint32_t wpp, G1JSlot* __restrict__ out, G1JSlot* __restrict__ ready, uint32_t own) {
     __builtin_amdgcn_s_setprio(3);
     const uint32_t t = blockIdx.x * blockDim.x + threadIdx.x, quad = t >> 2, r = t & 3u;
     if (quad >= count * parts) return;
-    const uint32_t q = quad / parts, j = quad % parts, lo = j * wpp, hi = min(p.windows, lo + wpp);
+    const uint32_t q = quad / parts, j = quad % parts;
     G1J acc = G1J::identity();
-    if (prs[q].n && lo < hi) acc = msm_horner_quad(window_sums + (size_t)q * p.windows + lo, hi - lo, p.c, r);
+    if (own) {
+        const uint32_t cq = prs[q].c, wq = prs[q].windows, shift = p.c * wpp;
+        const uint32_t lo = min(wq, msm_piece_first(cq, shift, j)), hi = min(wq, msm_piece_first(cq, shift, j + 1));
+        if (prs[q].n && lo < hi) {
+            acc = msm_horner_quad(window_sums + prs[q].seg_first + lo, hi - lo, cq, r);
+#pragma unroll 1
+            for (uint32_t i = lo * cq - shift * j; i > 0; --i) g1_dbl_quad(acc, r);
+        }
+    } else {
+        const uint32_t lo = j * wpp, hi = min(p.windows, lo + wpp);
+        if (prs[q].n && lo < hi) acc = msm_horner_quad(window_sums + (size_t)q * p.windows + lo, hi - lo, p.c, r);
+    }
     if (r == 0) out[quad] = acc;
     if (r == 0) { ready[quad].p.X = Fq::mul_chain(acc.X, acc.Z); ready[quad].p.Y = acc.Y; }
     if (r == 1) ready[quad].p.Z = Fq::mul_chain(acc.Z.sqr_chain(), acc.Z);
@@ -854,14 +866,41 @@
     }
     return r;
 }
-static void msm_upload_problems(hipStream_t s, const std::vector<MsmProblem>& v, bool assign_glv, MsmProblem* dst) {
+static void msm_upload_problems(hipStream_t s, const std::vector<MsmProblem>& v, const MsmLayout* shape, MsmProblem* dst) {
     uint32_t glv_next = 0;
     const uint32_t count = (uint32_t)v.size();
     for (uint32_t q0 = 0; q0 < count; q0 += MSM_PROBLEM_CHUNK) {
         MsmProblemChunk ch;
         uint32_t k = std::min<uint32_t>(MSM_PROBLEM_CHUNK, count - q0);
-        for (uint32_t i = 0; i < k; ++i) { ch.p[i] = v[q0 + i]; if (assign_glv) { ch.p[i].glv_off = glv_next; glv_next += v[q0 + i].n; } }
+        for (uint32_t i = 0; i < k; ++i) {
+            ch.p[i] = v[q0 + i];
+            if (shape) {
+                const MsmProblemShape& ps = shape->prob[q0 + i];
+                ch.p[i].glv_off = glv_next; glv_next += v[q0 + i].n;
+                ch.p[i].c = ps.c; ch.p[i].windows = ps.windows; ch.p[i].seg_first = ps.seg_first; ch.p[i].dig_off = ps.dig_off;
+            }
+        }
         hipLaunchKernelGGL(msm_set_problems, dim3(1), dim3(64), 0, s, ch, k, dst + q0);
+    }
+}
+#define MSM_SEG_CHUNK 240
+struct MsmSegChunk { MsmSegInfo s[MSM_SEG_CHUNK]; };
+struct MsmOrderChunk { uint32_t s[4 * MSM_SEG_CHUNK]; };
+static_assert(sizeof(MsmSegChunk) <= 4000 && sizeof(MsmOrderChunk) <= 4000, "a chunk of a segment table travels as one kernel argument (4 KB limit)");
+__global__ void __launch_bounds__(256) msm_set_segs(MsmSegChunk ch, uint32_t count, MsmSegInfo* __restrict__ dst) { if (threadIdx.x < count) dst[threadIdx.x] = ch.s[threadIdx.x]; }
+__global__ void __launch_bounds__(256) msm_set_order(MsmOrderChunk ch, uint32_t count, uint32_t* __restrict__ dst) { for (uint32_t i = threadIdx.x; i < count; i += 256) dst[i] = ch.s[i]; }
+static void msm_upload_layout(hipStream_t s, const MsmLayout& L, MsmSegInfo* seg_dst, uint32_t* order_dst) {
+    for (size_t i0 = 0; i0 < L.seg.size(); i0 += MSM_SEG_CHUNK) {
+        MsmSegChunk ch;
+        const uint32_t k = (uint32_t)std::min<size_t>(MSM_SEG_CHUNK, L.seg.size() - i0);
+        for (uint32_t i = 0; i < k; ++i) ch.s[i] = L.seg[i0 + i];
+        hipLaunchKernelGGL(msm_set_segs, dim3(1), dim3(256), 0, s, ch, k, seg_dst + i0);
+    }
+    for (size_t i0 = 0; i0 < L.order.size(); i0 += 4 * MSM_SEG_CHUNK) {
+        MsmOrderChunk ch;
+        const uint32_t k = (uint32_t)std::min<size_t>(4 * MSM_SEG_CHUNK, L.order.size() - i0);
+        for (uint32_t i = 0; i < k; ++i) ch.s[i] = L.order[i0 + i];
+        hipLaunchKernelGGL(msm_set_order, dim3(1), dim3(256), 0, s, ch, k, order_dst + i0);
     }
 }
 
@@ -897,7 +936,7 @@
     for (size_t i = 0; i < a.size(); ++i) {
         const MsmProblem &x = a[i], &y = b[i];
         if (x.scalars != y.scalars || x.bases != y.bases || x.out != y.out || x.sstride != y.sstride || x.bstride != y.bstride || x.n != y.n || x.n1 != y.n1 ||
-            x.scalars2 != y.scalars2 || x.bases2 != y.bases2 || x.phi != y.phi || x.phi2 != y.phi2 || x.nnz != y.nnz) return false;
+            x.scalars2 != y.scalars2 || x.bases2 != y.bases2 || x.phi != y.phi || x.phi2 != y.phi2 || x.nnz != y.nnz || x.may_narrow != y.may_narrow) return false;
     }
     return true;
 }
@@ -910,83 +949,119 @@
     const bool cut = L.cut;
     uint32_t nmax = L.nmax; const size_t total = L.total, total_nz = L.total_nz;
     const std::vector<MsmProblem>& launch_p = L.launch_p;
-    const bool uploaded = !ws.resident.empty() && ws.resident_no_split == ws.tune.msm_no_term_split && msm_same_problems(ws.resident, pr.p);
+    const uint32_t count = (uint32_t)launch_p.size();
+    if (nmax > MSM_ENTRY_TERM) { set_last_error("msm_enqueue_multi: more than 2^30 terms in one problem"); return H2V_ERR_BAD_ARGUMENT; }
+    if (total > ws.cap_terms) { set_last_error("msm_enqueue_multi: terms exceed workspace capacity"); return H2V_ERR_BAD_ARGUMENT; }
+    const bool latency = msm_latency_bound(total);
+    MsmPlan p = nmax ? msm_plan(nmax, latency) : MsmPlan{0, 2, 0, 3};
+    uint32_t nbq = p.windows * p.buckets;
+    if (nmax && ((size_t)nbq * count > ws.cap_buckets || total * 2 * p.windows > ws.cap_list)) { set_last_error("msm_enqueue_multi: workspace too small"); return H2V_ERR_BAD_ARGUMENT; }
+    uint32_t parts = 0, wpp = 0, shift = 0;
+    if (split) msm_split_shape(p, split->want_parts, parts, wpp, shift);
+    const uint32_t stride = 2 * nmax;
+    const size_t sort_lds_wide = ((size_t)p.buckets + MSM_SORT_THREADS) * 4 + (size_t)stride * 2;
+    const bool lds_sort = nmax <= MSM_LDS_SORT_MAX_TERMS && sort_lds_wide <= 150 * 1024 && (size_t)count * p.windows * stride <= ws.cap_list &&
+                          (size_t)count * p.windows <= (size_t)128 * ws.cap_problems && !ws.tune.msm_global_sort;
+    std::vector<uint32_t> terms(count);
+    std::vector<uint8_t> narrow(count, 0);
+    MsmNarrow nw;
+    for (uint32_t q = 0; q < count; ++q) terms[q] = launch_p[q].n;
+    if (nmax && lds_sort && !cut && !latency) {
+        uint32_t n_marked = 0;
+        for (uint32_t q = 0; q < count; ++q) if (launch_p[q].may_narrow) n_marked = std::max(n_marked, launch_p[q].n);
+        if (n_marked) nw = msm_plan_narrow(n_marked);
+        bool any = false;
+        for (uint32_t q = 0; q < count; ++q) if (launch_p[q].may_narrow && msm_take_narrow(launch_p[q].n, nw, p, parts, shift)) { narrow[q] = 1; any = true; }
+        if (any) {
+            const MsmLayout t = msm_layout(terms.data(), narrow.data(), count, p, nmax, nw, true);
+            if (t.nb > ws.cap_buckets || t.list_words > ws.cap_list || t.list_words >= ((size_t)1 << 32) || t.dig_words > ws.glv.cap || t.seg.size() > (size_t)128 * ws.cap_problems)
+                std::fill(narrow.begin(), narrow.end(), (uint8_t)0);
+        }
+    }
+    const MsmLayout lay = msm_layout(terms.data(), narrow.data(), count, p, nmax, nw, lds_sort);
+    const uint32_t nb = lay.nb;
+    const bool uploaded = !ws.resident.empty() && ws.resident_no_split == ws.tune.msm_no_term_split && msm_same_problems(ws.resident, pr.p) && ws.resident_shape == lay.prob &&
+                          ws.resident_lds == (lds_sort ? 1 : 0);
     if (!uploaded) {
-        if (cut) msm_upload_problems(s, L.parents_p, false, ws.parents.p);
-        msm_upload_problems(s, launch_p, true, ws.problems.p);
-        ws.resident = pr.p; ws.resident_no_split = ws.tune.msm_no_term_split;
-    }
-    const uint32_t count = (uint32_t)launch_p.size();
+        if (cut) msm_upload_problems(s, L.parents_p, nullptr, ws.parents.p);
+        msm_upload_problems(s, launch_p, &lay, ws.problems.p);
+        if (nmax) msm_upload_layout(s, lay, ws.seg_info.p, ws.seg_order.p);
+        ws.resident = pr.p; ws.resident_no_split = ws.tune.msm_no_term_split; ws.resident_shape = lay.prob; ws.resident_lds = lds_sort ? 1 : 0;
+    }
     ws.final_problems = cut ? ws.parents.p : ws.problems.p;
     if (nmax == 0) {
-        hipLaunchKernelGGL(msm_final, dim3((4 * count + 63) / 64), dim3(64), 0, s, ws.window_sums.p, ws.problems.p, count, MsmPlan{0, 2, 0, 3});
+        hipLaunchKernelGGL(msm_final, dim3((4 * count + 63) / 64), dim3(64), 0, s, ws.window_sums.p, ws.problems.p, count, p, 0u);
         H2V_HIP_CHECK(hipGetLastError());
         return 0;
     }
-    if (nmax > MSM_ENTRY_TERM) { set_last_error("msm_enqueue_multi: more than 2^30 terms in one problem"); return H2V_ERR_BAD_ARGUMENT; }
-    if (total > ws.cap_terms) { set_last_error("msm_enqueue_multi: terms exceed workspace capacity"); return H2V_ERR_BAD_ARGUMENT; }
-    MsmPlan p = msm_plan(nmax, msm_latency_bound(total));
-    uint32_t nbq = p.windows * p.buckets, nb = nbq * count;
-    if (nb > ws.cap_buckets || total * 2 * p.windows > ws.cap_list) { set_last_error("msm_enqueue_multi: workspace too small"); return H2V_ERR_BAD_ARGUMENT; }
-    const uint32_t stride = 2 * nmax;
-    const size_t sort_lds = ((size_t)p.buckets + MSM_SORT_THREADS) * 4 + (size_t)stride * 2;
-    const bool lds_sort = nmax <= MSM_LDS_SORT_MAX_TERMS && sort_lds <= 150 * 1024 && (size_t)count * p.windows * stride <= ws.cap_list &&
-                          (size_t)count * p.windows <= (size_t)128 * ws.cap_problems && !ws.tune.msm_global_sort;
     MsmSeg g;
     if (lds_sort) {
+        const size_t sort_lds = ((size_t)lay.max_buckets + MSM_SORT_THREADS) * 4 + (size_t)stride * 2;
         hipLaunchKernelGGL(msm_glv_prep, dim3((nmax + 255) / 256, count), dim3(256), 0, s, ws.problems.p, count, p, ws.glv.p, ws.phi_pts.p);
         if (sort_lds > 64 * 1024) H2V_HIP_CHECK(hipFuncSetAttribute((const void*)msm_sort_lds, hipFuncAttributeMaxDynamicSharedMemorySize, (int)sort_lds));
-        hipLaunchKernelGGL(msm_sort_lds, dim3(p.windows, count), dim3(MSM_SORT_THREADS), sort_lds, s, ws.problems.p, ws.glv.p, p, stride, ws.counts.p, ws.offsets.p, ws.list.p, ws.seg_total.p);
-        hipLaunchKernelGGL(msm_seg_scan, dim3(1), dim3(1024), 0, s, ws.seg_total.p, p.windows * count, ws.seg_start.p, ws.counts.p + nb);
-        g = MsmSeg{ws.seg_start.p, p.windows * count, p.buckets, stride, MSM_ACC_LANES_PER_ROUND};
+        const uint32_t nseg = (uint32_t)lay.seg.size();
+        hipLaunchKernelGGL(msm_sort_lds, dim3(nseg), dim3(MSM_SORT_THREADS), sort_lds, s, ws.problems.p, ws.glv.p, ws.seg_info.p, lay.max_buckets, ws.counts.p, ws.offsets.p, ws.list.p, ws.seg_total.p);
+        hipLaunchKernelGGL(msm_seg_scan, dim3(1), dim3(1024), 0, s, ws.seg_total.p, nseg, ws.seg_start.p, ws.counts.p + nb);
+        g = MsmSeg{ws.seg_start.p, ws.seg_info.p, nseg, 0u, MSM_ACC_LANES_PER_ROUND};
     } else {
     H2V_HIP_CHECK(hipMemsetAsync(ws.counts.p, 0, ((size_t)nb + MSM_CONTROL_WORDS) * 4, s));
     H2V_HIP_CHECK(hipMemsetAsync(ws.seg_start.p, 0, 4, s));
     const uint32_t tiles = (nmax + MSM_TILE - 1) / MSM_TILE;
     dim3 gt(8 * ((count + 7) / 8) * tiles);
-    const uint32_t wpp = std::max<uint32_t>(1u, std::min<uint32_t>(p.windows, MSM_LDS_WORDS / p.buckets));
-    const size_t lds = (size_t)wpp * p.buckets * 4;
-    hipLaunchKernelGGL(msm_count_or_scatter<false>, gt, dim3(MSM_TILE_THREADS), lds, s, ws.problems.p, count, tiles, p, wpp, ws.counts.p, ws.offsets.p, ws.cursor.p, ws.list.p);
+    const uint32_t wpp_sort = std::max<uint32_t>(1u, std::min<uint32_t>(p.windows, MSM_LDS_WORDS / p.buckets));
+    const size_t lds = (size_t)wpp_sort * p.buckets * 4;
+    hipLaunchKernelGGL(msm_count_or_scatter<false>, gt, dim3(MSM_TILE_THREADS), lds, s, ws.problems.p, count, tiles, p, wpp_sort, ws.counts.p, ws.offsets.p, ws.cursor.p, ws.list.p);
     const uint32_t nblk = (nb + 1023) / 1024;
     hipLaunchKernelGGL(msm_block_sums, dim3(nblk), dim3(1024), 0, s, ws.counts.p, ws.block_sums.p, nb);
     hipLaunchKernelGGL(msm_scan_sums, dim3(1), dim3(1024), 0, s, ws.block_sums.p, nblk, ws.counts.p + nb + 1);
     hipLaunchKernelGGL(msm_offsets, dim3(nblk), dim3(1024), 0, s, ws.counts.p, ws.block_sums.p, ws.offsets.p, ws.cursor.p, nb);
-    hipLaunchKernelGGL(msm_count_or_scatter<true>, gt, dim3(MSM_TILE_THREADS), lds, s, ws.problems.p, count, tiles, p, wpp, ws.counts.p, ws.offsets.p, ws.cursor.p, ws.list.p);
-    g = MsmSeg{ws.seg_start.p, 1, nb, 0, MSM_ACC_LANES_PER_ROUND};
-    }
-    const uint32_t acc_blocks = msm_accumulate_blocks(total_nz * 2 * p.windows, MSM_ACC_LANES_PER_ROUND);
+    hipLaunchKernelGGL(msm_count_or_scatter<true>, gt, dim3(MSM_TILE_THREADS), lds, s, ws.problems.p, count, tiles, p, wpp_sort, ws.counts.p, ws.offsets.p, ws.cursor.p, ws.list.p);
+    g = MsmSeg{ws.seg_start.p, ws.seg_info.p, 1u, nbq, MSM_ACC_LANES_PER_ROUND};
+    }
+    size_t max_entries = 0;
+    if (lay.n_narrow) for (uint32_t q = 0; q < count; ++q) max_entries += (size_t)2 * lay.prob[q].windows * (launch_p[q].nnz ? std::min(launch_p[q].nnz, launch_p[q].n) : launch_p[q].n);
+    else max_entries = total_nz * 2 * p.windows;
+    const uint32_t acc_blocks = msm_accumulate_blocks(max_entries, MSM_ACC_LANES_PER_ROUND);
     {
         const G1A* phi_tab = lds_sort ? (const G1A*)ws.phi_pts.p : (const G1A*)nullptr;
         if (ws.profile) {
-            hipExtLaunchKernelGGL(msm_accumulate, dim3(acc_blocks), dim3(64), 0, s, ws.ev_acc[0], ws.ev_acc[1], 0, ws.problems.p, nbq, ws.counts.p, ws.offsets.p, ws.list.p, ws.bucket_pts.p, ws.partial.p, nb, g, ws.counts.p + nb, ws.cursor.p, phi_tab, ws.redo.p);
+            hipExtLaunchKernelGGL(msm_accumulate, dim3(acc_blocks), dim3(64), 0, s, ws.ev_acc[0], ws.ev_acc[1], 0, ws.problems.p, ws.counts.p, ws.offsets.p, ws.list.p, ws.bucket_pts.p, ws.partial.p, nb, g, ws.counts.p + nb, ws.cursor.p, ws.fix_start.p, phi_tab, ws.redo.p);
             ws.profile_recorded = true;
-        } else hipLaunchKernelGGL(msm_accumulate, dim3(acc_blocks), dim3(64), 0, s, ws.problems.p, nbq, ws.counts.p, ws.offsets.p, ws.list.p, ws.bucket_pts.p, ws.partial.p, nb, g, ws.counts.p + nb, ws.cursor.p, phi_tab, ws.redo.p);
-    }
-    hipLaunchKernelGGL(msm_accumulate_redo, dim3(256), dim3(64), 0, s, ws.problems.p, nbq, ws.counts.p, ws.offsets.p, ws.list.p, ws.bucket_pts.p, ws.partial.p, nb, g, ws.counts.p + nb, ws.cursor.p, ws.redo.p);
-    hipLaunchKernelGGL(msm_fixup, dim3((nb + 63) / 64 + MSM_FIXUP_TEAM_BLOCKS + MSM_FIXUP_HEAVY_BLOCKS), dim3(64), 0, s, ws.counts.p, ws.offsets.p, ws.partial.p, ws.cursor.p, ws.bucket_pts.p, nb, g);
+        } else hipLaunchKernelGGL(msm_accumulate, dim3(acc_blocks), dim3(64), 0, s, ws.problems.p, ws.counts.p, ws.offsets.p, ws.list.p, ws.bucket_pts.p, ws.partial.p, nb, g, ws.counts.p + nb, ws.cursor.p, ws.fix_start.p, phi_tab, ws.redo.p);
+    }
+    hipLaunchKernelGGL(msm_accumulate_redo, dim3(256), dim3(64), 0, s, ws.problems.p, ws.counts.p, ws.offsets.p, ws.list.p, ws.bucket_pts.p, ws.partial.p, nb, g, ws.counts.p + nb, ws.cursor.p, ws.fix_start.p, ws.redo.p);
+    hipLaunchKernelGGL(msm_fixup, dim3((nb + 63) / 64 + MSM_FIXUP_TEAM_BLOCKS + MSM_FIXUP_HEAVY_BLOCKS), dim3(64), 0, s, ws.counts.p, ws.fix_start.p, ws.partial.p, ws.cursor.p, ws.bucket_pts.p, nb, g);
     {
-        const uint32_t nw = p.windows * count;
-        uint32_t T = msm_window_threads(p.buckets, nw, ws.tune.msm_window_threads), wpw = 1;
-        if (T == 64 && p.buckets >= 256 && nw > 256 && nw <= 512 && !ws.tune.msm_window_threads) { T = 128; wpw = 2; }
-        const uint32_t wpw_forced = (uint32_t)ws.tune.msm_window_wpw;
-        if ((wpw_forced == 1 || wpw_forced == 2 || wpw_forced == 4) && T * wpw_forced <= MSM_WIN_THREADS) wpw = wpw_forced;
-        const uint32_t slots = ((T * wpw <= 64 && nw > 1024) || ws.tune.msm_window_slots == 3) ? 3u : (uint32_t)MSM_WIN_SLOTS;
-        const size_t win_lds = (size_t)slots * T * wpw * sizeof(G1J);
-        if (win_lds > 64 * 1024) H2V_HIP_CHECK(hipFuncSetAttribute((const void*)msm_window, hipFuncAttributeMaxDynamicSharedMemorySize, (int)win_lds));
-        hipLaunchKernelGGL(msm_window, dim3((nw + wpw - 1) / wpw), dim3(T * wpw), win_lds, s, ws.bucket_pts.p, ws.counts.p, ws.window_sums.p, p, nw, wpw, slots);
+        const uint32_t nw_wide = lay.n_wide;
+        if (nw_wide) {
+            uint32_t T = msm_window_threads(p.buckets, nw_wide, ws.tune.msm_window_threads), wpw = 1;
+            if (T == 64 && p.buckets >= 256 && nw_wide > 256 && nw_wide <= 512 && !ws.tune.msm_window_threads) { T = 128; wpw = 2; }
+            const uint32_t wpw_forced = (uint32_t)ws.tune.msm_window_wpw;
+            if ((wpw_forced == 1 || wpw_forced == 2 || wpw_forced == 4) && T * wpw_forced <= MSM_WIN_THREADS) wpw = wpw_forced;
+            const uint32_t slots = ((T * wpw <= 64 && nw_wide > 1024) || ws.tune.msm_window_slots == 3) ? 3u : (uint32_t)MSM_WIN_SLOTS;
+            const size_t win_lds = (size_t)slots * T * wpw * sizeof(G1J);
+            if (win_lds > 64 * 1024) H2V_HIP_CHECK(hipFuncSetAttribute((const void*)msm_window, hipFuncAttributeMaxDynamicSharedMemorySize, (int)win_lds));
+            hipLaunchKernelGGL(msm_window, dim3((nw_wide + wpw - 1) / wpw), dim3(T * wpw), win_lds, s, ws.bucket_pts.p, ws.counts.p, ws.window_sums.p, p, nw_wide, wpw, slots,
+                               lay.n_narrow ? (const MsmSegInfo*)ws.seg_info.p : (const MsmSegInfo*)nullptr, lay.n_narrow ? (const uint32_t*)ws.seg_order.p : (const uint32_t*)nullptr);
+        }
+        if (lay.n_narrow) {
+            const uint32_t T = lay.narrow_T, wpw = 64u / T;
+            const size_t win_lds = (size_t)MSM_WIN_SLOTS * 64 * sizeof(G1J);
+            hipLaunchKernelGGL(msm_window, dim3((lay.n_narrow + wpw - 1) / wpw), dim3(64), win_lds, s, ws.bucket_pts.p, ws.counts.p, ws.window_sums.p,
+                               MsmPlan{0, lay.narrow_c, nw.windows, lay.narrow_buckets}, lay.n_narrow, wpw, (uint32_t)MSM_WIN_SLOTS, (const MsmSegInfo*)ws.seg_info.p, (const uint32_t*)ws.seg_order.p + lay.n_wide);
+        }
     }
     const G1JSlot* sums = ws.window_sums.p;
     if (cut) {
         hipLaunchKernelGGL(msm_merge_windows, dim3((8 * n_callers * p.windows + 63) / 64), dim3(64), 0, s, ws.window_sums.p, ws.parents.p, n_callers, p.windows, ws.merged_sums.p);
         sums = ws.merged_sums.p;
     }
-    if (split && split->want_parts > 1 && p.windows > 1) {
-        const uint32_t want = std::min<uint32_t>(split->want_parts, MSM_MAX_PARTS);
-        const uint32_t wpp = (p.windows + want - 1) / want, parts = (p.windows + wpp - 1) / wpp;
-        hipLaunchKernelGGL(msm_final_parts, dim3((4 * n_callers * parts + 63) / 64), dim3(64), 0, s, sums, ws.final_problems, n_callers, p, parts, wpp, ws.pieces.p, ws.pieces.p + (size_t)MSM_MAX_PARTS * ws.cap_problems);
-        split->parts = parts; split->shift = p.c * wpp; split->count = n_callers; split->pts = ws.pieces.p; split->ready = ws.pieces.p + (size_t)MSM_MAX_PARTS * ws.cap_problems;
+    const uint32_t own = cut ? 0u : 1u;
+    if (parts) {
+        hipLaunchKernelGGL(msm_final_parts, dim3((4 * n_callers * parts + 63) / 64), dim3(64), 0, s, sums, ws.final_problems, n_callers, p, parts, wpp, ws.pieces.p, ws.pieces.p + (size_t)MSM_MAX_PARTS * ws.cap_problems, own);
+        split->parts = parts; split->shift = shift; split->count = n_callers; split->pts = ws.pieces.p; split->ready = ws.pieces.p + (size_t)MSM_MAX_PARTS * ws.cap_problems;
     } else {
-        hipLaunchKernelGGL(msm_final, dim3((4 * n_callers + 63) / 64), dim3(64), 0, s, sums, ws.final_problems, n_callers, p);
+        hipLaunchKernelGGL(msm_final, dim3((4 * n_callers + 63) / 64), dim3(64), 0, s, sums, ws.final_problems, n_callers, p, own);
     }
     H2V_HIP_CHECK(hipGetLastError());
     return 0;
diff --git a/halo2_verifier_amd/csrc/msm_plan.h b/halo2_verifier_amd/csrc/msm_plan.h
--- /dev/null
+++ b/halo2_verifier_amd/csrc/msm_plan.h
@@ -0,0 +1,122 @@
+#pragma once
+#include <stdint.h>
+#include <algorithm>
+#include <vector>
+
+#if defined(__HIPCC__)
+#define H2V_PLAN_HD __host__ __device__
+#else
+#define H2V_PLAN_HD
+#endif
+
+namespace h2v {
+
+struct MsmPlan {
+    uint32_t n;
+    uint32_t c;
+    uint32_t windows;
+    uint32_t buckets;
+};
+#define MSM_MAX_PARTS 6
+
+static inline uint32_t msm_window_threads(uint32_t buckets, uint32_t n_workgroups = 0xffffffffu, int forced = 0) {
+    if (buckets <= 64) return std::max(1u, buckets);
+    if (n_workgroups != 0xffffffffu && (forced == 64 || forced == 128 || forced == 256)) return (uint32_t)forced;
+    if (buckets > 2048 || (buckets >= 256 && n_workgroups <= 256)) return 256u;
+    return 64u;
+}
+
+static inline uint32_t msm_windows_of(uint32_t c) { return (130 + c - 1) / c; }
+static inline double msm_throughput_cost(uint32_t n, uint32_t c, uint32_t T) {
+    const uint32_t w = msm_windows_of(c), b = 1u << (c - 1), slice = (b + T - 1) / T;
+    double lg = 0; for (uint32_t t = T; t > 1; t >>= 1) lg += 1;
+    return (double)w * (11.0 * 2.0 * n + 16.0 * T * (2.0 * slice + 1.5 * c + 1.0 + lg));
+}
+static inline double msm_cost_under(uint32_t n, const MsmPlan& p) { return msm_throughput_cost(n, p.c, msm_window_threads(p.buckets)); }
+
+static inline MsmPlan msm_plan_choose(uint32_t n, bool latency) {
+    MsmPlan best{n, 2, 65, 2};
+    double best_cost = 1e300;
+    for (uint32_t c = 2; c <= 15; ++c) {
+        uint32_t w = msm_windows_of(c);
+        uint32_t b = 1u << (c - 1);
+        uint32_t T = msm_window_threads(b), slice = (b + T - 1) / T;
+        double lg = 0; for (uint32_t t = T; t > 1; t >>= 1) lg += 1;
+        double cost = latency ? 9.0 * w + 9.0 * (2.0 * slice + 1.5 * c + 1.0 + lg) + 5.0 * std::min<double>(32.0, 2.0 * n)
+                              : msm_throughput_cost(n, c, T);
+        if (cost < best_cost) { best_cost = cost; best = MsmPlan{n, c, w, b}; }
+    }
+    return best;
+}
+
+struct MsmNarrow { uint32_t c = 0, windows = 0, buckets = 0, T = 0; double cost = 1e300; };
+static inline MsmNarrow msm_plan_narrow(uint32_t n) {
+    MsmNarrow best;
+    for (uint32_t c = 2; c <= 15; ++c) {
+        const uint32_t b = 1u << (c - 1);
+        for (uint32_t T = 8; T <= 64 && T <= b; T <<= 1) {
+            const double cost = msm_throughput_cost(n, c, T);
+            if (cost < best.cost) { best.c = c; best.windows = msm_windows_of(c); best.buckets = b; best.T = T; best.cost = cost; }
+        }
+    }
+    return best;
+}
+H2V_PLAN_HD static inline uint32_t msm_piece_first(uint32_t c, uint32_t shift, uint32_t j) { return (shift * j + c - 1) / c; }
+H2V_PLAN_HD static inline uint32_t msm_piece_trailing(uint32_t c, uint32_t shift, uint32_t j) { return msm_piece_first(c, shift, j) * c - shift * j; }
+static inline bool msm_narrow_fits_pieces(uint32_t c, uint32_t windows, uint32_t parts, uint32_t shift) { return parts == 0 || c * (windows - 1) < shift * parts; }
+static inline void msm_split_shape(const MsmPlan& p, uint32_t want, uint32_t& parts, uint32_t& wpp, uint32_t& shift) {
+    parts = 0; wpp = 0; shift = 0;
+    if (want <= 1 || p.windows <= 1) return;
+    want = std::min<uint32_t>(want, MSM_MAX_PARTS);
+    wpp = (p.windows + want - 1) / want; parts = (p.windows + wpp - 1) / wpp; shift = p.c * wpp;
+}
+static inline bool msm_take_narrow(uint32_t n, const MsmNarrow& nw, const MsmPlan& p, uint32_t parts, uint32_t shift) {
+    return nw.c != 0 && msm_throughput_cost(n, nw.c, nw.T) < msm_cost_under(n, p) && msm_narrow_fits_pieces(nw.c, nw.windows, parts, shift);
+}
+
+struct MsmSegInfo { uint32_t bin0, bins, prob, list0; };
+struct MsmProblemShape { uint32_t c, windows, buckets, T, seg_first, bin_first, dig_off, narrow; };
+inline bool operator==(const MsmProblemShape& a, const MsmProblemShape& b) {
+    return a.c == b.c && a.windows == b.windows && a.buckets == b.buckets && a.T == b.T && a.seg_first == b.seg_first && a.bin_first == b.bin_first && a.dig_off == b.dig_off && a.narrow == b.narrow;
+}
+struct MsmLayout {
+    std::vector<MsmProblemShape> prob;
+    std::vector<MsmSegInfo> seg;
+    std::vector<uint32_t> order;
+    uint32_t n_wide = 0, n_narrow = 0;
+    uint32_t narrow_T = 0, narrow_buckets = 0, narrow_c = 0;
+    uint32_t nb = 0, max_buckets = 0;
+    size_t list_words = 0, dig_words = 0;
+};
+static inline MsmLayout msm_layout(const uint32_t* terms, const uint8_t* narrow, uint32_t count, const MsmPlan& p, uint32_t nmax, const MsmNarrow& nw, bool lds) {
+    MsmLayout L;
+    L.prob.resize(count);
+    uint32_t seg = 0, bin = 0; size_t list = 0, dig = 0;
+    for (uint32_t q = 0; q < count; ++q) {
+        const bool nar = narrow && narrow[q];
+        MsmProblemShape& s = L.prob[q];
+        s.narrow = nar ? 1u : 0u;
+        s.c = nar ? nw.c : p.c; s.windows = nar ? nw.windows : p.windows; s.buckets = nar ? nw.buckets : p.buckets; s.T = nar ? nw.T : 0u;
+        s.seg_first = seg; s.bin_first = bin; s.dig_off = (uint32_t)dig;
+        L.max_buckets = std::max(L.max_buckets, s.buckets);
+        for (uint32_t w = 0; w < s.windows; ++w) {
+            if (lds) L.seg.push_back(MsmSegInfo{bin, s.buckets, q, (uint32_t)list});
+            L.order.push_back(seg);
+            list += nar ? 2 * (size_t)terms[q] : 2 * (size_t)nmax;
+            bin += s.buckets; ++seg;
+        }
+        dig += (size_t)s.windows * terms[q];
+        (nar ? L.n_narrow : L.n_wide) += s.windows;
+    }
+    if (L.n_narrow) {
+        L.narrow_T = nw.T; L.narrow_buckets = nw.buckets; L.narrow_c = nw.c;
+        std::vector<uint32_t> wide, nar;
+        for (uint32_t q = 0; q < count; ++q) for (uint32_t w = 0; w < L.prob[q].windows; ++w) (L.prob[q].narrow ? nar : wide).push_back(L.prob[q].seg_first + w);
+        L.order = wide; L.order.insert(L.order.end(), nar.begin(), nar.end());
+    }
+    L.nb = bin; L.list_words = list; L.dig_words = dig;
+    if (!lds) L.seg.push_back(MsmSegInfo{0, bin, 0, 0});
+    return L;
+}
+
+}
```

Result: slower. 11.66 million (-1.6%).
